# cslab-ntua/sparsex

Measured on AMD Instinct MI355X. Metric: SpMV GFLOP/s (2*nnz/t, alpha=0.5, x/y resident in HBM), higher is better.
Workload: dtype f64

## Files before the change

include/sparsex_hip.h:

```cpp
#ifndef SPARSEX_HIP_H
#define SPARSEX_HIP_H

#include <sparsex/sparsex.h>
#include <stdint.h>

#ifdef __cplusplus
extern "C" {
#endif

spx_error_t spx_hip_matvec_mult(spx_value_t alpha, const spx_matrix_t *A,
                                const spx_value_t *x_dev, spx_value_t *y_dev,
                                void *stream);
spx_error_t spx_hip_matvec_kernel(spx_value_t alpha, const spx_matrix_t *A,
                                  const spx_value_t *x_dev, spx_value_t beta,
                                  spx_value_t *y_dev, void *stream);

spx_error_t spx_hip_matvec_trans_mult(spx_value_t alpha, const spx_matrix_t *A,
                                      const spx_value_t *x_dev, spx_value_t *y_dev,
                                      void *stream);
spx_error_t spx_hip_matvec_trans_kernel(spx_value_t alpha, const spx_matrix_t *A,
                                        const spx_value_t *x_dev, spx_value_t beta,
                                        spx_value_t *y_dev, void *stream);
int spx_hip_matvec_trans_mode(const spx_matrix_t *A);

spx_error_t spx_hip_matvec_mult_f32(spx_value_t alpha, const spx_matrix_t *A, const spx_value_t *x_dev,
                                    spx_value_t *y_dev, void *stream);
spx_error_t spx_hip_matvec_kernel_f32(spx_value_t alpha, const spx_matrix_t *A, const spx_value_t *x_dev,
                                      spx_value_t beta, spx_value_t *y_dev, void *stream);
int64_t spx_hip_mat_values_f32_bytes(const spx_matrix_t *A);
double spx_hip_mat_values_f32_narrow_seconds(const spx_matrix_t *A);

spx_error_t spx_hip_matmat_kernel(spx_value_t alpha, const spx_matrix_t *A, size_t nvec,
                                  const spx_value_t *X_dev, size_t ldx, spx_value_t beta,
                                  spx_value_t *Y_dev, size_t ldy, void *stream);
int spx_hip_matmat_group(const spx_matrix_t *A);

spx_error_t spx_hip_matmat_rm_kernel(spx_value_t alpha, const spx_matrix_t *A, size_t nvec,
                                     const spx_value_t *X_dev, size_t ldx, spx_value_t beta,
                                     spx_value_t *Y_dev, size_t ldy, void *stream);
int spx_hip_matmat_rm_group(const spx_matrix_t *A);

spx_error_t spx_hip_matmat_kernel_f32(spx_value_t alpha, const spx_matrix_t *A, size_t nvec,
                                      const spx_value_t *X_dev, size_t ldx, spx_value_t beta,
                                      spx_value_t *Y_dev, size_t ldy, void *stream);
spx_error_t spx_hip_matmat_rm_kernel_f32(spx_value_t alpha, const spx_matrix_t *A, size_t nvec,
                                         const spx_value_t *X_dev, size_t ldx, spx_value_t beta,
                                         spx_value_t *Y_dev, size_t ldy, void *stream);
int spx_hip_matmat_group_f32(const spx_matrix_t *A);

typedef struct spx_hip_vec spx_hip_vec_t;

void spx_hip_vec_touch(const spx_vector_t *v);
int spx_hip_vec_page_locked(const spx_vector_t *v);

spx_hip_vec_t *spx_hip_vec_create(size_t size);
spx_hip_vec_t *spx_hip_vec_create_from_host(const spx_vector_t *v);
spx_error_t spx_hip_vec_destroy(spx_hip_vec_t *v);
spx_value_t *spx_hip_vec_data(spx_hip_vec_t *v);
size_t spx_hip_vec_size(const spx_hip_vec_t *v);
spx_error_t spx_hip_vec_upload(spx_hip_vec_t *dst, const spx_vector_t *src, void *stream);
spx_error_t spx_hip_vec_download(const spx_hip_vec_t *src, spx_vector_t *dst, void *stream);
spx_error_t spx_hip_vec_init(spx_hip_vec_t *v, spx_value_t val, void *stream);
spx_error_t spx_hip_vec_scale(const spx_hip_vec_t *v1, spx_hip_vec_t *v2, spx_value_t num,
                              void *stream);
spx_error_t spx_hip_vec_scale_add(const spx_hip_vec_t *v1, const spx_hip_vec_t *v2,
                                  spx_hip_vec_t *v3, spx_value_t num, void *stream);
spx_error_t spx_hip_vec_add(const spx_hip_vec_t *v1, const spx_hip_vec_t *v2,
                            spx_hip_vec_t *v3, void *stream);
spx_error_t spx_hip_vec_sub(const spx_hip_vec_t *v1, const spx_hip_vec_t *v2,
                            spx_hip_vec_t *v3, void *stream);
spx_error_t spx_hip_vec_mul(const spx_hip_vec_t *v1, const spx_hip_vec_t *v2,
                            spx_value_t *result, void *stream);
spx_error_t spx_hip_vec_copy(const spx_hip_vec_t *v1, spx_hip_vec_t *v2, void *stream);
spx_error_t spx_hip_vec_mul_dev(const spx_hip_vec_t *v1, const spx_hip_vec_t *v2,
                                spx_value_t *result_dev, void *stream);
spx_error_t spx_hip_vec_scale_add_ratio(const spx_hip_vec_t *v1, const spx_hip_vec_t *v2, spx_hip_vec_t *v3,
                                        spx_value_t scale, const spx_value_t *num_dev,
                                        const spx_value_t *den_dev, void *stream);
spx_error_t spx_hip_vec_cg_update(spx_hip_vec_t *x, const spx_hip_vec_t *p, spx_hip_vec_t *r,
                                  const spx_hip_vec_t *ap, spx_value_t *rr_dev,
                                  const spx_value_t *pap_dev, spx_value_t *beta_dev, void *stream);
spx_error_t spx_hip_vec_mul_elem(const spx_hip_vec_t *v1, const spx_hip_vec_t *v2, spx_hip_vec_t *v3, void *stream);
spx_error_t spx_hip_vec_reciprocal(const spx_hip_vec_t *v1, spx_hip_vec_t *v2, spx_value_t if_zero, void *stream);
spx_error_t spx_hip_vec_pcg_update(spx_hip_vec_t *x, const spx_hip_vec_t *p, spx_hip_vec_t *r, const spx_hip_vec_t *ap,
                                   const spx_hip_vec_t *minv, spx_value_t *rz_dev, const spx_value_t *pap_dev,
                                   spx_value_t *beta_dev, spx_value_t *rr_dev, void *stream);
spx_error_t spx_hip_vec_pcg_direction(spx_hip_vec_t *p, const spx_hip_vec_t *r, const spx_hip_vec_t *minv,
                                      const spx_value_t *beta_dev, void *stream);
spx_error_t spx_hip_probe_read_write(const spx_hip_vec_t *src, spx_hip_vec_t *dst, size_t chunk_doubles,
                                     size_t write_doubles, void *stream);
spx_error_t spx_hip_matvec_kernel_vec(spx_value_t alpha, const spx_matrix_t *A,
                                      const spx_hip_vec_t *x, spx_value_t beta,
                                      spx_hip_vec_t *y, void *stream);
spx_error_t spx_hip_matvec_kernel_f32_vec(spx_value_t alpha, const spx_matrix_t *A, const spx_hip_vec_t *x,
                                          spx_value_t beta, spx_hip_vec_t *y, void *stream);
spx_error_t spx_hip_matvec_trans_kernel_vec(spx_value_t alpha, const spx_matrix_t *A,
                                            const spx_hip_vec_t *x, spx_value_t beta,
                                            spx_hip_vec_t *y, void *stream);

typedef struct spx_hip_transport {
    void *ctx;
    int rank, world;
    int (*exchange_host)(void *ctx, const uint64_t *send, const size_t *send_off,
                         const size_t *send_cnt, uint64_t *recv, const size_t *recv_off,
                         const size_t *recv_cnt);
    int (*exchange_device)(void *ctx, const spx_value_t *send, const size_t *send_off,
                           const size_t *send_cnt, spx_value_t *recv, const size_t *recv_off,
                           const size_t *recv_cnt, void *stream);
} spx_hip_transport_t;

#define SPX_RCCL_ID_BYTES 128
spx_error_t spx_hip_rccl_unique_id(void *id);
// ... 182 lines not shown
```

sparsex_amd/api.py:

```python
import ctypes as C
import os

import numpy as np

SPX_SUCCESS = 0
SPX_FAILURE = -1
SPX_MAT_REORDER = 42
SPX_VEC_AS_IS = 43
SPX_VEC_TUNE = 44
SPX_INDEX_ZERO_BASED = 45
SPX_INDEX_ONE_BASED = 46

_HERE = os.path.dirname(os.path.abspath(__file__))


def lib_path():
    return os.environ.get("SPX_LIB_PATH") or os.path.join(_HERE, "lib", "libsparsex.so")


class SpxError(RuntimeError):
    pass


class VectorStruct(C.Structure):
# ... 56 lines not shown

class UnitRecord(C.Structure):
    _fields_ = [("type", C.c_int32), ("delta", C.c_int32), ("size", C.c_int32),
                ("row", C.c_int32), ("col", C.c_int32)]


_lib = None


def lib():
    global _lib
    if _lib is not None:
        return _lib
    path = lib_path()
    if not os.path.exists(path):
        raise SpxError(
            "libsparsex.so is not built (%s); run `make lib` or "
            "__graft_entry__.build() -- there is no fallback path" % path)
    L = C.CDLL(path, mode=C.RTLD_GLOBAL)
    vp, i, d = C.c_void_p, C.c_int, C.c_double
    L.spx_input_load_csr.restype = vp
    L.spx_input_load_mmf.restype = vp
    L.spx_input_load_mmf.argtypes = [C.c_char_p]
    L.spx_input_destroy.argtypes = [vp]
    L.spx_mat_tune.restype = vp
    L.spx_mat_destroy.argtypes = [vp]
    L.spx_mat_get_nrows.argtypes = [vp]
    L.spx_mat_get_ncols.argtypes = [vp]
    L.spx_mat_get_nnz.argtypes = [vp]
    L.spx_mat_get_partition.restype = vp
    L.spx_mat_get_partition.argtypes = [vp]
    L.spx_partition_get_rs.restype = C.POINTER(C.c_int)
    L.spx_partition_get_rs.argtypes = [vp]
    L.spx_partition_get_re.restype = C.POINTER(C.c_int)
    L.spx_partition_get_re.argtypes = [vp]
    L.spx_partition_destroy.argtypes = [vp]
    L.spx_option_set.argtypes = [C.c_char_p, C.c_char_p]
    L.spx_option_set.restype = None
    L.spx_hip_options_reset.restype = None
    L.spx_vec_create_from_buff.restype = C.POINTER(VectorStruct)
    L.spx_vec_create_from_buff.argtypes = [C.POINTER(C.c_double), vp, C.c_size_t, vp,
                                           C.c_uint]
    L.spx_vec_destroy.argtypes = [C.POINTER(VectorStruct)]
    L.spx_vec_destroy.restype = None
    L.spx_matvec_mult.argtypes = [d, vp, C.POINTER(VectorStruct), C.POINTER(VectorStruct)]
    L.spx_matvec_kernel.argtypes = [d, vp, C.POINTER(VectorStruct), d,
                                    C.POINTER(VectorStruct)]
    L.spx_hip_matvec_mult.argtypes = [d, vp, vp, vp, vp]
    L.spx_hip_matvec_kernel.argtypes = [d, vp, vp, d, vp, vp]
    L.spx_hip_mat_info.argtypes = [vp, C.POINTER(HipInfo)]
    L.spx_hip_mat_export_csx.argtypes = [vp, i, C.POINTER(CsxExport)]
    L.spx_hip_mat_export_units.restype = C.c_int64
    L.spx_hip_mat_export_units.argtypes = [vp, i, C.POINTER(UnitRecord), C.c_int64]
    L.spx_hip_mat_tune_log.restype = C.c_char_p
    L.spx_hip_mat_tune_log.argtypes = [vp]
    L.spx_hip_vec_create.restype = vp
    L.spx_hip_vec_create.argtypes = [C.c_size_t]
    L.spx_hip_vec_destroy.argtypes = [vp]
    L.spx_hip_vec_data.restype = vp
    L.spx_hip_vec_data.argtypes = [vp]
    L.spx_hip_vec_size.restype = C.c_size_t
    L.spx_hip_vec_size.argtypes = [vp]
    L.spx_hip_vec_upload.argtypes = [vp, C.POINTER(VectorStruct), vp]
    L.spx_hip_vec_download.argtypes = [vp, C.POINTER(VectorStruct), vp]
    L.spx_hip_vec_init.argtypes = [vp, d, vp]
    L.spx_hip_vec_scale.argtypes = [vp, vp, d, vp]
    L.spx_hip_vec_scale_add.argtypes = [vp, vp, vp, d, vp]
    L.spx_hip_vec_add.argtypes = [vp, vp, vp, vp]
    L.spx_hip_vec_sub.argtypes = [vp, vp, vp, vp]
    L.spx_hip_vec_mul.argtypes = [vp, vp, C.POINTER(C.c_double), vp]
    L.spx_hip_vec_copy.argtypes = [vp, vp, vp]
    L.spx_hip_vec_mul_dev.argtypes = [vp, vp, vp, vp]
    L.spx_hip_vec_scale_add_ratio.argtypes = [vp, vp, vp, d, vp, vp, vp]
    L.spx_hip_vec_cg_update.argtypes = [vp, vp, vp, vp, vp, vp, vp, vp]
    L.spx_hip_matvec_kernel_vec.argtypes = [d, vp, vp, d, vp, vp]
    L.spx_hip_matvec_trans_mult.argtypes = [d, vp, vp, vp, vp]
    L.spx_hip_matvec_trans_kernel.argtypes = [d, vp, vp, d, vp, vp]
    L.spx_hip_matvec_trans_kernel_vec.argtypes = [d, vp, vp, d, vp, vp]
    L.spx_hip_matvec_mult_f32.argtypes = [d, vp, vp, vp, vp]
    L.spx_hip_matvec_kernel_f32.argtypes = [d, vp, vp, d, vp, vp]
    L.spx_hip_matvec_kernel_f32_vec.argtypes = [d, vp, vp, d, vp, vp]
    L.spx_hip_mat_values_f32_bytes.restype = C.c_int64
    L.spx_hip_mat_values_f32_bytes.argtypes = [vp]
    L.spx_hip_mat_values_f32_narrow_seconds.restype = C.c_double
    L.spx_hip_mat_values_f32_narrow_seconds.argtypes = [vp]
    L.spx_hip_matvec_trans_mode.restype = C.c_int
    L.spx_hip_matvec_trans_mode.argtypes = [vp]
    L.spx_hip_mat_values_plan.argtypes = [vp, vp, vp, i]
    L.spx_hip_mat_values_plan_drop.argtypes = [vp]
    L.spx_hip_mat_set_values.argtypes = [vp, vp, vp]
    L.spx_hip_mat_set_values_host.argtypes = [vp, vp]
    L.spx_hip_mat_values_plan_get.argtypes = [vp, C.POINTER(ValuesPlan)]
    L.spx_hip_mat_diag_plan.argtypes = [vp]
    L.spx_hip_mat_diag_plan_drop.argtypes = [vp]
    L.spx_hip_mat_get_diag.argtypes = [vp, vp, vp]
    L.spx_hip_mat_get_diag_vec.argtypes = [vp, vp, vp]
    L.spx_hip_mat_get_diag_host.argtypes = [vp, vp]
    L.spx_hip_mat_diag_plan_get.argtypes = [vp, C.POINTER(DiagPlan)]
    L.spx_hip_vec_mul_elem.argtypes = [vp, vp, vp, vp]
    L.spx_hip_vec_reciprocal.argtypes = [vp, vp, d, vp]
    L.spx_hip_vec_pcg_update.argtypes = [vp, vp, vp, vp, vp, vp, vp, vp, vp, vp]
    L.spx_hip_vec_pcg_direction.argtypes = [vp, vp, vp, vp, vp]
    L.spx_log_disable_all.restype = None
    L.spx_log_error_console.restype = None
    _lib = L
    return L


def option_set(option, value):
    lib().spx_option_set(str(option).encode(), str(value).encode())


def options_reset():
    lib().spx_hip_options_reset()


class Input:

    def __init__(self, handle, keep=()):
        self.handle = handle
        self._keep = keep

    def destroy(self):
        if self.handle:
            lib().spx_input_destroy(self.handle)
            self.handle = None

    def __del__(self):
        try:
            self.destroy()
        except Exception:
            pass


def input_load_csr(rowptr, colind, values, nrows, ncols, indexing=SPX_INDEX_ZERO_BASED):
    rp = np.ascontiguousarray(rowptr, dtype=np.int32)
    ci = np.ascontiguousarray(colind, dtype=np.int32)
    va = np.ascontiguousarray(values, dtype=np.float64)
    h = lib().spx_input_load_csr(
        rp.ctypes.data_as(C.c_void_p), ci.ctypes.data_as(C.c_void_p),
        va.ctypes.data_as(C.c_void_p), C.c_int(nrows), C.c_int(ncols), C.c_int(indexing))
    if not h:
        raise SpxError("spx_input_load_csr failed")
    return Input(h, keep=(rp, ci, va))


def input_load_mmf(filename):
    h = lib().spx_input_load_mmf(str(filename).encode())
    if not h:
        raise SpxError("spx_input_load_mmf failed for %s" % filename)
    return Input(h)


class Matrix:

    def __init__(self, handle):
        self.handle = handle
        L = lib()
        self.nrows = L.spx_mat_get_nrows(handle)
        self.ncols = L.spx_mat_get_ncols(handle)
        self.nnz = L.spx_mat_get_nnz(handle)

    def matvec_mult(self, alpha, x, y):
        return self._host(alpha, x, None, y)

    def matvec_kernel(self, alpha, x, beta, y):
        return self._host(alpha, x, beta, y)

    def _host(self, alpha, x, beta, y):
        L = lib()
        assert x.dtype == np.float64 and y.dtype == np.float64
        assert x.flags.c_contiguous and y.flags.c_contiguous
        xv = L.spx_vec_create_from_buff(x.ctypes.data_as(C.POINTER(C.c_double)), None,
                                        x.size, None, SPX_VEC_AS_IS)
        yv = L.spx_vec_create_from_buff(y.ctypes.data_as(C.POINTER(C.c_double)), None,
                                        y.size, None, SPX_VEC_AS_IS)
        try:
            if beta is None:
                rc = L.spx_matvec_mult(alpha, self.handle, xv, yv)
            else:
                rc = L.spx_matvec_kernel(alpha, self.handle, xv, beta, yv)
        finally:
            L.spx_vec_destroy(xv)
            L.spx_vec_destroy(yv)
        if rc != SPX_SUCCESS:
            raise SpxError("spx_matvec failed (see stderr)")
        return y

    def partition(self):
        L = lib()
        p = L.spx_mat_get_partition(self.handle)
        n = self.info().nr_partitions
        rs = [L.spx_partition_get_rs(p)[i] for i in range(n)]
        re = [L.spx_partition_get_re(p)[i] for i in range(n)]
        L.spx_partition_destroy(p)
        return rs, re

    def hip_matvec_mult(self, alpha, x_ptr, y_ptr, stream=0):
        rc = lib().spx_hip_matvec_mult(alpha, self.handle, x_ptr, y_ptr, stream)
        if rc != SPX_SUCCESS:
            raise SpxError("spx_hip_matvec_mult failed (see stderr)")

    def hip_matvec_kernel(self, alpha, x_ptr, beta, y_ptr, stream=0):
        rc = lib().spx_hip_matvec_kernel(alpha, self.handle, x_ptr, beta, y_ptr, stream)
        if rc != SPX_SUCCESS:
            raise SpxError("spx_hip_matvec_kernel failed (see stderr)")

    def hip_matvec_trans_kernel(self, alpha, x_ptr, beta, y_ptr, stream=0):
        rc = lib().spx_hip_matvec_trans_kernel(alpha, self.handle, x_ptr, beta, y_ptr, stream)
        if rc != SPX_SUCCESS:
            raise SpxError("spx_hip_matvec_trans_kernel failed (see stderr)")

    def trans_mode(self):
        return int(lib().spx_hip_matvec_trans_mode(self.handle))

    def matvec_trans(self, alpha, x, beta, y, stream=None):
        import torch
        pairs = (("x", x, self.nrows), ("y", y, self.ncols))
        for name, t, n in pairs:
            if not isinstance(t, torch.Tensor):
                raise ValueError("%s must be a torch tensor" % name)
            if t.dtype != torch.float64:
                raise ValueError("%s must be float64, not %s" % (name, t.dtype))
            if t.dim() != 1 or t.shape[0] != n:
                raise ValueError("%s must have the shape (%d,), not %s" % (name, n, tuple(t.shape)))
            if t.shape[0] > 1 and t.stride(0) != 1:
                raise ValueError("%s needs stride(0) == 1, not %d" % (name, t.stride(0)))
        for name, t, n in pairs:
            if t.device.type != "cuda":
                raise ValueError("%s must live on the matrix' HIP device, not on %s" % (name, t.device))
        if x.device != y.device:
            raise ValueError("x and y live on different devices (%s, %s)" % (x.device, y.device))
        inf = self.info()
        if inf.on_device and x.device.index != inf.device:
            raise ValueError("the matrix lives on cuda:%d, the tensors on %s" % (inf.device, x.device))
        st = stream if stream is not None else torch.cuda.current_stream(y.device)
        self.hip_matvec_trans_kernel(alpha, x.data_ptr(), beta, y.data_ptr(), st.cuda_stream)
        return y

    def hip_matvec_kernel_f32(self, alpha, x_ptr, beta, y_ptr, stream=0):
        rc = lib().spx_hip_matvec_kernel_f32(alpha, self.handle, x_ptr, beta, y_ptr, stream)
        if rc != SPX_SUCCESS:
            raise SpxError("spx_hip_matvec_kernel_f32 failed (see stderr)")

    def values_f32_bytes(self):
        return int(lib().spx_hip_mat_values_f32_bytes(self.handle))

    def matvec_f32(self, alpha, x, beta, y, stream=None):
        import torch
        pairs = (("x", x, self.ncols), ("y", y, self.nrows))
        for name, t, n in pairs:
            if not isinstance(t, torch.Tensor):
                raise ValueError("%s must be a torch tensor" % name)
            if t.dtype != torch.float64:
                raise ValueError("%s must be float64, not %s" % (name, t.dtype))
            if t.dim() != 1 or t.shape[0] != n:
                raise ValueError("%s must have the shape (%d,), not %s" % (name, n, tuple(t.shape)))
            if t.shape[0] > 1 and t.stride(0) != 1:
                raise ValueError("%s needs stride(0) == 1, not %d" % (name, t.stride(0)))
        for name, t, n in pairs:
            if t.device.type != "cuda":
                raise ValueError("%s must live on the matrix' HIP device, not on %s" % (name, t.device))
        if x.device != y.device:
            raise ValueError("x and y live on different devices (%s, %s)" % (x.device, y.device))
        inf = self.info()
        if inf.on_device and x.device.index != inf.device:
            raise ValueError("the matrix lives on cuda:%d, the tensors on %s" % (inf.device, x.device))
        st = stream if stream is not None else torch.cuda.current_stream(y.device)
        self.hip_matvec_kernel_f32(alpha, x.data_ptr(), beta, y.data_ptr(), st.cuda_stream)
        return y

    def hip_matmat_kernel(self, alpha, x_ptr, ldx, nvec, beta, y_ptr, ldy, stream=0):
        L = lib()
        L.spx_hip_matmat_kernel.restype = C.c_int
        L.spx_hip_matmat_kernel.argtypes = [C.c_double, C.c_void_p, C.c_size_t, C.c_void_p, C.c_size_t,
                                            C.c_double, C.c_void_p, C.c_size_t, C.c_void_p]
        rc = L.spx_hip_matmat_kernel(alpha, self.handle, nvec, x_ptr, ldx, beta, y_ptr, ldy, stream)
        if rc != SPX_SUCCESS:
            raise SpxError("spx_hip_matmat_kernel failed (see stderr)")

    def matmat_group(self):
        L = lib()
        L.spx_hip_matmat_group.restype = C.c_int
        L.spx_hip_matmat_group.argtypes = [C.c_void_p]
        return int(L.spx_hip_matmat_group(C.c_void_p(self.handle)))

    def matmat(self, alpha, X, beta, Y, stream=None):
        return self._matmat(self.hip_matmat_kernel, alpha, X, beta, Y, stream)

    def _matmat(self, kernel, alpha, X, beta, Y, stream):
        import torch
        pairs = (("X", X, self.ncols), ("Y", Y, self.nrows))
        for name, t, n in pairs:
            if not isinstance(t, torch.Tensor):
                raise ValueError("%s must be a torch tensor" % name)
            if t.dtype != torch.float64:
                raise ValueError("%s must be float64, not %s" % (name, t.dtype))
            if t.dim() != 2 or t.shape[1] != n:
                raise ValueError("%s must have the shape (nvec, %d), not %s" % (name, n, tuple(t.shape)))
            if t.shape[0] > 0 and t.shape[1] > 1 and t.stride(1) != 1:
                raise ValueError("%s needs stride(1) == 1, not %d" % (name, t.stride(1)))
            if t.shape[0] > 1 and t.stride(0) < n:
                raise ValueError("%s: stride(0) %d is below the vector length %d" % (name, t.stride(0), n))
        if X.shape[0] != Y.shape[0]:
            raise ValueError("X holds %d vectors, Y %d" % (X.shape[0], Y.shape[0]))
        for name, t, n in pairs:
            if t.device.type != "cuda":
                raise ValueError("%s must live on the matrix' HIP device, not on %s" % (name, t.device))
        if X.device != Y.device:
            raise ValueError("X and Y live on different devices (%s, %s)" % (X.device, Y.device))
        inf = self.info()
        if inf.on_device and X.device.index != inf.device:
            raise ValueError("the matrix lives on cuda:%d, the tensors on %s" % (inf.device, X.device))
        nvec = int(X.shape[0])
        ldx = max(int(X.stride(0)), self.ncols) if nvec > 1 else max(self.ncols, 1)
        ldy = max(int(Y.stride(0)), self.nrows) if nvec > 1 else max(self.nrows, 1)
        st = stream if stream is not None else torch.cuda.current_stream(Y.device)
        kernel(alpha, X.data_ptr(), ldx, nvec, beta, Y.data_ptr(), ldy, st.cuda_stream)
        return Y

    def hip_matmat_kernel_f32(self, alpha, x_ptr, ldx, nvec, beta, y_ptr, ldy, stream=0):
        L = lib()
        L.spx_hip_matmat_kernel_f32.restype = C.c_int
        L.spx_hip_matmat_kernel_f32.argtypes = [C.c_double, C.c_void_p, C.c_size_t, C.c_void_p, C.c_size_t,
                                                C.c_double, C.c_void_p, C.c_size_t, C.c_void_p]
        rc = L.spx_hip_matmat_kernel_f32(alpha, self.handle, nvec, x_ptr, ldx, beta, y_ptr, ldy, stream)
        if rc != SPX_SUCCESS:
            raise SpxError("spx_hip_matmat_kernel_f32 failed (see stderr)")

# ... 750 lines not shown
```

sparsex_amd/csrc/api.cpp:

```cpp
#include <sparsex/sparsex.h>
#include <sparsex_hip.h>

#include "config.hpp"
#include "csx_emit.hpp"
#include "device.hpp"
#include "dist.hpp"
#include "encoder.hpp"
#include "gpu_emit.hpp"
#include "input.hpp"
#include "reorder.hpp"
#include "stream_index.hpp"
#include "threads.hpp"

#include <chrono>
#include <cmath>
#include <cstdarg>
#include <cstdint>
#include <cstring>
#include <functional>
#include <memory>
#include <mutex>
#include <atomic>
#include <sstream>
#include <thread>
// ... 497 lines not shown
            emit_pieces(fulls, &tiles, use_segs ? &segs : nullptr);
            {
                struct Gone {
                    std::vector<Partition> fulls;
                    std::vector<SymSegVec> segs;
                    std::vector<std::vector<SymTile>> tiles;
                };
                Gone *g = new Gone();
                g->fulls.swap(fulls);
                g->segs.swap(segs);
                g->tiles.swap(tiles);
                release_after_upload = [g] {
                    parallel_for(g->fulls.size(), host_threads(), [&](size_t i) {
                        g->fulls[i] = Partition();
                        if (i < g->segs.size()) SymSegVec().swap(g->segs[i]);
                        if (i < g->tiles.size()) std::vector<SymTile>().swap(g->tiles[i]);
                    });
                    delete g;
                };
            }
            for (size_t k = 0; k < thin.size(); ++k) {
                if (k == 0 || thin[k].row != thin[k - 1].row) {
                    gs.mirror_rows.push_back((uint32_t) thin[k].row);
                    gs.mirror_ptr.push_back((uint32_t) k);
                }
                gs.mirror_col.push_back((uint32_t) thin[k].col);
                gs.mirror_val.push_back(thin[k].val);
            }
            gs.mirror_ptr.push_back((uint32_t) thin.size());
            gs.nnz_stored += thin.size();
            gs.n_delta_elems += thin.size();
        } else {
            Partition full;
            for (size_t i = 0; i < nown; ++i) append_sym_expanded(A->parts[i], full, gp.sym_remine);
            if (gs.sym_fused) full.nr_rows = (size_t) A->nrows;
            emit_gpu(full, gp, gs, hw);
        }
    } else if (A->col_phases <= 1) {
        emit_pieces(A->parts, nullptr);
    } else {
        const size_t K = A->col_phases;
        GpuEmitParams keep = gp;
        gp.max_rows = std::max<size_t>(gp.max_rows, SPX_MAX_WIDE_ROWS);
        for (size_t k = 0; k < K; ++k) {
            const idx_t c_lo = (idx_t)((int64_t) A->ncols * (int64_t) k / (int64_t) K) + 1;
            const idx_t c_hi = (idx_t)((int64_t) A->ncols * (int64_t)(k + 1) / (int64_t) K) + 1;
            std::vector<Partition> sub(nown);
            parallel_for(nown, hw, [&](size_t i) {
                const Partition &p = A->parts[i];
                Partition &q = sub[i];
                q.nr_rows = p.nr_rows; q.nr_cols = p.nr_cols; q.type = p.type; q.row_start = p.row_start;
                q.pool = p.pool;
                for (size_t e = 0; e < p.elems_size; ++e)
                    if (p.elems[e].col >= c_lo && p.elems[e].col < c_hi) {
                        q.elems.push_back(p.elems[e]);
                        q.nnz += p.elems[e].size;
                    }
                q.elems_size = q.elems.size();
            });
            gp.skip_empty = k > 0 || A->col_concurrent;
            const size_t rb0 = gs.rbs.size();
            emit_pieces(sub, nullptr);
            if (k > 0 && gs.rbs.size() > rb0) gs.rbs[rb0].flags |= SPX_RB_PHASE_START;
            if (A->col_concurrent && gs.rbs.size() == rb0) throw FatalError("column phases: an empty slice");
        }
        if (A->col_concurrent)
            for (SpxRowBlock &rb : gs.rbs) rb.flags |= SPX_RB_ACCUM;
        gp = keep;
        if (!gs.shared.empty()) throw FatalError("column phases: the matrix holds rows that are split over row-blocks");
    }
    const double t_emit1 = now_sec();
    A->conflict_rows.clear();
    if (sym && !gs.sym_fused) stream_touched_rows(gs, A->own_lo, A->conflict_rows);
    A->halo_cols.clear();
    if (A->own_lo > 0 || A->own_hi < A->nrows) stream_read_cols(gs, A->own_lo, A->own_hi, (size_t) A->ncols, A->halo_cols);
    A->first_block_row = A->own_lo;
    for (const SpxRowBlock &rb : gs.rbs) A->first_block_row = std::min<idx_t>(A->first_block_row, (idx_t) rb.row0);
    finalize_stream(gs, (size_t) A->nrows);
    if (sym) mark_private_rowblocks(gs, (size_t) A->nrows, A->own_lo, A->own_hi);
    std::vector<std::pair<uint32_t, uint32_t>>().swap(gs.direct_cols);
    gs.waves = (uint32_t) A->waves;
    gs.band_order = Config::instance().get_bool("spx.gpu.band_order");
    gs.arena = Config::instance().get_bool("spx.gpu.arena");
    gs.xw_budget = (A->unit_windows != 0 && !A->deterministic && !sym) ? (A->rb_joined ? std::max(A->xw_budget, JOINED_XW_BUDGET) : A->xw_budget) : 0u;
    gs.xw_gap = A->xw_gap;
    gs.xw_on = A->xw_on;
    gs.sx_plan = sym && A->sym_pipeline != 0 && !A->deterministic && A->wave_tiles != 1;
    gs.sx_on = A->sx_on;
    gs.sym_matmat = A->sym_matmat;
    gs.sym_atomic = A->sym_atomic && !A->deterministic;
    gs.deterministic = A->deterministic;
    gs.wave_tiles = A->deterministic || A->wave_tiles == 1;
    A->nnz_stored = gs.nnz_stored;
    A->n_unit_elems = gs.n_unit_elems;
    A->n_delta_elems = gs.n_delta_elems;
    A->n_units = gs.n_units;
    A->value_bytes = gs.values.size() * sizeof(val_t);
    A->index_bytes = gs.index_bytes();
    A->n_rowblocks = gs.rbs.size();
    A->n_shared = gs.shared.size();
    A->has_tiles = stream_has_tiles(gs);
    A->has_symtiles = stream_has_pass(gs, SPX_PASS_SYMTILE);
    if (A->dev) {
        device_free(A->dev);
        A->dev = nullptr;
    }
    const double t_emit2 = now_sec();
    if (!A->host_only) {
        A->dev = device_upload(gs, (size_t) A->nrows, (size_t) A->ncols, sym, A->own_lo, A->own_hi,
                               A->device_ordinal);
        device_set_trans_windows(A->dev, A->trans_windows);
        log_msg(LOG_INFO, "descriptor stream: emitted in %.2f s, finalized in %.2f s, uploaded in %.2f s (%zu row-blocks)\n",
                t_emit1 - t_emit0, t_emit2 - t_emit1, now_sec() - t_emit2, gs.rbs.size());
        if (A->dist && sym) {
            device_set_init_rows(A->dev, (size_t) dist_first_init_row(*A));
        }
        keep_index(A, std::move(gs));
    } else {
        A->host_stream.reset(new GpuStream(std::move(gs)));
    }
    if (release_after_upload) {
        std::function<void()> f;
        f.swap(release_after_upload);
        A->release_wait();
        A->release_later(std::move(f));
    }
}

static void autotune_launch(spx_matrix_t *A, bool tune_waves, bool tune_spill, bool tune_wave_tiles, bool tune_xw)
{
    A->release_wait();
    const double t_est = device_time_spmv(A->dev, 2, 3);
    const int N = (int) std::min(100.0, std::max(8.0, 0.02 / std::max(t_est, 1e-7)));
    const int W = std::max(2, N / 10);
    auto best_time = [&]() {
        A->release_wait();
        double best = device_time_spmv(A->dev, W, N);
        for (int rep = 0; rep < 3; ++rep) best = std::min(best, device_time_spmv(A->dev, 0, N));
        return best;
    };
    auto time_xw = [&](bool &xw) {
        if (!tune_xw || !device_has_xw(A->dev) || A->wave_tiles == 1) {
            xw = device_get_xw(A->dev);
            return best_time();
        }
        device_set_xw(A->dev, false);
        const double t0 = best_time();
        device_set_xw(A->dev, true);
        const double t1 = best_time();
        xw = t1 < 0.985 * t0;
        device_set_xw(A->dev, xw);
        return std::min(t0, xw ? t1 : t0);
    };
    if (!tune_waves) {
        if (tune_wave_tiles && !device_has_tiles(A->dev) && !(A->unit_windows == 1 && device_has_xw(A->dev))) {
            auto t_of = [&](bool on) {
                device_set_wave_tiles(A->dev, on);
                return best_time();
            };
            const double t0 = t_of(false), t1 = t_of(true);
            bool on = t1 < 0.985 * t0;
            if (on) {
                const double t0b = t_of(false), t1b = t_of(true);
                on = t1b < 0.985 * t0b;
            }
            A->wave_tiles = on ? 1 : 0;
// ... 58 lines not shown
            emit_and_upload(A);
            bool xw2 = false;
            const double t2 = time_with(2, xw2);
            if (t2 < 0.985 * best_t) {
                best_t = t2;
                best_waves = 2;
                best_scale = scale;
                best_xw = xw2;
            }
        }
        A->xw_on = best_xw;
        if (A->rb_scale != best_scale) {
            A->rb_scale = best_scale;
            A->waves = best_waves;
            emit_and_upload(A);
        }
    }
    if (A->auto_rb && A->n_rowblocks > 4096 &&
        auto_target_elems(A, 2.0) != auto_target_elems(A, best_scale)) {
        A->rb_scale = 2.0;
        A->waves = best_waves;
        emit_and_upload(A);
        bool xwb = false;
        const double tb = time_with(best_waves, xwb);
        if (tb < 0.985 * best_t) {
            best_t = tb;
            best_scale = 2.0;
            best_xw = xwb;
            A->xw_on = best_xw;
        } else {
            A->rb_scale = best_scale;
            A->xw_on = best_xw;
            emit_and_upload(A);
        }
    }
    A->rb_scale = best_scale;
    A->waves = best_waves;
    A->xw_on = best_xw;
    if (A->auto_rb && best_xw && A->wave_tiles != 1 && A->emit_params.max_rows <= SPX_MAX_RB_ROWS &&
        A->value_bytes > ((size_t) 1 << 30)) {
        A->rb_joined = true;
        A->waves = 8;
        emit_and_upload(A);
        bool xwj = false;
        const double tj = time_with(8, xwj);
        if (xwj && tj < 0.995 * best_t) {
            best_t = tj;
            best_waves = 8;
            log_msg(LOG_INFO, "launch autotune: row-blocks joined side by side (%zu of them)\n", A->n_rowblocks);
        } else {
            A->rb_joined = false;
            A->waves = best_waves;
            A->xw_on = best_xw;
            emit_and_upload(A);
        }
    }
    A->waves = best_waves;
    A->xw_on = best_xw;
    device_set_waves(A->dev, best_waves);
    device_set_xw(A->dev, best_xw);
    log_msg(LOG_INFO, "launch autotune: %d wavefronts per workgroup, row-block scale %.2f%s, unit windows %s (%.2f us per SpMV)\n",
            best_waves, best_scale, A->rb_joined ? ", joined" : "", best_xw ? "on" : "off", 1e6 * best_t);
}

static int read_trans_windows()
{
    const std::string tw = Config::instance().get_str("spx.gpu.trans_windows");
    if (tw != "auto" && tw != "true" && tw != "false") {
        log_msg(LOG_ERR, "spx.gpu.trans_windows: true, false or auto\n");
        throw FatalError("bad spx.gpu.trans_windows");
    }
    return tw == "auto" ? -1 : (tw == "true" ? 1 : 0);
}

static int read_values_f32()
{
    const std::string v = Config::instance().get_str("spx.gpu.values_f32");
    if (v != "true" && v != "false" && v != "all") {
        log_msg(LOG_ERR, "spx.gpu.values_f32: false, true or all\n");
        throw FatalError("bad spx.gpu.values_f32");
    }
    return v == "all" ? 2 : (v == "true" ? 1 : 0);
}
static bool wants_values_f32(int mode, bool symmetric) { return mode == 2 || (mode == 1 && !symmetric); }

static spx_matrix_t *do_tune(spx_input_t *in)
{
    Config &cfg = Config::instance();
    const double t0 = now_sec();
    const size_t P = cfg.nr_partitions();
    long world = std::max<long>(1, cfg.get_long("spx.rt.gpu_world"));
    long rank = cfg.get_long("spx.rt.gpu_rank");
    if (rank < 0 || rank >= world || P % (size_t) world != 0) {
        log_msg(LOG_ERR, "spx.rt.gpu_rank/gpu_world (%ld/%ld) do not divide "
                "spx.rt.nr_threads=%zu partitions\n", rank, world, P);
        throw FatalError("bad gpu_rank/gpu_world");
    }
    const size_t first = (size_t) rank * (P / (size_t) world);
    const size_t last = first + P / (size_t) world;
    const long slice_rows = cfg.get_long("spx.rt.global_rows");
    const long slice_off = slice_rows > 0 ? cfg.get_long("spx.rt.row_offset") : 0;
    if (slice_rows > 0 && (world != 1 || slice_off < 0 || slice_off + (long) in->nrows > slice_rows)) {
        log_msg(LOG_ERR, "spx.rt.row_offset/global_rows (%ld/%ld) do not hold the %ld input rows "
                "(and exclude spx.rt.gpu_world > 1)\n", slice_off, slice_rows, (long) in->nrows);
        throw FatalError("bad row slice");
    }
    in->mat->row_base = (size_t) slice_off;
    in->mat->global_rows = slice_rows > 0 ? (size_t) slice_rows : 0;
    const idx_t rows_end = slice_rows > 0 ? (idx_t)(slice_off + in->nrows) : in->nrows;
    const bool sym = cfg.get_bool("spx.matrix.symmetric");
    const bool host_only = cfg.get_bool("spx.rt.host_only");
    EncoderParams prm = EncoderParams::from_config(cfg);
    XformSeq seq = cfg.xform();
    cfg.cpu_affinity();
    log_msg(LOG_INFO, "Format: %s\n", sym ? "CSX-sym" : "CSX");
    if (!host_only && device_count() <= 0) {
        log_msg(LOG_ERR, "no usable HIP device: this library multiplies on an MI355X "
                "only (spx.rt.host_only=true preprocesses without one)\n");
        throw FatalError("no HIP device");
    }

    std::unique_ptr<matrix> A(new matrix);
    A->nrows = slice_rows > 0 ? (spx_index_t) slice_rows : in->nrows;
    A->ncols = in->ncols;
    A->nnz = in->nnz;
    A->symmetric = sym ? 1 : 0;
    A->permutation = SPX_INVALID_PERM;
    A->nr_partitions = P;
    A->first_part = first;
    A->last_part = last;
    A->full_colind = cfg.get_bool("spx.matrix.full_colind");
    A->dev = nullptr;
    A->host_only = host_only;
    A->device_ordinal = (int) cfg.get_long("spx.rt.device");
    A->input_row_base = slice_rows > 0 ? (int64_t) slice_off : -1;

    const size_t nown = last - first;
    std::vector<std::ostringstream> logs(nown);
    std::vector<std::string> errors(nown);
    std::vector<PartitionSym> sparts;
    if (sym) {
        build_partitions_sym(*in->mat, P, first, last, sparts, A->bounds);
        A->diag.resize(nown);
    } else {
        build_partitions(*in->mat, P, first, last, A->parts, A->bounds);
    }

    const double t_parts = now_sec();
    log_msg(LOG_INFO, "partitions built in %.2f s\n", t_parts - t0);
    auto work = [&](size_t i) {
        try {
            std::ostream *lg = &logs[i];
            *lg << "==> Thread: #" << (first + i) << "\n==== ENCODING STATISTICS ====\n";
            if (sym) {
                PartitionSym &ps = sparts[i];
                ps.divide();
                Encoder e1(&ps.m1, prm), e2(&ps.m2, prm);
                if (seq.explicit_deltas) {
                    e1.encode_serial(seq);
                    e2.encode_serial(seq);
                } else {
                    e1.remove_ignore(seq);
                    e2.remove_ignore(seq);
                    if (ps.lower.row_start > 0) e1.encode_all(lg);
                    e2.encode_all(lg);
                }
// ... 45 lines not shown
    A->emit_params.sym_pure_passes = cfg.get_bool("spx.gpu.sym_pure_passes");
    A->emit_params.x_window = cfg.get_bool("spx.gpu.x_window");
    {
        const std::string m = cfg.get_str("spx.gpu.sym_segments");
        if (m != "auto" && m != "true" && m != "false") {
            log_msg(LOG_ERR, "spx.gpu.sym_segments: true, false or auto\n");
            throw FatalError("bad spx.gpu.sym_segments");
        }
        A->emit_params.sym_segments = m == "auto" ? -1 : (m == "true" ? 1 : 0);
        const long wide = cfg.get_long("spx.gpu.sym_wide_rows");
        if (wide < 1 || wide > SPX_MAX_WIDE_ROWS) {
            log_msg(LOG_ERR, "spx.gpu.sym_wide_rows: 1 .. %d\n", SPX_MAX_WIDE_ROWS);
            throw FatalError("bad spx.gpu.sym_wide_rows");
        }
        A->emit_params.wide_rows = (size_t) wide;
        const long mr = cfg.get_long("spx.gpu.sym_segment_min");
        if (mr < 2 || mr > 8) {
            log_msg(LOG_ERR, "spx.gpu.sym_segment_min: 2 .. 8\n");
            throw FatalError("bad spx.gpu.sym_segment_min");
        }
        A->emit_params.sym_min_run = (size_t) mr;
        const long xr = cfg.get_long("spx.gpu.sym_segment_max");
        if (xr < mr || xr > SPX_MAX_SEG_WIDTH) {
            log_msg(LOG_ERR, "spx.gpu.sym_segment_max: spx.gpu.sym_segment_min .. %d\n", SPX_MAX_SEG_WIDTH);
            throw FatalError("bad spx.gpu.sym_segment_max");
        }
        A->emit_params.sym_max_run = (size_t) xr;
    }
    A->emit_params.stack_segments = cfg.get_bool("spx.gpu.stack_segments");
    {
        idx_t lo = nown ? A->bounds[first].row_start : 0;
        idx_t hi = nown ? A->bounds[last - 1].row_start + A->bounds[last - 1].nr_rows : 0;
        if (last == P) hi = rows_end;
        A->own_lo = lo;
        A->own_hi = hi;
    }
    A->waves = (int) cfg.get_long("spx.gpu.waves");
    const bool autotune = A->waves == 0;
    if (autotune) A->waves = 4;
    const std::string spill_mode = cfg.get_str("spx.gpu.sym_spill");
    if (spill_mode != "auto" && spill_mode != "lists" && spill_mode != "atomic") {
        log_msg(LOG_ERR, "spx.gpu.sym_spill: lists, atomic or auto\n");
        throw FatalError("bad spx.gpu.sym_spill");
    }
    A->deterministic = cfg.get_bool("spx.gpu.deterministic");
    A->sym_atomic = spill_mode == "atomic" && !A->deterministic;
    A->spill_mode = spill_mode == "lists" ? 0 : (spill_mode == "atomic" ? 1 : -1);
    {
        const std::string sm = cfg.get_str("spx.gpu.sym_matmat");
        if (sm != "true" && sm != "false") {
            log_msg(LOG_ERR, "spx.gpu.sym_matmat: true or false\n");
            throw FatalError("bad spx.gpu.sym_matmat");
        }
        A->sym_matmat = sm == "true" && sym && A->emit_params.sym_once;
        if (A->sym_matmat) {
            if (spill_mode == "auto" && !A->deterministic) A->sym_atomic = true;
            A->emit_params.wide_rows = std::min<size_t>(A->emit_params.wide_rows, SPX_MAX_RB_ROWS);
        }
    }
    const std::string wt_mode = cfg.get_str("spx.gpu.wave_tiles");
    if (wt_mode != "auto" && wt_mode != "true" && wt_mode != "false") {
        log_msg(LOG_ERR, "spx.gpu.wave_tiles: true, false or auto\n");
        throw FatalError("bad spx.gpu.wave_tiles");
    }
    A->wave_tiles = wt_mode == "true" ? 1 : 0;
    const std::string xw_mode = cfg.get_str("spx.gpu.unit_windows");
    if (xw_mode != "auto" && xw_mode != "true" && xw_mode != "false") {
        log_msg(LOG_ERR, "spx.gpu.unit_windows: true, false or auto\n");
        throw FatalError("bad spx.gpu.unit_windows");
    }
    {
        const long xb = cfg.get_long("spx.gpu.unit_window_doubles"), xg = cfg.get_long("spx.gpu.unit_window_gap");
        if (xb < 0 || xb > 16384 || xg < 0 || xg > 255) {
            log_msg(LOG_ERR, "spx.gpu.unit_window_doubles: 0 .. 16384, spx.gpu.unit_window_gap: 0 .. 255\n");
            throw FatalError("bad spx.gpu.unit_window_doubles / spx.gpu.unit_window_gap");
        }
        A->xw_budget = (uint32_t) xb;
        A->xw_gap = (uint32_t) xg;
    }
    A->unit_windows = xw_mode == "auto" ? -1 : (xw_mode == "true" ? 1 : 0);
    A->xw_on = xw_mode == "true";
    A->trans_windows = read_trans_windows();
    A->values_f32 = read_values_f32();
    const std::string sx_mode = cfg.get_str("spx.gpu.sym_pipeline");
    if (sx_mode != "auto" && sx_mode != "true" && sx_mode != "false") {
        log_msg(LOG_ERR, "spx.gpu.sym_pipeline: true, false or auto\n");
        throw FatalError("bad spx.gpu.sym_pipeline");
    }
    A->sym_pipeline = sx_mode == "auto" ? -1 : (sx_mode == "true" ? 1 : 0);
    A->sx_on = sx_mode == "true";
    const std::string ph_mode = cfg.get_str("spx.gpu.col_phases");
    const bool ph_conc = ph_mode.size() == 2 && ph_mode[0] == 'c';
    long ph_fixed = ph_mode == "auto" ? 0 : strtol(ph_mode.c_str() + (ph_conc ? 1 : 0), nullptr, 10);
    if (ph_mode != "auto" && (ph_fixed < 1 || ph_fixed > 8 || (ph_conc && ph_fixed != 2 && ph_fixed != 4 && ph_fixed != 8))) {
        log_msg(LOG_ERR, "spx.gpu.col_phases: 1 .. 8 (launched in turn), c2 | c4 | c8 (one launch, a group of XCDs each) or auto\n");
        throw FatalError("bad spx.gpu.col_phases");
    }
    A->col_phases = (!sym && ph_fixed > 1) ? (size_t) ph_fixed : 1;
    A->col_concurrent = A->col_phases > 1 && ph_conc && !A->deterministic;
    if (A->col_phases > 1 && ph_conc && !A->col_concurrent) A->col_phases = 1;
    try {
        emit_and_upload(A.get());
    } catch (const FatalError &) {
        if (A->col_phases <= 1) throw;
        A->col_phases = 1;
        emit_and_upload(A.get());
    }
    const bool tune_spill = spill_mode == "auto" && !A->deterministic && !A->has_symsegs && !A->sym_matmat;
    const bool tune_wt = wt_mode == "auto" && !A->deterministic && !A->has_symsegs;
    const bool tune_xw = xw_mode == "auto" && !A->deterministic && !sym;
    const double t_auto = now_sec();
    if (A->dev && A->nnz_stored >= 100000 && (autotune || tune_spill || tune_wt || tune_xw))
        autotune_launch(A.get(), autotune, tune_spill, tune_wt, tune_xw);
    if (A->dev && sym && A->sym_pipeline == -1 && device_has_sx(A->dev)) {
        A->release_wait();
        const double t_est = device_time_spmv(A->dev, 2, 3);
        const int N = (int) std::min(100.0, std::max(8.0, 0.02 / std::max(t_est, 1e-7)));
        auto best_of = [&](bool on) {
            device_set_sx(A->dev, on);
            double best = device_time_spmv(A->dev, std::max(2, N / 10), N);
            for (int rep = 0; rep < 3; ++rep) best = std::min(best, device_time_spmv(A->dev, 0, N));
            return best;
        };
        const double t0 = best_of(false), t1 = best_of(true);
        A->sx_on = t1 < 0.985 * t0;
        device_set_sx(A->dev, A->sx_on);
        log_msg(LOG_INFO, "read-once pipeline: %s (%.2f us per SpMV with, %.2f without)\n", A->sx_on ? "on" : "off", 1e6 * t1, 1e6 * t0);
    }
    const double t_auto_end = now_sec();
    if (A->dev && !sym && ph_mode == "auto" && A->n_shared == 0 && A->nnz_stored >= 100000 &&
        2 * A->n_delta_elems >= A->nnz_stored && (size_t) A->ncols * sizeof(val_t) >= ((size_t) 6 << 20)) {
        auto best_of = [&]() {
            double best = device_time_spmv(A->dev, 10, 100);
            for (int rep = 0; rep < 3; ++rep) best = std::min(best, device_time_spmv(A->dev, 0, 100));
            return best;
        };
        const double t_plain = best_of();
        size_t K = 1;
        double t_ph = t_plain;
        if (!A->deterministic) {
            for (size_t k : {(size_t) 2, (size_t) 4}) {
                if ((size_t) A->ncols * sizeof(val_t) < k * ((size_t) 3 << 19)) break;
                try {
                    A->col_phases = k;
                    A->col_concurrent = true;
                    emit_and_upload(A.get());
                    const double t = best_of();
                    if (t < 0.97 * t_ph) {
                        t_ph = t;
                        K = k;
                    }
                } catch (const FatalError &) {
                    break;
                }
            }
        }
        if (A->col_phases != K || !A->col_concurrent) {
            A->col_phases = K;
            A->col_concurrent = K > 1;
            emit_and_upload(A.get());
        }
        log_msg(LOG_INFO, "column slices: %zu on XCD groups %.2f us, plain %.2f us per SpMV\n", K, 1e6 * t_ph, 1e6 * t_plain);
    }

    if (A->dev && wants_values_f32(A->values_f32, sym)) device_build_values_f32(A->dev);

    if (!cfg.get_bool("spx.rt.keep_encoded")) {
        std::vector<Partition> *old = new std::vector<Partition>();
        old->swap(A->parts);
        A->release_later([old] {
            parallel_for(old->size(), host_threads(), [&](size_t i) { (*old)[i] = Partition(); });
            delete old;
        });
    }
    log_msg(LOG_INFO, "launch parameters measured in %.2f s\n", t_auto_end - t_auto);
    A->emit_seconds = now_sec() - t1;
    return A.release();
}

spx_matrix_t *spx_mat_tune(spx_input_t *in, ...)
try {
    if (!in) {
        SETERROR_1(SPX_ERR_ARG_INVALID, "invalid input matrix");
        return SPX_INVALID_MAT;
    }
    va_list ap;
    va_start(ap, in);
    spx_option_t option = va_arg(ap, spx_option_t);
    va_end(ap);
    std::vector<idx_t> perm;
    if (option == SPX_MAT_REORDER && Config::instance().get_long("spx.rt.global_rows") > 0) {
        SETWARNING(SPX_WARN_REORDER);
        option = 0;
    }
    int re_mode = SPX_DIST_REORDER_RCM;
    size_t re_world = 1;
// ... 479 lines not shown
    if (good) {
        good = h.nrows >= 0 && h.ncols >= 0 && bnd.size() == 3 * h.nr_partitions &&
               h.first_part <= h.last_part && h.last_part <= h.nr_partitions &&
               (perm.empty() || perm.size() == (size_t) h.nrows) && h.own_lo >= 0 &&
               h.own_lo <= h.own_hi && h.own_hi <= h.nrows &&
               (!h.symmetric || gs->dvalues.size() == (size_t) h.nrows);
        for (int32_t v : perm) good = good && v >= 0 && v < h.nrows;
    }
    if (good) {
        gs->n_carry = h.n_carry;
        gs->sym_fused = (h.pad & 1u) != 0;
        gs->pass_stride = h.pad >> 1;
        gs->n_spill = h.n_spill;
        gs->lds_doubles = h.lds_doubles;
        gs->waves = h.waves;
        gs->sym_atomic = h.sym_atomic != 0;
        gs->deterministic = (h.pad3 & 1u) != 0;
        gs->wave_tiles = (h.pad3 & 2u) != 0;
        gs->xw_on = (h.pad3 & 4u) != 0;
        gs->sx_on = (h.pad3 & 8u) != 0;
        gs->sx_plan = gs->sx_on;
        gs->xw_gap = gs->xw_on ? ((h.pad3 >> 8) & 255u) : 16u;
        gs->xw_budget = gs->xw_on ? (h.pad3 >> 16) : 0u;
        gs->nnz_stored = h.nnz_stored; gs->n_unit_elems = h.n_unit_elems;
        gs->n_delta_elems = h.n_delta_elems; gs->n_units = h.n_units;
        good = stream_checksum(*gs) == h.checksum;
        if (!good) why = "tuned-matrix file is damaged (checksum of the index arrays)";
        else good = stream_validate(*gs, (size_t) h.nrows, (size_t) h.ncols, gs->values.size(), why);
    }
    if (!good) {
        SETERROR_1(SPX_ERR_FILE, why.c_str());
        return SPX_INVALID_MAT;
    }
    A->nrows = h.nrows; A->ncols = h.ncols; A->nnz = h.nnz; A->symmetric = h.symmetric;
    A->permutation = SPX_INVALID_PERM;
    if (!perm.empty()) {
        A->permutation = (spx_perm_t *) malloc(perm.size() * sizeof(spx_perm_t));
        std::copy(perm.begin(), perm.end(), A->permutation);
    }
    A->nr_partitions = h.nr_partitions; A->first_part = h.first_part; A->last_part = h.last_part;
    for (size_t i = 0; i < h.nr_partitions; ++i)
        A->bounds.push_back(PartBounds{bnd[3 * i], bnd[3 * i + 1], (size_t) bnd[3 * i + 2]});
    A->full_colind = false;
    A->dev = nullptr;
    A->waves = (h.waves == 2 || h.waves == 8) ? (int) h.waves : 4;
    A->own_lo = h.own_lo; A->own_hi = h.own_hi;
    if (h.first_part == 0 && h.last_part == h.nr_partitions && (h.own_lo > 0 || h.own_hi < h.nrows))
        A->input_row_base = h.own_lo;
    A->nnz_stored = h.nnz_stored; A->n_unit_elems = h.n_unit_elems;
    A->n_delta_elems = h.n_delta_elems; A->n_units = h.n_units;
    A->value_bytes = gs->values.size() * sizeof(val_t);
    A->index_bytes = gs->index_bytes();
    A->n_rowblocks = gs->rbs.size();
    A->n_shared = gs->shared.size();
    A->has_tiles = stream_has_tiles(*gs);
    A->has_symtiles = stream_has_pass(*gs, SPX_PASS_SYMTILE);
    A->has_symsegs = stream_has_symsegs(*gs);
    A->sym_atomic = gs->sym_atomic;
    A->deterministic = gs->deterministic;
    A->wave_tiles = gs->wave_tiles ? 1 : 0;
    A->xw_on = gs->xw_on;
    A->unit_windows = gs->xw_on ? 1 : 0;
    A->sx_on = gs->sx_on;
    A->sym_pipeline = gs->sx_on ? 1 : 0;
    A->xw_budget = gs->xw_budget;
    A->xw_gap = gs->xw_gap;
    {
        size_t slices = 1;
        for (size_t i = 1; i < gs->rbs.size(); ++i) slices += (gs->rbs[i].flags & SPX_RB_PHASE_START) ? 1 : 0;
        A->col_phases = slices;
        A->col_concurrent = slices > 1 && !gs->rbs.empty() && (gs->rbs[0].flags & SPX_RB_ACCUM);
    }
    A->tune_seconds = 0.0;
    A->auto_rb = false;
    const double t0 = now_sec();
    Config &cfg = Config::instance();
    A->host_only = cfg.get_bool("spx.rt.host_only");
    A->device_ordinal = (int) cfg.get_long("spx.rt.device");
    A->full_colind = cfg.get_bool("spx.matrix.full_colind");
    A->sym_matmat = gs->sym_matmat = A->symmetric && cfg.get_str("spx.gpu.sym_matmat") == "true";
    try {
        A->trans_windows = read_trans_windows();
        A->values_f32 = read_values_f32();
    } catch (const FatalError &) {
        SETERROR_0(SPX_ERR_TUNED_MAT);
        return SPX_INVALID_MAT;
    }
    if (A->symmetric && !gs->sym_fused) stream_touched_rows(*gs, A->own_lo, A->conflict_rows);
    if (A->own_lo > 0 || A->own_hi < A->nrows) stream_read_cols(*gs, A->own_lo, A->own_hi, (size_t) A->ncols, A->halo_cols);
    A->first_block_row = A->own_lo;
    for (const SpxRowBlock &rb : gs->rbs) A->first_block_row = std::min<idx_t>(A->first_block_row, (idx_t) rb.row0);
    try {
        if (!A->host_only) {
            A->dev = device_upload(*gs, (size_t) A->nrows, (size_t) A->ncols, A->symmetric != 0,
                                   A->own_lo, A->own_hi, A->device_ordinal);
            device_set_trans_windows(A->dev, A->trans_windows);
            if (wants_values_f32(A->values_f32, A->symmetric != 0)) device_build_values_f32(A->dev);
            keep_index(A.get(), std::move(*gs));
        } else {
            A->host_stream = std::move(gs);
        }
    } catch (const FatalError &) {
        SETERROR_0(SPX_ERR_TUNED_MAT);
        return SPX_INVALID_MAT;
    }
    A->emit_seconds = now_sec() - t0;
    return A.release();
} SPX_C_BOUNDARY(return SPX_INVALID_MAT;)

spx_index_t spx_mat_get_nrows(const spx_matrix_t *A)
try {
    if (!A) { SETERROR_1(SPX_ERR_ARG_INVALID, "invalid matrix handle"); return SPX_FAILURE; }
    return A->nrows;
} SPX_C_BOUNDARY(return 0;)

spx_index_t spx_mat_get_ncols(const spx_matrix_t *A)
try {
    if (!A) { SETERROR_1(SPX_ERR_ARG_INVALID, "invalid matrix handle"); return SPX_FAILURE; }
    return A->ncols;
} SPX_C_BOUNDARY(return 0;)

spx_index_t spx_mat_get_nnz(const spx_matrix_t *A)
try {
    if (!A) { SETERROR_1(SPX_ERR_ARG_INVALID, "invalid matrix handle"); return SPX_FAILURE; }
    return A->nnz;
} SPX_C_BOUNDARY(return 0;)

static spx_partition_t *part_alloc(size_t n)
{
    spx_partition_t *p = (spx_partition_t *) malloc(sizeof(spx_partition_t));
    p->nr_partitions = n;
    p->parts = NULL;
    p->nodes = NULL;
    p->affinity = NULL;
    p->row_start = (spx_index_t *) malloc(sizeof(spx_index_t) * (n ? n : 1));
    p->row_end = (spx_index_t *) malloc(sizeof(spx_index_t) * (n ? n : 1));
    return p;
}

spx_partition_t *spx_mat_get_partition(const spx_matrix_t *A)
try {
    if (!A) {
        SETERROR_1(SPX_ERR_ARG_INVALID, "invalid matrix handle");
        return SPX_INVALID_PART;
    }
    spx_partition_t *p = part_alloc(A->nr_partitions);
    for (size_t i = 0; i < A->nr_partitions; ++i) {
        p->row_start[i] = A->bounds[i].row_start;
        p->row_end[i] = A->bounds[i].row_start + A->bounds[i].nr_rows;
    }
    return p;
} SPX_C_BOUNDARY(return SPX_INVALID_PART;)

spx_index_t *spx_partition_get_rs(const spx_partition_t *p)
try {
    if (!p) { SETERROR_1(SPX_ERR_ARG_INVALID, "invalid partition handle"); return NULL; }
    return p->row_start;
} SPX_C_BOUNDARY(return nullptr;)

spx_index_t *spx_partition_get_re(const spx_partition_t *p)
try {
    if (!p) { SETERROR_1(SPX_ERR_ARG_INVALID, "invalid partition handle"); return NULL; }
    return p->row_end;
} SPX_C_BOUNDARY(return nullptr;)

spx_perm_t *spx_mat_get_perm(const spx_matrix_t *A)
try {
    if (!A) {
        SETERROR_1(SPX_ERR_ARG_INVALID, "invalid matrix handle");
        return SPX_INVALID_PERM;
    }
    if (!A->permutation) {
        SETERROR_1(SPX_ERR_ARG_INVALID, "a permutation is not available");
        return SPX_INVALID_PERM;
    }
    return A->permutation;
} SPX_C_BOUNDARY(return SPX_INVALID_PERM;)

spx_partition_t *spx_partition_csr(const spx_index_t *rowptr, spx_index_t nr_rows,
// ... 165 lines not shown
    }
    return SPX_SUCCESS;
}

spx_error_t spx_hip_matvec_mult(spx_value_t alpha, const spx_matrix_t *A,
                                const spx_value_t *x_dev, spx_value_t *y_dev, void *stream)
try {
    return spx_hip_matvec_kernel(alpha, A, x_dev, 0.0, y_dev, stream);
} SPX_C_BOUNDARY(return SPX_FAILURE;)

spx_error_t spx_hip_matvec_kernel(spx_value_t alpha, const spx_matrix_t *A,
                                  const spx_value_t *x_dev, spx_value_t beta,
                                  spx_value_t *y_dev, void *stream)
try {
    if (check_dev(A, x_dev, y_dev) != SPX_SUCCESS) return SPX_FAILURE;
    try {
        device_spmv(A->dev, alpha, x_dev, beta, y_dev, stream);
    } catch (const FatalError &e) {
        SETERROR_1(SPX_ERR_TUNED_MAT, e.what.c_str());
        return SPX_FAILURE;
    }
    return SPX_SUCCESS;
} SPX_C_BOUNDARY(return SPX_FAILURE;)

spx_error_t spx_hip_matvec_trans_mult(spx_value_t alpha, const spx_matrix_t *A,
                                      const spx_value_t *x_dev, spx_value_t *y_dev, void *stream)
try {
    return spx_hip_matvec_trans_kernel(alpha, A, x_dev, 0.0, y_dev, stream);
} SPX_C_BOUNDARY(return SPX_FAILURE;)

spx_error_t spx_hip_matvec_trans_kernel(spx_value_t alpha, const spx_matrix_t *A,
                                        const spx_value_t *x_dev, spx_value_t beta,
                                        spx_value_t *y_dev, void *stream)
try {
    if (check_dev(A, x_dev, y_dev) != SPX_SUCCESS) return SPX_FAILURE;
    const uintptr_t x0 = (uintptr_t) x_dev, x1 = x0 + (size_t) A->nrows * sizeof(double);
    const uintptr_t y0 = (uintptr_t) y_dev, y1 = y0 + (size_t) A->ncols * sizeof(double);
    if (x0 < y1 && y0 < x1) {
        SETERROR_1(SPX_ERR_ARG_INVALID, "vectors x and y overlap");
        return SPX_FAILURE;
    }
    if (A->dist && !A->symmetric) {
        SETERROR_1(SPX_ERR_TUNED_MAT, "no transposed product on a general matrix with an exchange plan attached");
        return SPX_FAILURE;
    }
    try {
        device_spmv_trans(A->dev, alpha, x_dev, beta, y_dev, stream);
    } catch (const FatalError &e) {
        SETERROR_1(SPX_ERR_TUNED_MAT, e.what.c_str());
        return SPX_FAILURE;
    }
    return SPX_SUCCESS;
} SPX_C_BOUNDARY(return SPX_FAILURE;)

spx_error_t spx_hip_matvec_mult_f32(spx_value_t alpha, const spx_matrix_t *A,
                                    const spx_value_t *x_dev, spx_value_t *y_dev, void *stream)
try {
    return spx_hip_matvec_kernel_f32(alpha, A, x_dev, 0.0, y_dev, stream);
} SPX_C_BOUNDARY(return SPX_FAILURE;)

spx_error_t spx_hip_matvec_kernel_f32(spx_value_t alpha, const spx_matrix_t *A,
                                      const spx_value_t *x_dev, spx_value_t beta,
                                      spx_value_t *y_dev, void *stream)
try {
    if (check_dev(A, x_dev, y_dev) != SPX_SUCCESS) return SPX_FAILURE;
    const uintptr_t x0 = (uintptr_t) x_dev, x1 = x0 + (size_t) A->ncols * sizeof(double);
    const uintptr_t y0 = (uintptr_t) y_dev, y1 = y0 + (size_t) A->nrows * sizeof(double);
    if (x0 < y1 && y0 < x1) {
        SETERROR_1(SPX_ERR_ARG_INVALID, "vectors x and y overlap");
        return SPX_FAILURE;
    }
    try {
        device_spmv_f32(A->dev, alpha, x_dev, beta, y_dev, stream);
    } catch (const FatalError &e) {
        SETERROR_1(SPX_ERR_TUNED_MAT, e.what.c_str());
        return SPX_FAILURE;
    }
    return SPX_SUCCESS;
} SPX_C_BOUNDARY(return SPX_FAILURE;)

int64_t spx_hip_mat_values_f32_bytes(const spx_matrix_t *A)
try {
    return A && A->dev ? device_values_f32_bytes(A->dev) : -1;
} SPX_C_BOUNDARY(return -1;)

double spx_hip_mat_values_f32_narrow_seconds(const spx_matrix_t *A)
try {
    if (!A || !A->dev || device_values_f32_bytes(A->dev) <= 0) return -1.0;
    return device_time_narrow_values(A->dev);
} SPX_C_BOUNDARY(return -1.0;)

int spx_hip_matvec_trans_mode(const spx_matrix_t *A)
try {
    return A && A->dev ? device_trans_mode(A->dev) : -1;
} SPX_C_BOUNDARY(return -1;)

spx_error_t spx_hip_matvec_parts(spx_value_t alpha, const spx_matrix_t *A, const spx_value_t *x_dev,
                                 spx_value_t beta, spx_value_t *y_dev, int parts, void *stream, int *launched)
try {
    if (check_dev(A, x_dev, y_dev) != SPX_SUCCESS) return SPX_FAILURE;
    try {
        std::vector<size_t> bounds;
        const size_t K = (A->symmetric || parts < 2) ? 0 : device_plan_chunks(A->dev, (size_t) parts, bounds, 1);
        if (K == 0) {
            device_spmv(A->dev, alpha, x_dev, beta, y_dev, stream);
        } else {
            for (size_t k = 0; k < K; ++k) device_spmv_chunk(A->dev, k, alpha, x_dev, beta, y_dev, stream, 1);
        }
        if (launched) *launched = K ? (int) K : 1;
    } catch (const FatalError &e) {
        SETERROR_1(SPX_ERR_TUNED_MAT, e.what.c_str());
        return SPX_FAILURE;
    }
    return SPX_SUCCESS;
} SPX_C_BOUNDARY(return SPX_FAILURE;)

spx_error_t spx_hip_matvec_dist(spx_value_t alpha, const spx_matrix_t *A,
                                const spx_value_t *x_dev, spx_value_t beta,
                                spx_value_t *y_dev, int flags, void *stream)
try {
    if (check_dev(A, x_dev, y_dev) != SPX_SUCCESS) return SPX_FAILURE;
    if (!A->dist) {
        SETERROR_1(SPX_ERR_TUNED_MAT, "matrix has no exchange plan (spx_hip_mat_dist_attach)");
        return SPX_FAILURE;
    }
    try {
        if ((flags & SPX_DIST_OVERLAP) && (flags & SPX_DIST_HALO_X) && !(flags & SPX_DIST_GATHER_Y) &&
            !A->symmetric && A->dist->rounds && A->dist->world > 1) {
            dist_step_overlapped(A->dist, A->dev, alpha, x_dev, beta, y_dev, stream);
            return SPX_SUCCESS;
        }
        device_spmv(A->dev, alpha, x_dev, beta, y_dev, stream);
        dist_complete(A->dist, y_dev, (flags & SPX_DIST_GATHER_Y) != 0, (flags & SPX_DIST_HALO_X) != 0, stream);
    } catch (const FatalError &e) {
        SETERROR_1(SPX_ERR_TUNED_MAT, e.what.c_str());
        return SPX_FAILURE;
    }
    return SPX_SUCCESS;
} SPX_C_BOUNDARY(return SPX_FAILURE;)

static spx_error_t matmat_checked(bool f32, spx_value_t alpha, const spx_matrix_t *A, size_t nvec,
                                  const spx_value_t *X_dev, size_t ldx, spx_value_t beta,
                                  spx_value_t *Y_dev, size_t ldy, void *stream)
{
    if (!A) { SETERROR_1(SPX_ERR_ARG_INVALID, "invalid matrix handle"); return SPX_FAILURE; }
    if (!A->dev) {
        SETERROR_1(SPX_ERR_TUNED_MAT,
                   "matrix was tuned with spx.rt.host_only=true: no HIP executor");
        return SPX_FAILURE;
    }
    if (nvec == 0) return SPX_SUCCESS;
    if (!X_dev) { SETERROR_1(SPX_ERR_ARG_INVALID, "invalid block X"); return SPX_FAILURE; }
    if (!Y_dev) { SETERROR_1(SPX_ERR_ARG_INVALID, "invalid block Y"); return SPX_FAILURE; }
    const size_t nr = (size_t) A->nrows, nc = (size_t) A->ncols;
    if (ldx < nc || ldy < nr) {
        SETERROR_1(SPX_ERR_DIM, "leading dimension below the vector length (ldx >= ncols, ldy >= nrows)");
        return SPX_FAILURE;
    }
    const size_t limit = SIZE_MAX / sizeof(double);
    if ((ldx && nvec - 1 > (limit - nc) / ldx) || (ldy && nvec - 1 > (limit - nr) / ldy)) {
        SETERROR_1(SPX_ERR_ARG_INVALID, "block larger than the address space");
        return SPX_FAILURE;
    }
    const uintptr_t x0 = (uintptr_t) X_dev, x1 = x0 + ((nvec - 1) * ldx + nc) * sizeof(double);
    const uintptr_t y0 = (uintptr_t) Y_dev, y1 = y0 + ((nvec - 1) * ldy + nr) * sizeof(double);
    if (x0 < y1 && y0 < x1) {
// ... 844 lines not shown
```

sparsex_amd/csrc/config.cpp:

```cpp
#include "config.hpp"

#include <cstdlib>
#include <regex>
#include <sstream>

namespace spx {

Config &Config::instance()
{
    static Config c;
    return c;
}

Config::Config() { reset_defaults(); }

void Config::reset_defaults()
{
    props_.clear();
    props_["spx.rt.nr_threads"] = "1";
    props_["spx.rt.cpu_affinity"] = "0";
    props_["spx.preproc.heuristic"] = "ratio";
    props_["spx.preproc.xform"] = "all";
    props_["spx.preproc.sampling"] = "portion";
    props_["spx.preproc.sampling.nr_samples"] = "48";
    props_["spx.preproc.sampling.portion"] = "0.01";
    props_["spx.preproc.sampling.window_size"] = "0";
    props_["spx.matrix.symmetric"] = "false";
    props_["spx.matrix.split_blocks"] = "true";
    props_["spx.matrix.full_colind"] = "false";
    props_["spx.matrix.min_unit_size"] = "4";
    props_["spx.matrix.max_unit_size"] = "255";
    props_["spx.matrix.min_coverage"] = "0.1";
    props_["spx.matrix.onedim_blocks"] = "false";
    props_["spx.rt.host_only"] = "false";
    props_["spx.rt.gpu_rank"] = "0";
    props_["spx.rt.gpu_world"] = "1";
    props_["spx.rt.device"] = "-1";
    props_["spx.vec.register"] = "auto";
    props_["spx.vec.device"] = "false";
    props_["spx.rt.host_parts"] = "0";
    props_["spx.rt.dist_chunks"] = "4";
    props_["spx.rt.dist_reorder"] = "none";
    props_["spx.rt.row_offset"] = "0";
    props_["spx.rt.global_rows"] = "0";
    props_["spx.rt.keep_encoded"] = "true";
    props_["spx.gpu.rowblock_elems"] = "0";
    props_["spx.gpu.rowblock_rows"] = "512";
    props_["spx.gpu.stack_segments"] = "true";
    props_["spx.gpu.waves"] = "0";
    props_["spx.gpu.inline_desc"] = "true";
    props_["spx.gpu.arena"] = "false";
    props_["spx.gpu.band_order"] = "false";
    props_["spx.gpu.col_phases"] = "auto";
    props_["spx.gpu.keep_units"] = "true";
    props_["spx.gpu.recut_linear"] = "true";
    props_["spx.gpu.sym_once"] = "true";
    props_["spx.gpu.deterministic"] = "false";
    props_["spx.gpu.wave_tiles"] = "auto";
    props_["spx.gpu.x_window"] = "true";
    props_["spx.gpu.sym_segments"] = "auto";
    props_["spx.gpu.sym_segment_min"] = "2";
    props_["spx.gpu.sym_segment_max"] = "8";
    props_["spx.gpu.sym_wide_rows"] = "1024";
    props_["spx.gpu.sym_spill"] = "auto";
    props_["spx.gpu.sym_matmat"] = "false";
    props_["spx.gpu.sym_remine"] = "true";
    props_["spx.gpu.sym_pure_passes"] = "true";
    props_["spx.gpu.sym_pipeline"] = "auto";
    props_["spx.gpu.unit_windows"] = "auto";
    props_["spx.gpu.unit_window_doubles"] = "3072";
    props_["spx.gpu.unit_window_gap"] = "16";
    props_["spx.gpu.values_f32"] = "false";
    props_["spx.gpu.trans_windows"] = "auto";
}

bool Config::set(const std::string &key, const std::string &value)
{
    auto it = props_.find(key);
    if (it == props_.end()) {
        log_msg(LOG_WARN, "mnemonic \"%s\" not found\n", key.c_str());
        return false;
    }
    if (key == "spx.preproc.heuristic" && value != "ratio" && value != "cost") {
        log_msg(LOG_ERR, "invalid value \"%s\" while setting property "
                "\"spx.preproc.heuristic\"\n", value.c_str());
        throw FatalError("invalid heuristic");
    }
    if (key == "spx.preproc.sampling" && value != "none" && value != "window" &&
        value != "portion") {
        log_msg(LOG_ERR, "invalid value \"%s\" while setting property "
                "\"spx.preproc.sampling\"\n", value.c_str());
        throw FatalError("invalid sampling method");
    }
    it->second = value;
    return true;
}

void Config::load_from_env()
{
    const char *s;
    if ((s = getenv("SYMMETRIC"))) set("spx.matrix.symmetric", s);
    if ((s = getenv("CPU_AFFINITY"))) set("spx.rt.cpu_affinity", s);
    if ((s = getenv("NUM_THREADS"))) set("spx.rt.nr_threads", s);
    if ((s = getenv("XFORM_CONF"))) set("spx.preproc.xform", s);
    if ((s = getenv("WINDOW_SIZE"))) {
        set("spx.preproc.sampling", "window");
        set("spx.preproc.sampling.window_size", s);
    }
    if ((s = getenv("SAMPLES"))) set("spx.preproc.sampling.nr_samples", s);
    if ((s = getenv("SAMPLING_PORTION"))) {
        set("spx.preproc.sampling", "portion");
        set("spx.preproc.sampling.portion", s);
    }
    if ((s = getenv("SAMPLING"))) set("spx.preproc.sampling", s);
    if ((s = getenv("SPX_VEC_DEVICE"))) set("spx.vec.device", s);
}

std::string Config::get_str(const std::string &key) const
{
    auto it = props_.find(key);
    if (it == props_.end()) {
        log_msg(LOG_ERR, "property \"%s\" not found\n", key.c_str());
        throw FatalError("unknown property");
    }
    return it->second;
}

long Config::get_long(const std::string &key) const
{
    std::string v = get_str(key);
    char *end = nullptr;
    long r = strtol(v.c_str(), &end, 10);
    if (end == v.c_str() || *end != '\0') {
        log_msg(LOG_ERR, "invalid value \"%s\" while setting property \"%s\"\n",
                v.c_str(), key.c_str());
        throw FatalError("bad integer property");
    }
    return r;
}

double Config::get_double(const std::string &key) const
{
    std::string v = get_str(key);
    char *end = nullptr;
    double r = strtod(v.c_str(), &end);
    if (end == v.c_str() || *end != '\0') {
        log_msg(LOG_ERR, "invalid value \"%s\" while setting property \"%s\"\n",
                v.c_str(), key.c_str());
        throw FatalError("bad floating-point property");
    }
    return r;
}

bool Config::get_bool(const std::string &key) const
{
// ... 63 lines not shown
```

sparsex_amd/csrc/device.hpp:

```cpp
#pragma once

#include "gpu_emit.hpp"

#include <functional>
#include <string>
#include <vector>

namespace spx {

struct DeviceMatrix;

int device_count();
DeviceMatrix *device_upload(const GpuStream &s, size_t nrows, size_t ncols,
                            bool symmetric, idx_t own_row_lo, idx_t own_row_hi,
                            int device);
void device_free(DeviceMatrix *m);

void device_spmv(DeviceMatrix *m, double alpha, const double *d_x, double beta,
                 double *d_y, void *stream);

void device_build_values_f32(DeviceMatrix *m);
int64_t device_values_f32_bytes(const DeviceMatrix *m);
double device_time_narrow_values(DeviceMatrix *m);
void device_spmv_f32(DeviceMatrix *m, double alpha, const double *d_x, double beta,
                     double *d_y, void *stream);

void device_spmv_trans(DeviceMatrix *m, double alpha, const double *d_x, double beta,
                       double *d_y, void *stream);
void device_set_trans_windows(DeviceMatrix *m, int mode);
int device_trans_mode(const DeviceMatrix *m);

void device_spmm(DeviceMatrix *m, double alpha, const double *d_X, size_t ldx, size_t nvec, double beta,
                 double *d_Y, size_t ldy, void *stream);
int device_mv_group(const DeviceMatrix *m);
void device_spmm_rm(DeviceMatrix *m, double alpha, const double *d_X, size_t ldx, size_t nvec, double beta,
                    double *d_Y, size_t ldy, void *stream);
int device_mv_group_rm(const DeviceMatrix *m);
void device_spmm_f32(DeviceMatrix *m, double alpha, const double *d_X, size_t ldx, size_t nvec, double beta,
                     double *d_Y, size_t ldy, void *stream);
int device_mv_group_f32(const DeviceMatrix *m);
void device_spmm_rm_f32(DeviceMatrix *m, double alpha, const double *d_X, size_t ldx, size_t nvec, double beta,
                        double *d_Y, size_t ldy, void *stream);

size_t device_plan_chunks(DeviceMatrix *m, size_t K, std::vector<size_t> &row_bounds, int slot = 0);
void device_spmv_chunk(DeviceMatrix *m, size_t k, double alpha, const double *d_x, double beta,
                       double *d_y, void *stream, int slot = 0, int position = -1);

void device_spmv_host(DeviceMatrix *m, double alpha, const double *h_x, bool x_pinned,
                      double beta, double *h_y, bool y_pinned,
                      const std::function<void(double *, void *)> &after = nullptr,
                      uint64_t x_version = 0);

bool device_stream_is_capturing(void *stream);

void *device_host_alloc(size_t bytes);
void device_host_free(void *p);
size_t device_host_parts_min_bytes();
int device_host_register(void *p, size_t bytes);
void device_host_unregister(void *p);

void device_set_init_rows(DeviceMatrix *m, size_t first_row);

void device_set_sym_atomic(DeviceMatrix *m, bool on);
bool device_get_sym_atomic(const DeviceMatrix *m);
bool device_has_spill(const DeviceMatrix *m);

void device_set_deterministic(DeviceMatrix *m, bool on);
bool device_get_deterministic(const DeviceMatrix *m);
void device_set_wave_tiles(DeviceMatrix *m, bool on);
bool device_get_wave_tiles(const DeviceMatrix *m);
bool device_has_tiles(const DeviceMatrix *m);

void device_set_waves(DeviceMatrix *m, int waves);
int device_get_waves(const DeviceMatrix *m);

bool device_has_xw(const DeviceMatrix *m);
int device_host_order(const DeviceMatrix *m, int32_t *order, int cap);
void device_set_host_parts(DeviceMatrix *m, size_t parts);
int device_host_parts(const DeviceMatrix *m);
void device_set_xw(DeviceMatrix *m, bool on);
bool device_get_xw(const DeviceMatrix *m);
void device_xw_info(const DeviceMatrix *m, uint64_t &elems_lds, uint64_t &unit_elems, uint64_t &staged_doubles,
                    uint32_t &lds_bytes);

bool device_has_sx(const DeviceMatrix *m);
void device_set_sx(DeviceMatrix *m, bool on);
bool device_get_sx(const DeviceMatrix *m);
void device_sx_info(const DeviceMatrix *m, uint64_t &elems_sx, uint64_t &elems_sym, size_t &rowblocks);

double device_time_spmv(DeviceMatrix *m, int warmup, int launches);

void device_download(const DeviceMatrix *m, GpuStream &s);

double device_peek(const DeviceMatrix *m, bool diagonal, size_t index);
void device_poke(DeviceMatrix *m, bool diagonal, size_t index, double value);
void device_poke_mirror(DeviceMatrix *m, size_t index, double value);

struct ValuesPlan;
size_t device_values_plan_set(DeviceMatrix *m, const ValuesPlan &plan);
void device_values_plan_drop(DeviceMatrix *m);
void device_set_values(DeviceMatrix *m, const double *d_csr_values, void *stream);
void device_set_values_host(DeviceMatrix *m, const double *h_csr_values, size_t csr_nnz);
struct DiagPlan;
size_t device_diag_plan_set(DeviceMatrix *m, const DiagPlan &plan);
void device_diag_plan_drop(DeviceMatrix *m);
void device_get_diag(DeviceMatrix *m, double *d_diag, void *stream);
void device_get_diag_host(DeviceMatrix *m, double *h_diag);
size_t device_n_values(const DeviceMatrix *m);

struct DeviceMatrixInfo {
    size_t n_rowblocks, n_shared_rows;
    size_t value_bytes, index_bytes;
    int device;
};
void device_info(const DeviceMatrix *m, DeviceMatrixInfo &info);

}
```

sparsex_amd/csrc/device_runtime.cpp:

```cpp
#include "device.hpp"
#include "hip_check.hpp"
#include "spmv_launch.hpp"
#include "spx_abl.hpp"
#include "stream_index.hpp"
#include "sxplan.hpp"
#include "threads.hpp"
#include "values_plan.hpp"
#include "diag_plan.hpp"
#include "xwindows.hpp"

#include <hip/hip_runtime_api.h>

#include <algorithm>
#include <cstdio>
#include <cstdlib>
#include <cstring>
#include <string>
#include <type_traits>
#include <vector>

namespace spx {

struct DeviceMatrix {
    int device = 0;
    size_t nrows = 0, ncols = 0;
    bool symmetric = false;
    bool sym_fused = false;
    uint32_t pass_stride = 1;
    size_t own_lo = 0, own_hi = 0;
    size_t init_lo = 0;
    bool init_limited = false;
    uint32_t n_rb = 0, n_shared = 0, n_carry = 0;
    double *carry_mv = nullptr;
    uint32_t mv_rows = 0, mv_xwin = 0;
    bool sym_matmat = false;
    uint32_t mvsym_core = 0, mvsym_full = 0;
    SpxRowBlock *rbs = nullptr;
    double *values = nullptr;
    SpxUnitDesc *descs = nullptr;
    SpxPass *passes = nullptr;
    uint8_t *cidx = nullptr;
    uint16_t *segrows = nullptr;
    SpxSharedRow *shared = nullptr;
    double *carry = nullptr;
    double *dvalues = nullptr;
    bool has_tiles = false;
    int waves = 4;
    int waves_req = 4;
    uint32_t n_spill = 0, lds_doubles = SPX_MAX_RB_ROWS;
    double *spill = nullptr;
    uint32_t *fix_ptr = nullptr, *fix_idx = nullptr;
    size_t n_fix_ptr = 0, n_fix_idx = 0;
    bool sym_atomic = false;
    size_t n_private_rb = 0;
    bool use_private = false;
    size_t max_slot_groups = 0;
    std::vector<XcdSplit> xcd_split;
    std::vector<uint32_t> xcd_longest;
    bool accum = false;
    std::vector<uint32_t> launch_order;
    size_t band_stride = 0;
    bool launched_since_edit = true;
    bool has_symsegs = false;
    bool has_symtiles = false;
    bool wave_tiles = false;
    bool deterministic = false;
    uint32_t *slot_col = nullptr;
    size_t n_slot_col = 0;
    std::vector<std::pair<size_t, size_t>> private_rows;
    uint32_t n_mirror_rows = 0;
    size_t n_mirror_nnz = 0;
    uint32_t *mirror_rows = nullptr, *mirror_ptr = nullptr, *mirror_col = nullptr;
    double *mirror_val = nullptr;
    double *d_x = nullptr, *d_y = nullptr;
    double *p_x = nullptr, *p_y = nullptr;
    uint64_t x_version = 0;
    hipStream_t host_stream = nullptr;
    hipStream_t copy_stream = nullptr;
    std::vector<hipEvent_t> stage_events;
    std::vector<hipEvent_t> part_events;
    int host_parts = 0;
    bool host_x_by_need = false;
    size_t host_parts_want = 0;
    size_t value_bytes = 0, index_bytes = 0;
    size_t n_values = 0, n_descs = 0, n_passes = 0, n_cidx = 0, n_segrows = 0;
    void *arena = nullptr;
    size_t arena_bytes = 0;
    std::vector<uint64_t> rb_upto;
    std::vector<uint32_t> rb_row0;
    struct ChunkPlan {
        std::vector<XcdSplit> split;
        std::vector<uint32_t> longest;
        std::vector<size_t> bounds;
        size_t asked = 0;
        std::vector<uint32_t> order;
        std::vector<std::vector<uint32_t>> step_pieces;
        XcdSplit front;
        uint32_t front_longest = 0;
    };
    ChunkPlan chunks[3];
    SpxPass *passes_xw = nullptr;
    SpxUnitDesc *xdescs = nullptr;
    XwEntry *xw_tab = nullptr;
    uint32_t lds_doubles_xw = 0;
    uint32_t xw_budget = 0, xw_gap = 0;
    bool xw_on = false;
    uint64_t xw_elems = 0, xw_unit_elems = 0, xw_staged = 0;
    size_t xw_rowblocks = 0;
    bool trans_xw = false;
    uint32_t trans_lds_doubles = 0;
    SpxPass *passes_sx = nullptr;
    uint32_t *sx_tab = nullptr;
    bool sx_on = false;
    uint64_t sx_elems = 0, sx_sym_elems = 0;
    size_t sx_rowblocks = 0;
    std::vector<uint64_t> rb_xneed;
    size_t xneed_piece = 0;
    hipStream_t up_stream = nullptr;
    uint32_t *plan_values = nullptr, *plan_mirror = nullptr, *plan_diag = nullptr;
    size_t plan_n_diag = 0, plan_diag_lo = 0, plan_csr_nnz = 0, plan_bytes = 0;
    bool has_plan = false;
    float *values_f32 = nullptr;
    uint32_t *diag_pos = nullptr;
    size_t diag_n = 0;
    bool has_diag_plan = false;
};

constexpr size_t VALUES_SLACK = 160;

constexpr int MV_MAX_GROUP = 8;
constexpr size_t MV_LDS_BUDGET = (size_t) 80 << 10;
constexpr size_t MVSYM_LDS_BUDGET = (size_t) 80 << 10;
constexpr size_t MVSYM_LDS_FEW = (size_t) 40 << 10;

constexpr size_t STAGE_PIECE = (size_t) 16 << 20;
constexpr size_t HOST_PARTS = 8;
constexpr size_t HOST_PARTS_X = 24, HOST_PARTS_X_SYM = 16;
constexpr size_t HOST_X_PIECE = (size_t) 4 << 20;
constexpr size_t HOST_PARTS_MIN_BYTES = (size_t) 32 << 20;

static size_t host_parts_min_bytes()
{
    static const size_t v = getenv("SPX_HOST_PARTS_MIN_BYTES") ? (size_t) atoll(getenv("SPX_HOST_PARTS_MIN_BYTES"))
                                                               : HOST_PARTS_MIN_BYTES;
    return v;
}

static size_t host_xpiece_doubles(size_t ncols)
{
    static const size_t env = getenv("SPX_HOST_XPIECE_BYTES") ? (size_t) atoll(getenv("SPX_HOST_XPIECE_BYTES")) / sizeof(double) : 0;
    size_t piece = env ? env : HOST_X_PIECE / sizeof(double);
    piece = std::max(piece, (ncols + 63) / 64);
    return (piece + 511) & ~(size_t) 511;
}

int device_count()
{
    int n = 0;
    if (hipGetDeviceCount(&n) != hipSuccess) return 0;
    return n;
}

struct Placement {
    struct Item { void **dst; const void *src; size_t copy_bytes, alloc_bytes; };
    std::vector<Item> items;
    template <typename T, typename A>
    void put(T **dst, const std::vector<T, A> &v, size_t slack_elems = 0)
    {
        size_t bytes = (v.size() + slack_elems) * sizeof(T);
        if (bytes == 0) bytes = sizeof(T);
        items.push_back(Item{reinterpret_cast<void **>(dst), v.data(), v.size() * sizeof(T), bytes});
    }
    static size_t piece(size_t bytes)
    {
        const size_t a = bytes >= ((size_t) 1 << 20) ? ((size_t) 2 << 20) : 256u;
        return (bytes + a - 1) / a * a;
    }
    void flush(DeviceMatrix *m, bool arena)
    {
        if (!arena) {
            for (const Item &it : items) {
                void *d = nullptr;
                HIP_CHECK(hipMalloc(&d, it.alloc_bytes));
                *it.dst = d;
                HIP_CHECK(hipMemset(d, 0, it.alloc_bytes));
                if (it.copy_bytes) HIP_CHECK(hipMemcpy(d, it.src, it.copy_bytes, hipMemcpyHostToDevice));
            }
            return;
        }
        size_t total = 0;
        for (const Item &it : items) total += piece(it.alloc_bytes);
        total = (total + ((size_t) 2 << 20) - 1) & ~(((size_t) 2 << 20) - 1);
        void *base = nullptr;
        HIP_CHECK(hipMalloc(&base, total));
        m->arena = base;
        m->arena_bytes = total;
        HIP_CHECK(hipMemset(base, 0, total));
        std::vector<size_t> order(items.size());
        for (size_t i = 0; i < order.size(); ++i) order[i] = i;
        std::stable_sort(order.begin(), order.end(), [&](size_t a, size_t b) { return items[a].alloc_bytes > items[b].alloc_bytes; });
        size_t at = 0;
        for (size_t i : order) {
            const Item &it = items[i];
            char *d = static_cast<char *>(base) + at;
            *it.dst = d;
            if (it.copy_bytes) HIP_CHECK(hipMemcpy(d, it.src, it.copy_bytes, hipMemcpyHostToDevice));
            at += piece(it.alloc_bytes);
        }
    }
};

DeviceMatrix *device_upload(const GpuStream &s, size_t nrows, size_t ncols,
                            bool symmetric, idx_t own_lo, idx_t own_hi, int device)
{
    if (device_count() <= 0) {
        log_msg(LOG_ERR, "no usable HIP device: the SpMV path of this library runs "
                "on an MI355X only (set spx.rt.host_only=true to tune without one)\n");
        throw FatalError("no HIP device");
    }
    if (device >= 0) HIP_CHECK(hipSetDevice(device));
    if (!s.pass_stride && !s.rbs.empty()) throw FatalError("descriptor stream was not finalized");
    DeviceMatrix *m = new DeviceMatrix;
    HIP_CHECK(hipGetDevice(&m->device));
    m->nrows = nrows;
    m->ncols = ncols;
    m->symmetric = symmetric;
    m->sym_fused = symmetric && s.sym_fused;
    m->pass_stride = s.pass_stride;
    m->waves = m->waves_req = (s.waves == 2 || s.waves == 8) ? (int) s.waves : 4;
    m->own_lo = (size_t) own_lo;
    m->own_hi = (size_t) own_hi;
    m->n_rb = (uint32_t) s.rbs.size();
    m->n_shared = (uint32_t) s.shared.size();
    m->n_carry = s.n_carry;
    Placement place;
    const std::vector<double> no_doubles;
    std::vector<double> dv;
    std::vector<SpxRowBlock> rbs_ordered;
    std::vector<SpxPass> passes_ordered;
    place.put(&m->cidx, s.cidx, 64);
    place.put(&m->segrows, s.segrows, 80);
    place.put(&m->shared, s.shared);
    place.put(&m->carry, no_doubles, s.n_carry ? s.n_carry : 1);
    if (symmetric) {
        dv = s.dvalues;
        dv.resize(nrows, 0.0);
        place.put(&m->dvalues, dv);
    }
    m->n_spill = s.n_spill;
    m->lds_doubles = s.lds_doubles;
    for (const SpxRowBlock &rb : s.rbs)
        for (uint32_t k = 0; k < rb.n_pass && !m->has_tiles; ++k)
            m->has_tiles = s.passes[rb.pass_off + k].kind == SPX_PASS_SYMTILE ||
                           s.passes[rb.pass_off + k].kind == SPX_PASS_SYMSEG;
    if (!m->has_tiles) {
        for (const SpxRowBlock &rb : s.rbs) {
            m->mv_rows = std::max<uint32_t>(m->mv_rows, rb.n_rows);
            m->mv_xwin = std::max<uint32_t>(m->mv_xwin, rb.xwin_len);
        }
        place.put(&m->carry_mv, no_doubles, (size_t) MV_MAX_GROUP * (s.n_carry ? s.n_carry : 1));
        spmv_mv_allow_lds(160u * 1024u);
        if (!symmetric) spmv_mvr_allow_lds(160u * 1024u);
    } else if (symmetric && s.sym_matmat) {
        m->sym_matmat = true;
        for (const SpxRowBlock &rb : s.rbs) {
            m->mv_xwin = std::max<uint32_t>(m->mv_xwin, rb.xwin_len);
            m->mvsym_core = std::max<uint32_t>(m->mvsym_core, (uint32_t) rb.n_slots + rb.n_rows);
            m->mvsym_full = std::max<uint32_t>(m->mvsym_full, (uint32_t) rb.n_slots + rb.n_rows + rb.xwin_len);
        }
        place.put(&m->carry_mv, no_doubles, (size_t) MV_MAX_GROUP * (s.n_carry ? s.n_carry : 1));
        spmv_mv_allow_lds(160u * 1024u);
        spmv_mvsym_allow_lds(160u * 1024u);
    }
    for (const SpxRowBlock &rb : s.rbs)
        for (uint32_t k = 0; k < rb.n_pass && !m->has_symsegs; ++k)
            m->has_symsegs = s.passes[rb.pass_off + k].kind == SPX_PASS_SYMSEG;
    for (const SpxRowBlock &rb : s.rbs)
        for (uint32_t k = 0; k < rb.n_pass && !m->has_symtiles; ++k)
            m->has_symtiles = s.passes[rb.pass_off + k].kind == SPX_PASS_SYMTILE;
    if (s.n_spill) {
        place.put(&m->spill, no_doubles, s.n_spill);
        place.put(&m->fix_ptr, s.fix_ptr);
        place.put(&m->fix_idx, s.fix_idx);
        m->n_fix_ptr = s.fix_ptr.size();
        m->n_fix_idx = s.fix_idx.size();
        place.put(&m->slot_col, s.slot_group_col);
// ... 16 lines not shown
        for (const auto &r : pr) {
            if (!m->private_rows.empty() && m->private_rows.back().second == r.first) m->private_rows.back().second = r.second;
            else m->private_rows.push_back(r);
        }
        m->n_private_rb = pr.size();
        size_t covered = 0;
        for (const auto &r : m->private_rows) covered += r.second - r.first;
        if (m->private_rows.size() > 4 || covered * 4 < nrows) m->private_rows.clear();
        m->use_private = !m->private_rows.empty();
        for (const SpxRowBlock &rb : s.rbs) m->max_slot_groups = std::max<size_t>(m->max_slot_groups, (rb.n_slots + 7u) / 8u);
    }
    {
        const size_t n = s.rbs.size();
        std::vector<uint64_t> upto(n + 1, 0);
        for (size_t i = 0; i < n; ++i) {
            const uint64_t end = i + 1 < n ? s.rbs[i + 1].val_off : (uint64_t) s.values.size();
            upto[i + 1] = upto[i] + (end > s.rbs[i].val_off ? end - s.rbs[i].val_off : 0) + 64u + 2u * s.rbs[i].n_rows;
        }
        m->rb_upto = upto;
        m->rb_row0.resize(n);
        for (size_t i = 0; i < n; ++i) m->rb_row0[i] = s.rbs[i].row0;
        std::vector<size_t> starts(1, 0);
        for (size_t i = 1; i < n; ++i)
            if (s.rbs[i].flags & SPX_RB_PHASE_START) starts.push_back(i);
        starts.push_back(n);
        m->accum = n > 0 && (s.rbs[0].flags & SPX_RB_ACCUM) != 0;
        const size_t K = starts.size() - 1;
        if (m->accum && (K == 2 || K == 4 || K == 8)) {
            XcdSplit xs;
            const uint32_t per = (uint32_t)(8 / K);
            for (size_t k = 0; k < K; ++k) {
                const size_t lo = starts[k], hi = starts[k + 1];
                for (uint32_t j = 0; j < per; ++j) {
                    const uint64_t want = upto[lo] + (upto[hi] - upto[lo]) * j / per;
                    size_t i = (size_t)(std::lower_bound(upto.begin() + lo, upto.begin() + hi + 1, want) - upto.begin());
                    xs.first[k * per + j] = (uint32_t) std::min(std::max(i, lo), hi);
                }
            }
            xs.first[8] = (uint32_t) n;
            uint32_t longest = 0;
            for (uint32_t x = 0; x < 8; ++x) longest = std::max(longest, xs.first[x + 1] - xs.first[x]);
            m->xcd_split.push_back(xs);
            m->xcd_longest.push_back(longest);
            starts.assign(1, n);
        } else if (m->accum) {
            throw FatalError("column slices for one launch: 2, 4 or 8 of them");
        }
        for (size_t ph = 0; ph + 1 < starts.size(); ++ph) {
            const size_t lo = starts[ph], hi = starts[ph + 1];
            XcdSplit xs;
            xs.first[0] = (uint32_t) lo;
            for (uint32_t x = 1; x < 8; ++x) {
                const uint64_t want = upto[lo] + (upto[hi] - upto[lo]) * x / 8;
                size_t i = (size_t)(std::lower_bound(upto.begin() + lo, upto.begin() + hi + 1, want) - upto.begin());
                i = std::min(std::max<size_t>(i, xs.first[x - 1]), hi);
                xs.first[x] = (uint32_t) i;
            }
            xs.first[8] = (uint32_t) hi;
            uint32_t longest = 0;
            for (uint32_t x = 0; x < 8; ++x) longest = std::max(longest, xs.first[x + 1] - xs.first[x]);
            m->xcd_split.push_back(xs);
            m->xcd_longest.push_back(longest);
        }
    }
    {
        std::vector<uint32_t> order;
        if (s.band_order) {
            order.resize(s.rbs.size());
            for (size_t i = 0; i < order.size(); ++i) order[i] = (uint32_t) i;
            bool any = false;
            for (const XcdSplit &xs : m->xcd_split) {
                for (uint32_t x = 0; x < 8; ++x) {
                    size_t S = 0;
                    const std::vector<uint32_t> part = stream_band_order(s, xs.first[x], xs.first[x + 1], S);
                    if (part.empty()) continue;
                    std::copy(part.begin(), part.end(), order.begin() + xs.first[x]);
                    m->band_stride = S;
                    any = true;
                }
            }
            if (!any) order.clear();
        }
        if (order.empty()) {
            place.put(&m->values, s.values, VALUES_SLACK);
            place.put(&m->descs, s.descs, 8);
            place.put(&m->rbs, s.rbs);
            place.put(&m->passes, s.passes, (size_t) s.pass_stride + 6 * MAX_WAVES_PER_BLOCK);
        } else {
            const size_t stride = s.pass_stride;
            std::vector<SpxRowBlock> &rbs = rbs_ordered;
            std::vector<SpxPass> &passes = passes_ordered;
            rbs.resize(s.rbs.size());
            passes.resize(s.passes.size());
            for (size_t i = 0; i < order.size(); ++i) {
                rbs[i] = s.rbs[order[i]];
                rbs[i].pass_off = (uint32_t)(i * stride);
                std::copy(s.passes.begin() + (size_t) order[i] * stride, s.passes.begin() + ((size_t) order[i] + 1) * stride,
                          passes.begin() + i * stride);
            }
            place.put(&m->values, s.values, VALUES_SLACK);
            place.put(&m->descs, s.descs, 8);
            place.put(&m->rbs, rbs);
            place.put(&m->passes, passes, stride + 6 * MAX_WAVES_PER_BLOCK);
            m->launch_order.swap(order);
        }
    }
    if (m->has_symsegs && (size_t) m->lds_doubles * sizeof(double) + 8192u > 64u * 1024u) {
        spmv_allow_lds(SpmvFamily::symseg, 160u * 1024u);
        spmv_allow_lds(SpmvFamily::symseg_notile, 160u * 1024u);
    }
    if (s.deterministic) device_set_deterministic(m, true);
    else if (s.wave_tiles) device_set_wave_tiles(m, true);
    m->n_values = s.values.size(); m->n_descs = s.descs.size(); m->n_passes = s.passes.size();
    m->n_cidx = s.cidx.size(); m->n_segrows = s.segrows.size();
    m->value_bytes = s.values.size() * sizeof(double);
    m->index_bytes = s.index_bytes();
    try {
        place.flush(m, s.arena);
    } catch (...) {
        device_free(m);
        throw;
    }
    m->xw_budget = s.xw_budget;
    m->xw_gap = s.xw_gap;
    if (s.xw_budget && !symmetric && !m->accum && m->xcd_split.size() == 1 && !s.rbs.empty()) {
        try {
            XwPlan plan;
            plan_unit_xwindows(s, ncols, s.xw_budget, s.xw_gap, plan, host_threads());
            for (size_t i = 0; i < s.rbs.size(); ++i)
                m->trans_lds_doubles = std::max(m->trans_lds_doubles, (((uint32_t) s.rbs[i].n_rows + 1u) & ~1u) +
                                                                          plan.tab[i * XW_TAB].off_len);
            if (!m->launch_order.empty()) {
                const size_t stride = s.pass_stride;
                std::vector<SpxPass> po(plan.passes.size());
                std::vector<XwEntry> to(plan.tab.size());
                for (size_t i = 0; i < m->launch_order.size(); ++i) {
                    const size_t from = m->launch_order[i];
                    std::copy(plan.passes.begin() + from * stride, plan.passes.begin() + (from + 1) * stride, po.begin() + i * stride);
                    std::copy(plan.tab.begin() + from * XW_TAB, plan.tab.begin() + (from + 1) * XW_TAB, to.begin() + i * XW_TAB);
                }
                plan.passes.swap(po);
                plan.tab.swap(to);
            }
            if (plan.n_rb_windows && (size_t) plan.lds_doubles * sizeof(double) > 160u * 1024u) {
                log_msg(LOG_INFO, "unit windows: %u KB of LDS per workgroup do not fit, not used\n",
                        (unsigned) ((size_t) plan.lds_doubles * sizeof(double) / 1024u));
            } else if (plan.n_rb_windows) {
                auto up = [&](auto **dst, const auto &v, size_t slack) {
                    typedef typename std::remove_reference<decltype(v[0])>::type T;
                    const size_t bytes = (v.size() + slack) * sizeof(T);
                    HIP_CHECK(hipMalloc(reinterpret_cast<void **>(dst), bytes));
                    HIP_CHECK(hipMemset(*dst, 0, bytes));
                    HIP_CHECK(hipMemcpy(*dst, v.data(), v.size() * sizeof(T), hipMemcpyHostToDevice));
                };
                up(&m->passes_xw, plan.passes, (size_t) s.pass_stride + 6 * MAX_WAVES_PER_BLOCK);
                up(&m->xdescs, plan.xdescs, 8);
                up(&m->xw_tab, plan.tab, 0);
                m->lds_doubles_xw = plan.lds_doubles;
                m->xw_elems = plan.unit_elems_lds;
                m->xw_unit_elems = plan.unit_elems;
                m->xw_staged = plan.staged_doubles;
                m->xw_rowblocks = plan.n_rb_windows;
                m->xw_on = s.xw_on;
                if ((size_t) m->lds_doubles_xw * sizeof(double) > 64u * 1024u) spmv_xw_allow_lds(160u * 1024u);
                if ((size_t) m->trans_lds_doubles * sizeof(double) > 64u * 1024u) spmv_t_allow_lds(160u * 1024u);
                log_msg(LOG_INFO, "unit windows: %zu of %zu row-blocks, %.1f %% of the unit nonzeros read x from LDS, "
                        "%.2f doubles staged per such nonzero, %u KB of LDS per workgroup\n", plan.n_rb_windows, plan.n_rb_units,
                        100.0 * (double) plan.unit_elems_lds / (double) std::max<uint64_t>(plan.unit_elems, 1),
                        (double) plan.staged_doubles / (double) std::max<uint64_t>(plan.unit_elems_lds, 1),
                        (unsigned) (m->lds_doubles_xw * sizeof(double) / 1024u));
            }
        } catch (...) {
            device_free(m);
            throw;
        }
    }
    if (symmetric && s.sx_plan && m->has_symsegs && !m->has_symtiles &&
        m->xcd_split.size() == 1 && !s.rbs.empty() && !s.deterministic && !s.wave_tiles) {
        try {
            SxPlan plan;
            plan_sym_pipeline(s, plan, host_threads());
            const size_t lds_need = (size_t) m->lds_doubles * sizeof(double) + m->max_slot_groups * sizeof(uint32_t) +
                                    spmv_sx_header_bytes(s.pass_stride);
            if (!m->launch_order.empty()) {
                const size_t stride = s.pass_stride;
                std::vector<SpxPass> po(plan.passes.size());
                std::vector<uint32_t> no(plan.n_sx.size());
                for (size_t i = 0; i < m->launch_order.size(); ++i) {
                    std::copy(plan.passes.begin() + (size_t) m->launch_order[i] * stride,
                              plan.passes.begin() + ((size_t) m->launch_order[i] + 1) * stride, po.begin() + i * stride);
                    no[i] = plan.n_sx[m->launch_order[i]];
                }
                plan.passes.swap(po);
                plan.n_sx.swap(no);
            }
            if (plan.n_rb_sx && lds_need <= 160u * 1024u) {
                const size_t pbytes = (plan.passes.size() + (size_t) s.pass_stride + 6 * MAX_WAVES_PER_BLOCK) * sizeof(SpxPass);
                HIP_CHECK(hipMalloc(reinterpret_cast<void **>(&m->passes_sx), pbytes));
                HIP_CHECK(hipMemset(m->passes_sx, 0, pbytes));
                HIP_CHECK(hipMemcpy(m->passes_sx, plan.passes.data(), plan.passes.size() * sizeof(SpxPass), hipMemcpyHostToDevice));
                HIP_CHECK(hipMalloc(reinterpret_cast<void **>(&m->sx_tab), plan.n_sx.size() * sizeof(uint32_t)));
                HIP_CHECK(hipMemcpy(m->sx_tab, plan.n_sx.data(), plan.n_sx.size() * sizeof(uint32_t), hipMemcpyHostToDevice));
                m->sx_elems = plan.sx_elems;
                m->sx_sym_elems = plan.sym_elems;
                m->sx_rowblocks = plan.n_rb_sx;
                m->sx_on = s.sx_on;
                if (lds_need > 64u * 1024u) spmv_sx_allow_lds(160u * 1024u);
                log_msg(LOG_INFO, "read-once pipeline: %zu row-blocks, %llu of %llu read-once passes (%.1f %% of their nonzeros) "
                        "carry their geometry in the header\n", plan.n_rb_sx, (unsigned long long) plan.sx_passes,
                        (unsigned long long) plan.sym_passes,
                        100.0 * (double) plan.sx_elems / (double) std::max<uint64_t>(plan.sym_elems, 1));
            }
        } catch (...) {
            device_free(m);
            throw;
        }
    }
    if (!m->accum && !m->n_shared && m->xcd_split.size() == 1 && m->launch_order.empty() &&
        (!symmetric || !m->n_mirror_rows) && m->n_rb >= 64 &&
        m->nrows * sizeof(double) >= host_parts_min_bytes()) {
        try {
            m->xneed_piece = host_xpiece_doubles(m->ncols);
            stream_rowblock_xpieces(s, m->ncols, m->xneed_piece, m->rb_xneed, host_threads());
        } catch (...) {
            device_free(m);
            throw;
        }
    }
    return m;
}

void device_free(DeviceMatrix *m)
{
    if (!m) return;
    if (m->arena) {
        (void) hipFree(m->arena);
    } else {
        (void) hipFree(m->rbs); (void) hipFree(m->values); (void) hipFree(m->descs);
        (void) hipFree(m->passes);
        (void) hipFree(m->cidx); (void) hipFree(m->segrows); (void) hipFree(m->shared);
        (void) hipFree(m->carry);
        if (m->carry_mv) (void) hipFree(m->carry_mv);
        if (m->dvalues) (void) hipFree(m->dvalues);
        if (m->spill) (void) hipFree(m->spill);
        if (m->fix_ptr) (void) hipFree(m->fix_ptr);
        if (m->fix_idx) (void) hipFree(m->fix_idx);
        if (m->slot_col) (void) hipFree(m->slot_col);
        if (m->mirror_rows) (void) hipFree(m->mirror_rows);
        if (m->mirror_ptr) (void) hipFree(m->mirror_ptr);
        if (m->mirror_col) (void) hipFree(m->mirror_col);
        if (m->mirror_val) (void) hipFree(m->mirror_val);
    }
    device_values_plan_drop(m);
    device_diag_plan_drop(m);
    if (m->values_f32) (void) hipFree(m->values_f32);
    if (m->passes_sx) (void) hipFree(m->passes_sx);
    if (m->sx_tab) (void) hipFree(m->sx_tab);
    if (m->passes_xw) (void) hipFree(m->passes_xw);
    if (m->xdescs) (void) hipFree(m->xdescs);
    if (m->xw_tab) (void) hipFree(m->xw_tab);
    if (m->d_x) (void) hipFree(m->d_x);
    if (m->d_y) (void) hipFree(m->d_y);
    if (m->p_x) (void) hipHostFree(m->p_x);
    if (m->p_y) (void) hipHostFree(m->p_y);
    if (m->host_stream) (void) hipStreamDestroy(m->host_stream);
    if (m->copy_stream) (void) hipStreamDestroy(m->copy_stream);
    if (m->up_stream) (void) hipStreamDestroy(m->up_stream);
    for (hipEvent_t e : m->stage_events) (void) hipEventDestroy(e);
    for (hipEvent_t e : m->part_events) (void) hipEventDestroy(e);
    delete m;
}

struct SpmvPart {
    XcdSplit split;
    uint32_t longest;
    bool first, last;
};
static void device_product(DeviceMatrix *m, int K, double alpha, const double *X, size_t ldx, double beta, double *Y,
                           size_t ldy, void *stream_, const SpmvPart *part, bool f32 = false, bool rm = false);

void device_spmv(DeviceMatrix *m, double alpha, const double *d_x, double beta,
                 double *d_y, void *stream_)
{
    device_product(m, 1, alpha, d_x, 0, beta, d_y, 0, stream_, nullptr);
}

void device_build_values_f32(DeviceMatrix *m)
{
    HIP_CHECK(hipSetDevice(m->device));
    if (m->values_f32) {
        (void) hipFree(m->values_f32);
        m->values_f32 = nullptr;
    }
    const size_t n_alloc = (m->n_values + VALUES_SLACK + 3) & ~(size_t) 3;
    const size_t n_narrow = (m->n_values + 3) & ~(size_t) 3;
    void *d = nullptr;
    if (hipMalloc(&d, n_alloc * sizeof(float)) != hipSuccess) {
        (void) hipGetLastError();
        log_msg(LOG_ERR, "spx.gpu.values_f32: no room in HBM for a float copy of the values (%zu bytes)\n", n_alloc * sizeof(float));
        throw FatalError("spx.gpu.values_f32: cannot allocate " + std::to_string(n_alloc * sizeof(float)) +
                         " bytes of HBM for the float copy of the values");
    }
    m->values_f32 = static_cast<float *>(d);
    try {
        HIP_CHECK(hipMemset(d, 0, n_alloc * sizeof(float)));
        launch_narrow_values(nullptr, m->values_f32, m->values, n_narrow);
        HIP_CHECK(hipDeviceSynchronize());
    } catch (...) {
        (void) hipFree(d);
        m->values_f32 = nullptr;
        throw;
    }
    if (!m->has_tiles && m->carry_mv) {
        spmv_mv_f32_allow_lds(160u * 1024u);
        if (!m->symmetric) spmv_mvr_f32_allow_lds(160u * 1024u);
    }
}

int64_t device_values_f32_bytes(const DeviceMatrix *m)
// ... 49 lines not shown
    if (m->ncols) launch_scale(stream_, 1, d_y, 0, 0, m->ncols, beta);
    const bool windows = m->trans_xw && m->passes_xw;
    TransArgs a{};
    a.rbs = m->rbs; a.values = m->values; a.cidx = m->cidx; a.segrows = m->segrows;
    a.passes = windows ? m->passes_xw : m->passes;
    a.descs = windows ? m->xdescs : m->descs;
    a.xw_tab = windows ? m->xw_tab : nullptr;
    a.x = d_x; a.y = d_y; a.alpha = alpha; a.pass_stride = m->pass_stride;
    const size_t lds = (windows ? (size_t) m->trans_lds_doubles : (((size_t) m->mv_rows + 1u) & ~(size_t) 1)) * sizeof(double);
    for (size_t ph = 0; ph < m->xcd_split.size(); ++ph) {
        const uint32_t blocks = 8u * m->xcd_longest[ph];
        if (blocks) launch_spmv_t(windows, m->waves, blocks, lds, stream_, a, m->xcd_split[ph]);
    }
    HIP_CHECK(hipGetLastError());
}

void device_set_trans_windows(DeviceMatrix *m, int mode)
{
    m->trans_xw = m->passes_xw && !m->symmetric && (mode == 1 || (mode < 0 && m->xw_staged < m->xw_elems));
}

int device_trans_mode(const DeviceMatrix *m)
{
    if (m->symmetric) return 0;
    return m->trans_xw && m->passes_xw ? 2 : 1;
}

static bool diagonal_at_writeout(const DeviceMatrix *m) { return m->sym_fused && !m->sym_atomic; }

static KernelArgs kernel_args(const DeviceMatrix *m, double alpha, const double *d_x, double beta, double *d_y)
{
    KernelArgs a{};
    a.rbs = m->rbs; a.values = m->values; a.descs = m->descs; a.passes = m->passes;
    a.cidx = m->cidx; a.segrows = m->segrows;
    a.x = d_x; a.y = d_y; a.pass_stride = m->pass_stride;
    a.carry = m->carry; a.alpha = alpha; a.beta = beta; a.n_rb = m->n_rb;
    a.dvalues = diagonal_at_writeout(m) ? m->dvalues : nullptr;
    a.slot_col = m->slot_col;
    a.spill = m->spill;
    return a;
}

static bool launch_rowblocks(const DeviceMatrix *m, const KernelArgs &a_, const XcdSplit &xcd_now, uint32_t blocks,
                             void *stream, bool f32 = false)
{
    if (!blocks) return false;
    if (f32 && !m->values_f32) throw FatalError("no float copy of the values");
    KernelArgs af;
    if (f32) {
        af = a_;
        af.values = reinterpret_cast<const double *>(m->values_f32);
    }
    const KernelArgs &a = f32 ? af : a_;
    const size_t lds = m->lds_doubles * sizeof(double);
    if (m->wave_tiles && !m->accum) {
        launch_spmv(m->has_tiles ? SpmvFamily::symtile_det : SpmvFamily::det, m->waves, blocks, (size_t) m->waves * lds,
                    stream, a, xcd_now, f32);
        return m->has_tiles && m->n_spill != 0;
    }
    if (m->has_tiles) {
        const size_t lds_a = lds + m->max_slot_groups * sizeof(uint32_t);
        if (m->sym_atomic && m->has_symsegs && !m->has_symtiles && m->sx_on && m->passes_sx) {
            KernelArgs as = a;
            as.passes = m->passes_sx;
            launch_spmv_sx(m->waves, blocks, lds_a + spmv_sx_header_bytes(m->pass_stride), stream, as, xcd_now, m->sx_tab, f32);
        } else if (m->sym_atomic && m->has_symsegs && !m->has_symtiles) {
            launch_spmv(SpmvFamily::symseg_notile, m->waves, blocks, lds_a, stream, a, xcd_now, f32);
        } else if (m->sym_atomic && m->has_symsegs) {
            launch_spmv(SpmvFamily::symseg, m->waves, blocks, lds_a, stream, a, xcd_now, f32);
        } else if (m->sym_atomic) {
            launch_spmv(SpmvFamily::symtile_atomic, m->waves, blocks, lds_a, stream, a, xcd_now, f32);
        } else {
            launch_spmv(SpmvFamily::symtile, m->waves, blocks, lds, stream, a, xcd_now, f32);
        }
        return m->n_spill && !m->sym_atomic;
    }
    if (m->accum) {
        launch_spmv(SpmvFamily::accum, m->waves, blocks, lds, stream, a, xcd_now, f32);
    } else if (m->xw_on && m->passes_xw) {
        KernelArgs ax = a;
        ax.passes = m->passes_xw;
        ax.descs = m->xdescs;
        ax.xw_tab = m->xw_tab;
        launch_spmv_xw(m->waves, blocks, (size_t) m->lds_doubles_xw * sizeof(double), stream, ax, xcd_now, f32);
    } else {
        launch_spmv(SpmvFamily::plain, m->waves, blocks, lds, stream, a, xcd_now, f32);
    }
    return false;
}


static size_t mv_copies(const DeviceMatrix *m) { return m->wave_tiles && !m->accum ? (size_t) m->waves : 1u; }

static size_t mv_lds_bytes(const DeviceMatrix *m, int K, bool stage)
{
    return ((size_t) K * (mv_copies(m) * m->mv_rows + (stage ? m->mv_xwin : 0u))) * sizeof(double);
}

static size_t mvsym_lds_bytes(const DeviceMatrix *m, int K, bool stage)
{
    return (size_t) K * (stage ? m->mvsym_full : m->mvsym_core) * sizeof(double) + m->max_slot_groups * sizeof(uint32_t);
}

static bool mvsym_on(const DeviceMatrix *m)
{
    return m->has_tiles && m->sym_matmat && m->sym_atomic && !m->wave_tiles && m->carry_mv;
}

int device_mv_group(const DeviceMatrix *m)
{
    if (mvsym_on(m)) {
        for (int K = MV_MAX_GROUP; K >= 2; K /= 2)
            if (mvsym_lds_bytes(m, K, false) <= MVSYM_LDS_BUDGET) return K;
        return 1;
    }
    if (m->has_tiles || !m->carry_mv) return 1;
    for (int K = MV_MAX_GROUP; K >= 2; K /= 2)
        if (mv_lds_bytes(m, K, false) <= MV_LDS_BUDGET) return K;
    return 1;
}

static uint32_t mv_n_carry(const DeviceMatrix *m) { return m->n_carry ? m->n_carry : 1u; }

static void launch_rowblocks_mv(const DeviceMatrix *m, int K, const KernelArgs &a, size_t ldx, size_t ldy,
                                const XcdSplit &xcd_now, uint32_t blocks, void *stream, bool rm, bool f32 = false)
{
    if (!blocks) return;
    if (f32 && !m->values_f32) throw FatalError("no float copy of the values");
    if (f32 && m->has_tiles) throw FatalError("the float multi-vector product has no kernel for read-once passes");
    MvArgs mv{};
    static_cast<StreamArgs &>(mv) = a;
    if (f32) mv.values = reinterpret_cast<const double *>(m->values_f32);
    mv.x = a.x; mv.y = a.y; mv.ldx = ldx; mv.ldy = ldy;
    mv.carry = m->carry_mv; mv.n_carry = mv_n_carry(m);
    mv.dvalues = a.dvalues; mv.alpha = a.alpha; mv.beta = a.beta; mv.pass_stride = a.pass_stride;
    if (rm) {
        MvrArgs mr{};
        static_cast<MvArgs &>(mr) = mv;
        mr.stage = m->mv_xwin && mv_lds_bytes(m, K, true) <= MV_LDS_BUDGET ? 1u : 0u;
        mr.x16 = ((uintptr_t) a.x % 16u == 0 && (ldx * sizeof(double)) % 16u == 0) ? 1u : 0u;
        const MvFamily family = m->wave_tiles && !m->accum ? MvFamily::det : m->accum ? MvFamily::accum : MvFamily::plain;
        (f32 ? launch_spmv_mvr_f32 : launch_spmv_mvr)(family, K, m->waves, blocks, mv_lds_bytes(m, K, mr.stage != 0), stream,
                                                      mr, xcd_now);
        return;
    }
    if (m->has_tiles) {
        MvSymArgs ms{};
        static_cast<MvArgs &>(ms) = mv;
        ms.slot_col = a.slot_col;
        ms.stage = m->mv_xwin && mvsym_lds_bytes(m, K, true) <= MVSYM_LDS_BUDGET ? 1u : 0u;
        const size_t lds = mvsym_lds_bytes(m, K, ms.stage != 0);
        launch_spmv_mvsym(K, lds > MVSYM_LDS_FEW ? MAX_WAVES_PER_BLOCK : m->waves, blocks, lds, stream, ms, xcd_now);
        return;
    }
    mv.stage = m->mv_xwin && mv_lds_bytes(m, K, true) <= MV_LDS_BUDGET ? 1u : 0u;
    const MvFamily family = m->wave_tiles && !m->accum ? MvFamily::det : m->accum ? MvFamily::accum : MvFamily::plain;
    (f32 ? launch_spmv_mv_f32 : launch_spmv_mv)(family, K, m->waves, blocks, mv_lds_bytes(m, K, mv.stage != 0), stream, mv,
                                                xcd_now);
}

static void device_product(DeviceMatrix *m, int K, double alpha, const double *X, size_t ldx, double beta, double *Y,
                           size_t ldy, void *stream_, const SpmvPart *part, bool f32, bool rm)
{
    int cur = -1;
    if (hipGetDevice(&cur) != hipSuccess || cur != m->device)
        throw FatalError("the matrix lives on HIP device " + std::to_string(m->device) +
                         ", the calling thread's current device is " + std::to_string(cur));
// ... 260 lines not shown
        return;
    }
    if (!blocks) return;
    launch_rowblocks(m, kernel_args(m, alpha, d_x, beta, d_y), xs, blocks, stream_);
    HIP_CHECK(hipGetLastError());
}

void device_set_init_rows(DeviceMatrix *m, size_t first_row)
{
    m->init_lo = first_row;
    m->init_limited = true;
}

void device_set_sym_atomic(DeviceMatrix *m, bool on)
{
    m->sym_atomic = (on || m->has_symsegs) && m->has_tiles && !m->wave_tiles;
}

void device_set_wave_tiles(DeviceMatrix *m, bool on)
{
    m->wave_tiles = on;
    if (!on) {
        m->waves = m->waves_req;
        return;
    }
    m->sym_atomic = false;
    const size_t per_copy = (size_t) m->lds_doubles * sizeof(double);
    int w = m->waves_req;
    while (w > 2 && (size_t) w * per_copy > 160u * 1024u) w /= 2;
    if ((size_t) w * per_copy > 160u * 1024u) throw FatalError("row-blocks too large for per-wavefront tiles");
    m->waves = w;
    spmv_allow_lds(SpmvFamily::det, 160u * 1024u);
    spmv_allow_lds(SpmvFamily::symtile_det, 160u * 1024u);
}
bool device_get_wave_tiles(const DeviceMatrix *m) { return m->wave_tiles; }
bool device_has_tiles(const DeviceMatrix *m) { return m->has_tiles; }

void device_set_deterministic(DeviceMatrix *m, bool on)
{
    m->deterministic = on;
    if (on) device_set_wave_tiles(m, true);
}
bool device_get_deterministic(const DeviceMatrix *m) { return m->deterministic; }
bool device_get_sym_atomic(const DeviceMatrix *m) { return m->sym_atomic; }
bool device_has_spill(const DeviceMatrix *m) { return m->has_tiles && m->n_spill; }

void device_set_waves(DeviceMatrix *m, int waves)
{
    m->waves = m->waves_req = (waves == 2 || waves == 8) ? waves : 4;
    if (m->wave_tiles) device_set_wave_tiles(m, true);
}

int device_get_waves(const DeviceMatrix *m) { return m->waves; }

int device_host_parts(const DeviceMatrix *m) { return m ? m->host_parts : 0; }
void device_set_host_parts(DeviceMatrix *m, size_t parts) { m->host_parts_want = std::min<size_t>(parts, 64); }

int device_host_order(const DeviceMatrix *m, int32_t *order, int cap)
{
    if (!m || m->host_parts < 2 || !m->host_x_by_need) return 0;
    const DeviceMatrix::ChunkPlan &cp = m->chunks[2];
    for (int j = 0; j < cap && j < (int) cp.order.size(); ++j) order[j] = (int32_t) cp.order[(size_t) j];
    return (int) cp.order.size();
}

bool device_has_sx(const DeviceMatrix *m) { return m->passes_sx != nullptr; }
void device_set_sx(DeviceMatrix *m, bool on) { m->sx_on = on && m->passes_sx && m->sym_atomic && !m->wave_tiles; }
bool device_get_sx(const DeviceMatrix *m) { return m->sx_on && m->passes_sx && m->sym_atomic && !m->wave_tiles; }
void device_sx_info(const DeviceMatrix *m, uint64_t &elems_sx, uint64_t &elems_sym, size_t &rowblocks)
{
    elems_sx = m->sx_elems;
    elems_sym = m->sx_sym_elems;
    rowblocks = m->sx_rowblocks;
}
bool device_has_xw(const DeviceMatrix *m) { return m->passes_xw != nullptr; }
void device_set_xw(DeviceMatrix *m, bool on) { m->xw_on = on && m->passes_xw && !m->wave_tiles; }
bool device_get_xw(const DeviceMatrix *m) { return m->xw_on && m->passes_xw && !m->wave_tiles; }
void device_xw_info(const DeviceMatrix *m, uint64_t &elems_lds, uint64_t &unit_elems, uint64_t &staged, uint32_t &lds_bytes)
{
    elems_lds = m->xw_elems;
    unit_elems = m->xw_unit_elems;
    staged = m->xw_staged;
    lds_bytes = (uint32_t) (m->lds_doubles_xw * sizeof(double));
}

static void ensure_staging(DeviceMatrix *m)
{
    const size_t xb = m->ncols * sizeof(double), yb = m->nrows * sizeof(double);
    if (!m->d_x) {
        HIP_CHECK(hipMalloc(reinterpret_cast<void **>(&m->d_x), xb ? xb : 8));
        HIP_CHECK(hipMalloc(reinterpret_cast<void **>(&m->d_y), yb ? yb : 8));
    }
    if (!m->p_x) {
        HIP_CHECK(hipHostMalloc(reinterpret_cast<void **>(&m->p_x), xb ? xb : 8, hipHostMallocDefault));
        HIP_CHECK(hipHostMalloc(reinterpret_cast<void **>(&m->p_y), yb ? yb : 8, hipHostMallocDefault));
    }
    if (!m->host_stream) HIP_CHECK(hipStreamCreateWithFlags(&m->host_stream, hipStreamNonBlocking));
}

double device_time_spmv(DeviceMatrix *m, int warmup, int launches)
{
    HIP_CHECK(hipSetDevice(m->device));
    if (!m->d_x) {
        const size_t xb = m->ncols * sizeof(double), yb = m->nrows * sizeof(double);
        HIP_CHECK(hipMalloc(reinterpret_cast<void **>(&m->d_x), xb ? xb : 8));
        HIP_CHECK(hipMalloc(reinterpret_cast<void **>(&m->d_y), yb ? yb : 8));
    }
    if (!m->host_stream) HIP_CHECK(hipStreamCreateWithFlags(&m->host_stream, hipStreamNonBlocking));
    hipStream_t st = m->host_stream;
    HIP_CHECK(hipMemsetAsync(m->d_x, 0, m->ncols * sizeof(double), st));
    HIP_CHECK(hipMemsetAsync(m->d_y, 0, m->nrows * sizeof(double), st));
    m->x_version = 0;
    hipEvent_t e0, e1;
    HIP_CHECK(hipEventCreate(&e0));
    HIP_CHECK(hipEventCreate(&e1));
    for (int i = 0; i < warmup; ++i) device_spmv(m, 1.0, m->d_x, 0.0, m->d_y, st);
    HIP_CHECK(hipEventRecord(e0, st));
    for (int i = 0; i < launches; ++i) device_spmv(m, 1.0, m->d_x, 0.0, m->d_y, st);
    HIP_CHECK(hipEventRecord(e1, st));
    HIP_CHECK(hipEventSynchronize(e1));
    float ms = 0.f;
    HIP_CHECK(hipEventElapsedTime(&ms, e0, e1));
    (void) hipEventDestroy(e0);
    (void) hipEventDestroy(e1);
    return 1e-3 * ms / (launches > 0 ? launches : 1);
}

namespace {


void copy_threads(void *dst, const void *src, size_t bytes)
{
    const unsigned t = bytes >= ((size_t) 4 << 20) ? std::min(4u, host_threads()) : 1u;
    if (t <= 1) {
        std::memcpy(dst, src, bytes);
        return;
    }
    const size_t part = ((bytes / t) + 63) & ~(size_t) 63;
    parallel_for(t, t, [&](size_t k) {
        const size_t a = std::min(bytes, k * part), b = k + 1 == t ? bytes : std::min(bytes, (k + 1) * part);
        if (b > a) std::memcpy(static_cast<char *>(dst) + a, static_cast<const char *>(src) + a, b - a);
    });
}

void upload_staged(double *d, double *stage, const double *h, size_t bytes, hipStream_t st)
{
    for (size_t off = 0; off < bytes; off += STAGE_PIECE) {
        const size_t n = std::min(STAGE_PIECE, bytes - off);
        copy_threads(reinterpret_cast<char *>(stage) + off, reinterpret_cast<const char *>(h) + off, n);
        HIP_CHECK(hipMemcpyAsync(reinterpret_cast<char *>(d) + off, reinterpret_cast<char *>(stage) + off, n,
                                 hipMemcpyHostToDevice, st));
    }
}

}

void device_spmv_host(DeviceMatrix *m, double alpha, const double *h_x, bool x_pinned,
                      double beta, double *h_y, bool y_pinned,
                      const std::function<void(double *, void *)> &after, uint64_t x_version)
{
    HIP_CHECK(hipSetDevice(m->device));
    const size_t xb = m->ncols * sizeof(double), yb = m->nrows * sizeof(double);
    ensure_staging(m);
    hipStream_t st = m->host_stream;
    const bool whole = m->own_lo == 0 && m->own_hi == m->nrows && (!m->symmetric || m->sym_fused);
    std::vector<size_t> bounds;
// ... 488 lines not shown
```

sparsex_amd/csrc/gpu_emit.hpp:

```cpp
#pragma once

#include "gpu_format.h"
#include "partition.hpp"

#include <utility>
#include <vector>

namespace spx {

struct SymTile {
    idx_t row0, col0;
    val_t v[64];
};

struct SymSeg {
    idx_t row, col;
    uint8_t width;
    val_t v[8];
};
typedef std::vector<SymSeg, BigAlloc<SymSeg>> SymSegVec;

struct GpuStream {
    ValVec values;
    std::vector<SpxUnitDesc> descs;
    std::vector<SpxPass> passes;
    std::vector<uint8_t> cidx;
    std::vector<uint16_t> segrows;
    std::vector<SpxRowBlock> rbs;
    std::vector<SpxSharedRow> shared;
    uint32_t n_carry = 0;
    std::vector<val_t> dvalues;
    bool sym_fused = false;
    std::vector<uint32_t> spill_col;
    std::vector<uint32_t> fix_ptr, fix_idx;
    std::vector<uint32_t> slot_group_col;
    std::vector<std::pair<uint32_t, uint32_t>> direct_cols;
    std::vector<uint32_t> mirror_rows;
    std::vector<uint32_t> mirror_ptr;
    std::vector<uint32_t> mirror_col;
    std::vector<val_t> mirror_val;
    bool sym_atomic = false;
    bool deterministic = false;
    bool wave_tiles = false;
    uint32_t n_spill = 0;
    uint32_t lds_doubles = SPX_MAX_RB_ROWS;
    uint32_t pass_stride = 0;
    uint32_t waves = 4;
    bool band_order = false;
    bool arena = false;
    uint32_t xw_budget = 0, xw_gap = 16;
    bool xw_on = false;
    bool sx_plan = false, sx_on = false;
    bool sym_matmat = false;
    size_t nnz_stored = 0;
    size_t n_unit_elems = 0;
    size_t n_delta_elems = 0;
    size_t n_units = 0;

    size_t n_pass_used() const
    {
        size_t n = 0;
        for (const SpxRowBlock &rb : rbs) n += rb.n_pass;
        return n;
    }
    size_t index_bytes() const
    {
        return descs.size() * sizeof(SpxUnitDesc) + n_pass_used() * sizeof(SpxPass) + cidx.size() +
               (sym_atomic ? slot_group_col.size() : fix_ptr.size() + fix_idx.size()) * 4 +
               (mirror_rows.size() + mirror_ptr.size() + mirror_col.size()) * 4 +
               segrows.size() * 2 + rbs.size() * sizeof(SpxRowBlock);
    }
};

struct GpuEmitParams {
    size_t target_elems = 2048;
    size_t max_rows = SPX_MAX_RB_ROWS;
    size_t sym_min_run = 2;
    size_t sym_max_run = SPX_MAX_SEG_WIDTH;
    size_t wide_rows = SPX_MAX_RB_ROWS;
    bool skip_empty = false;
    bool stack_segments = true;
    bool recut_linear = true;
    bool inline_desc = true;
    bool keep_units = true;
    bool sym_remine = true;
    bool x_window = true;
    int sym_segments = -1;
    bool sym_pure_passes = true;
    bool sym_once = true;
    const std::vector<SymTile> *tiles = nullptr;
    const SymSegVec *symsegs = nullptr;
};

void emit_gpu(const Partition &p, const GpuEmitParams &prm, GpuStream &out, unsigned nthreads = 1);

void append_stream(GpuStream &dst, GpuStream &&src, uint64_t values_placed_at = UINT64_MAX);

void finalize_stream(GpuStream &s, size_t nrows);

void mark_private_rowblocks(GpuStream &s, size_t nrows, idx_t own_lo, idx_t own_hi);

void append_sym_expanded(const Partition &lower, Partition &out, bool remine_upper = true);

struct SymRange { idx_t lo, hi; };
struct MirrorPoint { idx_t row, col; val_t val; };
void build_sym_ranges(const std::vector<Partition> &lowers, const std::vector<SymRange> &ranges,
                      bool want_tiles, std::vector<Partition> &outs,
                      std::vector<std::vector<SymTile>> &tiles, unsigned nthreads,
                      std::vector<MirrorPoint> *sparse_mirror = nullptr,
                      std::vector<SymSegVec> *symsegs = nullptr, size_t min_run = 2, size_t max_run = SPX_MAX_SEG_WIDTH);

inline void unit_elem_coords(const Elem &u, size_t k, idx_t &r, idx_t &c)
{
    const idx_t d = (idx_t) u.delta;
    switch (u.type) {
    case ENC_H:  r = u.row;               c = u.col + (idx_t) k * d; return;
    case ENC_V:  r = u.row + (idx_t) k * d; c = u.col;               return;
    case ENC_D:  r = u.row + (idx_t) k * d; c = u.col + (idx_t) k * d; return;
    case ENC_AD: r = u.row + (idx_t) k * d; c = u.col - (idx_t) k * d; return;
    default: break;
    }
    const idx_t a = (idx_t) enc_block_align(u.type);
    if (enc_is_block_row(u.type)) {
        r = u.row + (idx_t) k % a;
        c = u.col + (idx_t) k / a;
    } else {
        r = u.row + (idx_t) k / a;
        c = u.col + (idx_t) k % a;
    }
}

}
// ... 1 lines not shown
```

sparsex_amd/csrc/handles.hpp:

```cpp
#pragma once

#include <sparsex/sparsex.h>
#include <sparsex_hip.h>

#include "csx_emit.hpp"
#include "device.hpp"
#include "gpu_emit.hpp"
#include "input.hpp"
#include "xwindows.hpp"
#include "sxplan.hpp"
#include "values_plan.hpp"
#include "diag_plan.hpp"

#include <algorithm>
#include <functional>
#include <memory>
#include <mutex>
#include <string>
#include <vector>
#include <thread>

namespace spx { struct DistPlan; }

using namespace spx;

struct input {
    spx_index_t nrows, ncols, nnz;
    char type;
    MatrixInput *mat;
};

struct partition {
    size_t nr_partitions;
    size_t *parts;
    int *nodes;
    int *affinity;
    spx_index_t *row_start;
    spx_index_t *row_end;
};

struct matrix {
    spx_index_t nrows = 0, ncols = 0, nnz = 0;
    int symmetric = 0;
    spx_perm_t *permutation = SPX_INVALID_PERM;
    size_t nr_partitions = 0;
    size_t first_part = 0, last_part = 0;
    std::vector<PartBounds> bounds;
    std::vector<Partition> parts;
    std::vector<std::thread> release_threads;
    template <class F> void release_later(F &&f)
    {
        std::function<void()> work(std::forward<F>(f));
        try {
            release_threads.emplace_back([work] { work(); });
        } catch (const std::exception &) {
            work();
        }
    }
    void release_wait()
    {
        for (std::thread &t : release_threads)
            if (t.joinable()) t.join();
        release_threads.clear();
    }
    ~matrix() { release_wait(); }
    std::vector<std::vector<val_t>> diag;
    std::vector<std::unique_ptr<CsxStream>> exported;
    std::vector<std::vector<spx_index_t>> exported_rows_info;
    bool full_colind = false;
    DeviceMatrix *dev = nullptr;
    std::unique_ptr<GpuStream> host_stream;
    std::unique_ptr<GpuStream> index;
    idx_t own_lo = 0, own_hi = 0;
    std::vector<idx_t> conflict_rows;
    std::vector<idx_t> halo_cols;
    idx_t first_block_row = 0;
    spx::DistPlan *dist = nullptr;
    GpuEmitParams emit_params;
    bool auto_rb = false;
    double rb_scale = 1.0;
    int waves = 4;
    size_t col_phases = 1;
    bool col_concurrent = false;
    bool host_only = false;
    bool has_tiles = false;
    bool sym_atomic = false;
    bool deterministic = false;
    bool has_symtiles = false;
    bool has_symsegs = false;
    int spill_mode = -1;
    bool sym_matmat = false;
    int wave_tiles = -1;
    int unit_windows = -1;
    bool xw_on = false;
    int values_f32 = 0;
    int trans_windows = -1;
    bool rb_joined = false;
    int sym_pipeline = -1;
    bool sx_on = false;
    uint32_t xw_budget = 3072, xw_gap = 16;
    std::unique_ptr<spx::XwPlan> xw_inspect;
    std::unique_ptr<spx::SxPlan> sx_inspect;
    std::unique_ptr<spx::ValuesPlan> values_plan;
    size_t values_plan_bytes = 0;
    bool values_refreshed = false;
    std::unique_ptr<spx::DiagPlan> diag_plan;
    size_t diag_plan_bytes = 0;
    spx::ValuesDigest pre_refresh_digest;
    bool has_pre_refresh_digest = false, edited_while_stale = false;
    int64_t input_row_base = -1;
    int device_ordinal = -1;
    std::vector<std::vector<idx_t>> spans;
    std::vector<idx_t> max_span;
    size_t nnz_stored = 0, n_unit_elems = 0, n_delta_elems = 0, n_units = 0;
    size_t value_bytes = 0, index_bytes = 0, n_rowblocks = 0, n_shared = 0;
    double tune_seconds = 0.0, emit_seconds = 0.0;
    std::string log;
    std::mutex mtx;
};

inline idx_t dist_first_init_row(const matrix &A)
{
    idx_t first = A.first_block_row;
    if (A.conflict_rows.empty()) return first;
    if (A.has_tiles) first = std::min(first, A.conflict_rows.front());
    return std::max(first, std::min(A.conflict_rows.front(), A.own_lo));
}
```

sparsex_amd/csrc/spmv_launch.hpp:

```cpp
#pragma once

#include "gpu_format.h"
#include "xwindows.hpp"

#include <cstddef>
#include <cstdint>

namespace spx {

struct StreamArgs {
    const SpxRowBlock *rbs;
    const SpxPass *passes;
    const double *values;
    const SpxUnitDesc *descs;
    const uint8_t *cidx;
    const uint16_t *segrows;
};

struct KernelArgs : StreamArgs {
    const double *x;
    double *y;
    double *carry;
    const double *dvalues;
    double *spill;
    const uint32_t *slot_col;
    double alpha, beta;
    const double *dvalues_priv;
    double beta_priv;
    uint32_t n_rb;
    uint32_t pass_stride;
    const XwEntry *xw_tab;
};

struct XcdSplit {
    uint32_t first[9];
};

constexpr int MAX_WAVES_PER_BLOCK = 8;

enum class SpmvFamily {
    plain,
    accum,
    symtile,
    symtile_atomic,
    symseg,
    symseg_notile,
    det,
    symtile_det,
};

void launch_spmv(SpmvFamily family, int waves, unsigned blocks, size_t lds_bytes, void *stream, const KernelArgs &a,
                 const XcdSplit &xs, bool f32 = false);
void spmv_allow_lds(SpmvFamily family, size_t bytes);
void launch_sym_init(void *stream, int nvec, double *y, size_t ldy, const double *x, size_t ldx, const double *dvalues,
                     size_t lo, size_t hi, size_t own_lo, size_t own_hi, double alpha, double beta, bool f32 = false);
void launch_sym_mirror_rows(void *stream, int nvec, const uint32_t *rows, const uint32_t *ptr, const uint32_t *col,
                            const double *val, const double *x, size_t ldx, double *y, size_t ldy, double alpha,
                            uint32_t n, bool f32 = false);
void launch_scale(void *stream, int nvec, double *y, size_t ldy, size_t lo, size_t hi, double beta);
void launch_fixup(void *stream, int nvec, const SpxSharedRow *shared, uint32_t n_shared, const double *carry,
                  uint32_t n_carry, double *y, size_t ldy, double alpha, double beta, const double *dvalues,
                  const double *x, size_t ldx, bool f32 = false);
void launch_symfix(void *stream, const uint32_t *fix_ptr, const uint32_t *fix_idx, const double *spill, double *y,
                   double alpha, size_t nrows);

void launch_spmv_sx(int waves, unsigned blocks, size_t lds_bytes, void *stream, const KernelArgs &a, const XcdSplit &xs,
                    const uint32_t *sx_tab, bool f32 = false);
size_t spmv_sx_header_bytes(uint32_t pass_stride);
void spmv_sx_allow_lds(size_t bytes);

void launch_spmv_xw(int waves, unsigned blocks, size_t lds_bytes, void *stream, const KernelArgs &a, const XcdSplit &xs,
                    bool f32 = false);
void spmv_xw_allow_lds(size_t bytes);

struct TransArgs : StreamArgs {
    const double *x;
    double *y;
    double alpha;
    uint32_t pass_stride;
    const XwEntry *xw_tab;
};
void launch_spmv_t(bool windows, int waves, unsigned blocks, size_t lds_bytes, void *stream, const TransArgs &a,
                   const XcdSplit &xs);
void spmv_t_allow_lds(size_t bytes);

struct MvArgs : StreamArgs {
    const double *x;
    double *y;
    size_t ldx, ldy;
    double *carry;
    const double *dvalues;
    double alpha, beta;
    uint32_t n_carry;
    uint32_t pass_stride;
    uint32_t stage;
};
enum class MvFamily {
    plain,
    accum,
    det,
};
void launch_spmv_mv(MvFamily family, int K, int waves, unsigned blocks, size_t lds_bytes, void *stream, const MvArgs &a,
                    const XcdSplit &xs);
void spmv_mv_allow_lds(size_t bytes);
void launch_spmv_mv_f32(MvFamily family, int K, int waves, unsigned blocks, size_t lds_bytes, void *stream, const MvArgs &a,
                        const XcdSplit &xs);
void spmv_mv_f32_allow_lds(size_t bytes);

struct MvrArgs : MvArgs {
    uint32_t x16;
};
void launch_spmv_mvr(MvFamily family, int K, int waves, unsigned blocks, size_t lds_bytes, void *stream, const MvrArgs &a,
                     const XcdSplit &xs);
void spmv_mvr_allow_lds(size_t bytes);
void launch_spmv_mvr_f32(MvFamily family, int K, int waves, unsigned blocks, size_t lds_bytes, void *stream,
                         const MvrArgs &a, const XcdSplit &xs);
void spmv_mvr_f32_allow_lds(size_t bytes);
void launch_scale_rm(void *stream, int nvec, double *y, size_t ldy, size_t lo, size_t hi, double beta);
void launch_fixup_rm(void *stream, int nvec, const SpxSharedRow *shared, uint32_t n_shared, const double *carry,
                     uint32_t n_carry, double *y, size_t ldy, double alpha, double beta);

struct MvSymArgs : MvArgs {
    const uint32_t *slot_col;
};
void launch_spmv_mvsym(int K, int waves, unsigned blocks, size_t lds_bytes, void *stream, const MvSymArgs &a,
                       const XcdSplit &xs);
void spmv_mvsym_allow_lds(size_t bytes);

void launch_refresh_values(void *stream, double *dst, const uint32_t *map, const double *src, size_t n,
                           float *dst_f32 = nullptr);
void launch_gather_diag(void *stream, double *dst, const uint32_t *pos, const double *values, size_t n);
void launch_narrow_values(void *stream, float *dst, const double *src, size_t n);

}
```

sparsex_amd/csrc/spmv_xw_kernels.hip:

```cpp
#include "spmv_device.hpp"

#include <cstddef>
#include <cstdio>
#include <cstdlib>
#include <vector>

namespace spx {


template <int B, class V = double>
struct XwStage {
    uint2 q[B];
    uint32_t segl[B];
    uint32_t width[B];
    uint32_t row0[B];
    typename ValueVec<V>::pair_u va[B], vb[B];
};

template <int B, class V = double>
__device__ __forceinline__ void xw_issue(const KernelArgs &a, const SpxRowBlock &rb, const PassWords (&ps)[B],
                                         XwStage<B, V> &S, int lane)
{
#pragma unroll
    for (int b = 0; b < B; ++b) {
        const uint32_t nseg = ps[b].nseg(), W = ps[b].width();
        const bool active = (uint32_t) lane < nseg;
        const uint32_t l = active ? (uint32_t) lane : 0u;
        S.segl[b] = ps[b].seg0() + l + (active ? 0x10000u : 0u);
        S.width[b] = W;
        S.row0[b] = ps[b].w[5];
        const uint64_t mk = (ps[b].flags() & SPX_PASSF_INLINE) ? 0ull : ps[b].mask();
        const uint32_t rank = ps[b].rank0() + (active ? starts_upto(mk, lane) : 0u);
        S.q[b] = ld_stream(reinterpret_cast<const uint2 *>(a.descs + rb.desc_off + rank));
        const V *vals = reinterpret_cast<const V *>(a.values) + rb.val_off + ps[b].val_off();
        const uint32_t off_a = W == 1u ? l : 2u * l;
        const uint32_t off_b = W == 3u ? 2u * nseg + l : (W == 4u ? 2u * nseg + 2u * l : off_a);
        S.va[b] = *reinterpret_cast<const typename ValueVec<V>::pair_u *>(vals + off_a);
        S.vb[b] = *reinterpret_cast<const typename ValueVec<V>::pair_u *>(vals + off_b);
    }
}

template <int W, class V2 = spx_d2u_t>
__device__ __forceinline__ void xw_finish_pass(uint2 q, uint32_t segl, uint32_t row0, V2 va, V2 vb,
                                               double *tile, const double *xw)
{
    const UnitOrigin o = unit_origin(q.y, segl, row0);
    const int row = o.row;
    const double *xp = xw + (int) (q.x + (uint32_t) o.dcol);
    double t = (double) va.x * xp[0];
    if (W >= 2) t = fma((double) va.y, xp[1], t);
    if (W >= 3) t = fma((double) vb.x, xp[2], t);
    if (W >= 4) t = fma((double) vb.y, xp[3], t);
    if (segl >> 16) atomicAdd(&tile[row], t);
}

template <int B, class V = double>
__device__ __forceinline__ void xw_finish(const XwStage<B, V> &S, double *tile, const double *xw)
{
#pragma unroll
    for (int b = 0; b < B; ++b) {
        switch (S.width[b]) {
        case 1: xw_finish_pass<1>(S.q[b], S.segl[b], S.row0[b], S.va[b], S.vb[b], tile, xw); break;
        case 2: xw_finish_pass<2>(S.q[b], S.segl[b], S.row0[b], S.va[b], S.vb[b], tile, xw); break;
        case 3: xw_finish_pass<3>(S.q[b], S.segl[b], S.row0[b], S.va[b], S.vb[b], tile, xw); break;
        default: xw_finish_pass<4>(S.q[b], S.segl[b], S.row0[b], S.va[b], S.vb[b], tile, xw); break;
        }
    }
}

template <int W, class V = double>
__device__ __forceinline__ void xw_wide(const KernelArgs &a, const SpxRowBlock &rb, const PassWords &ps,
                                        double *tile, const double *xw, int lane)
{
    const uint32_t nseg = ps.nseg();
    const bool active = (uint32_t) lane < nseg;
    const uint32_t l = active ? (uint32_t) lane : 0u;
    const uint64_t mk = (ps.flags() & SPX_PASSF_INLINE) ? 0ull : ps.mask();
    const uint32_t rank = ps.rank0() + (active ? starts_upto(mk, lane) : 0u);
    const uint2 q = ld_stream(reinterpret_cast<const uint2 *>(a.descs + rb.desc_off + rank));
    const V *vals = reinterpret_cast<const V *>(a.values) + rb.val_off + ps.val_off();
    typename ValueVec<V>::pair v2[W / 2];
    V v1 = 0;
#pragma unroll
    for (int p = 0; p < W / 2; ++p)
        v2[p] = ld_stream(reinterpret_cast<const typename ValueVec<V>::pair *>(vals + (uint32_t) p * 2u * nseg + l * 2u));
    if (W & 1) v1 = ld_stream(vals + (uint32_t) (W / 2) * 2u * nseg + l);
    const UnitOrigin o = unit_origin(q.y, ps.seg0() + l, ps.w[5]);
    const int row = o.row;
    const double *xp = xw + (int) (q.x + (uint32_t) o.dcol);
    double t = 0.0;
#pragma unroll
    for (int p = 0; p < W / 2; ++p) {
        t = fma((double) v2[p].x, xp[2 * p], t);
        t = fma((double) v2[p].y, xp[2 * p + 1], t);
    }
    if (W & 1) t = fma((double) v1, xp[W - 1], t);
    if (active) atomicAdd(&tile[row], t);
}

template <class V = double>
__device__ __forceinline__ void xw_one(const KernelArgs &a, const SpxRowBlock &rb, const PassWords &ps,
                                       double *tile, const double *win, const double *xw, int lane)
{
    if (ps.kind() == SPX_PASS_UNIT && (ps.flags() & SPX_PASSF_XLDS)) {
        if (ps.width() <= 4u) {
            XwStage<1, V> S;
            xw_issue<1, V>(a, rb, {ps}, S, lane);
            xw_finish<1, V>(S, tile, xw);
            return;
        }
        switch (ps.width()) {
        case 5: xw_wide<5, V>(a, rb, ps, tile, xw, lane); break;
        case 6: xw_wide<6, V>(a, rb, ps, tile, xw, lane); break;
        case 7: xw_wide<7, V>(a, rb, ps, tile, xw, lane); break;
        default: xw_wide<8, V>(a, rb, ps, tile, xw, lane); break;
        }
    } else {
        run_pass<1, V>(a, rb, ps.pass(), tile, win, lane);
    }
}

template <int WAVES>
__device__ __forceinline__ int xw_in_range(int t, int lo, int hi)
{
    return (t >= lo && t < hi) ? (hi - 1 - t) / WAVES + 1 : 0;
}

template <int WAVES, class V = double>
__device__ __forceinline__ void xw_run(const KernelArgs &a, const SpxRowBlock &rb, const uint32_t *hdr, int hi,
                                       int n_in, int &t, XwStage<2, V> &A, double *tile, const double *xw, int lane)
{
    XwStage<2, V> B;
    PassWords c0, c1;
    const int n_rounds = (n_in + 1) / 2, t_end = t + n_in * WAVES;
#define SPX_XW_HEADERS()                                                                          \
    do {                                                                                          \
        t += 2 * WAVES;                                                                           \
        c0 = lds_pass(hdr, t);                                                                    \
        c1 = lds_pass(hdr, t + WAVES);                                                            \
        if (t + WAVES >= hi) c1 = no_pass(c0);                                                    \
    } while (0)
    int r = 1;
    for (; r + 1 < n_rounds; r += 2) {
        SPX_XW_HEADERS();
        xw_issue<2, V>(a, rb, {c0, c1}, B, lane);
        xw_finish<2, V>(A, tile, xw);
        SPX_XW_HEADERS();
        xw_issue<2, V>(a, rb, {c0, c1}, A, lane);
        xw_finish<2, V>(B, tile, xw);
    }
    if (r < n_rounds) {
        SPX_XW_HEADERS();
        xw_issue<2, V>(a, rb, {c0, c1}, B, lane);
        xw_finish<2, V>(A, tile, xw);
        xw_finish<2, V>(B, tile, xw);
    } else {
        xw_finish<2, V>(A, tile, xw);
    }
    t = t_end;
#undef SPX_XW_HEADERS
}

template <int WAVES, class V = double>
__device__ __forceinline__ void spmv_body_xw(const KernelArgs &a, const XcdSplit &xs, double *lds)
{
    constexpr int BLOCK_THREADS = 64 * WAVES;
    const int lane = threadIdx.x & 63;
    const int wave = __builtin_amdgcn_readfirstlane(threadIdx.x >> 6);
    const uint32_t xcd = blockIdx.x & 7u;
    const uint32_t rb_idx = xs.first[xcd] + (blockIdx.x >> 3);
    if (rb_idx >= xs.first[xcd + 1u]) return;

    const SpxPass *pass0 = a.passes + (size_t) rb_idx * a.pass_stride;
    spx_const_words_t passes = (spx_const_words_t) (uintptr_t) pass0;
    const SpxRowBlock rb = a.rbs[rb_idx];
    const uint2 xw_entry = *reinterpret_cast<const uint2 *>(a.xw_tab + (size_t) rb_idx * XW_TAB + (lane & (XW_TAB - 1)));
    PassWords c0 = load_pass(passes, wave), c1 = load_pass(passes, wave + WAVES);
    const int n_rows = rb.n_rows;
    double *tile = lds;
    for (int i = threadIdx.x; i < n_rows; i += BLOCK_THREADS) lds[i] = 0.0;
    double *win = lds + n_rows;
    {
        const int xwl = rb.xwin_len;
        const double *xsrc = a.x + rb.xwin_base;
        for (int i = threadIdx.x; i < xwl; i += BLOCK_THREADS) win[i] = xsrc[i];
    }
    double *xw = lds + ((n_rows + (int) rb.xwin_len + 1) & ~1);
    const uint32_t range = (uint32_t) __builtin_amdgcn_readlane((int) xw_entry.x, 0);
    const uint32_t xw_total = (uint32_t) __builtin_amdgcn_readlane((int) xw_entry.y, 0);
    const int lo = (int) (range & 0xffffu), hi = (int) (range >> 16);
    uint32_t *hdr = reinterpret_cast<uint32_t *>(xw + xw_total);
    uint32_t odd_base = 0, odd_at = 0xffffffffu;
#pragma unroll
    for (uint32_t k = 0; k < XW_MAX; ++k) {
        const uint32_t base = (uint32_t) __builtin_amdgcn_readlane((int) xw_entry.x, (int) (XW_RANGES + k));
        const uint32_t off_len = (uint32_t) __builtin_amdgcn_readlane((int) xw_entry.y, (int) (XW_RANGES + k));
        const uint32_t len = off_len >> 16, off = off_len & 0xffffu;
        if (len == 0) break;
        const double *src = a.x + base;
        for (uint32_t c = (uint32_t) wave * 128u; c + 1u < len; c += (uint32_t) WAVES * 128u) {
            const uint32_t i = c + 2u * (uint32_t) lane;
            if (i + 1u < len)
                __builtin_amdgcn_global_load_lds(src + i, (__attribute__((address_space(3))) void *) (xw + off + c), 16, 0, 0);
        }
        if (len & 1u) {
            odd_base = base + len - 1u;
            odd_at = off + len - 1u;
        }
    }
    if (odd_at != 0xffffffffu && threadIdx.x == 0) xw[odd_at] = a.x[odd_base];
    {
        const uint32_t n_words = 6u * (a.pass_stride + 4u * (uint32_t) WAVES);
        const uint32_t *src = reinterpret_cast<const uint32_t *>(pass0);
        for (uint32_t c = (uint32_t) wave * 256u; c < n_words; c += (uint32_t) WAVES * 256u) {
            const uint32_t i = c + 4u * (uint32_t) lane;
            if (i < n_words)
                __builtin_amdgcn_global_load_lds(src + i, (__attribute__((address_space(3))) void *) (hdr + c), 16, 0, 0);
        }
    }
    const int n_pass = rb.n_pass;
    int t = wave;
    const int n_first = xw_in_range<WAVES>(t, lo, hi);
    XwStage<2, V> A;
    if (n_first > 0) {
        if (t + WAVES >= hi) c1 = no_pass(c0);
        xw_issue<2, V>(a, rb, {c0, c1}, A, lane);
    }
    __syncthreads();

    if (n_first > 0) xw_run<WAVES, V>(a, rb, hdr, hi, n_first, t, A, tile, xw, lane);
    while (t < n_pass) {
        const int n_in = xw_in_range<WAVES>(t, lo, hi);
        c0 = lds_pass(hdr, t);
        c1 = lds_pass(hdr, t + WAVES);
        if (n_in > 0) {
            if (t + WAVES >= hi) c1 = no_pass(c0);
            xw_issue<2, V>(a, rb, {c0, c1}, A, lane);
            xw_run<WAVES, V>(a, rb, hdr, hi, n_in, t, A, tile, xw, lane);
            continue;
        }
        xw_one<V>(a, rb, c0, tile, win, xw, lane);
        if (t + WAVES < n_pass) xw_one<V>(a, rb, c1, tile, win, xw, lane);
        t += 2 * WAVES;
    }
    __syncthreads();

    if (rb.flags & SPX_RB_SHARED) {
        if (threadIdx.x == 0) a.carry[rb.carry_slot] = tile[0];
    } else {
        for (int i = threadIdx.x; i < n_rows; i += BLOCK_THREADS) {
            const size_t g = (size_t) rb.row0 + i;
            double tt = a.alpha * tile[i];
            if (a.beta != 0.0) tt += a.beta * a.y[g];
            a.y[g] = tt;
        }
    }
}

template <int WAVES>
__global__ __launch_bounds__(64 * WAVES)
void csx_spmv_xw_kernel(SPX_KERNEL_PARAMS, const XwEntry *xw_tab_)
{
    SPX_KERNEL_ARGS(a);
    a.xw_tab = xw_tab_;
    extern __shared__ double lds_dyn[];
    spmv_body_xw<WAVES>(a, xcd_split, lds_dyn);
}

template <int WAVES>
__global__ __launch_bounds__(64 * WAVES)
void csx_spmv_xw_f32_kernel(SPX_KERNEL_PARAMS, const XwEntry *xw_tab_)
{
    SPX_KERNEL_ARGS(a);
    a.xw_tab = xw_tab_;
    extern __shared__ double lds_dyn[];
    spmv_body_xw<WAVES, float>(a, xcd_split, lds_dyn);
}

void launch_spmv_xw(int waves, unsigned blocks, size_t lds_bytes, void *stream_, const KernelArgs &a, const XcdSplit &xs,
                    bool f32)
{
    hipStream_t stream = static_cast<hipStream_t>(stream_);
#define SPX_LAUNCH_XW(KERNEL, W)                                                                   \
    hipLaunchKernelGGL(KERNEL<W>, dim3(blocks), dim3(64 * W), lds_bytes, stream, a.rbs,              \
                       a.passes, a.n_rb, a.pass_stride, xs, a.values, a.descs, a.cidx, a.segrows,   \
                       a.x, a.y, a.carry, a.dvalues, a.spill, a.slot_col, a.alpha, a.beta,           \
                       a.dvalues_priv, a.beta_priv, a.xw_tab)
    if (f32) {
        if (waves == 2) SPX_LAUNCH_XW(csx_spmv_xw_f32_kernel, 2);
        else if (waves == 8) SPX_LAUNCH_XW(csx_spmv_xw_f32_kernel, 8);
        else SPX_LAUNCH_XW(csx_spmv_xw_f32_kernel, 4);
    } else {
        if (waves == 2) SPX_LAUNCH_XW(csx_spmv_xw_kernel, 2);
        else if (waves == 8) SPX_LAUNCH_XW(csx_spmv_xw_kernel, 8);
        else SPX_LAUNCH_XW(csx_spmv_xw_kernel, 4);
    }
#undef SPX_LAUNCH_XW
}

void spmv_xw_allow_lds(size_t bytes)
{
    const int b = (int) bytes;
    (void) hipFuncSetAttribute(reinterpret_cast<const void *>(&csx_spmv_xw_kernel<2>), hipFuncAttributeMaxDynamicSharedMemorySize, b);
    (void) hipFuncSetAttribute(reinterpret_cast<const void *>(&csx_spmv_xw_kernel<4>), hipFuncAttributeMaxDynamicSharedMemorySize, b);
    (void) hipFuncSetAttribute(reinterpret_cast<const void *>(&csx_spmv_xw_kernel<8>), hipFuncAttributeMaxDynamicSharedMemorySize, b);
    (void) hipFuncSetAttribute(reinterpret_cast<const void *>(&csx_spmv_xw_f32_kernel<2>), hipFuncAttributeMaxDynamicSharedMemorySize, b);
    (void) hipFuncSetAttribute(reinterpret_cast<const void *>(&csx_spmv_xw_f32_kernel<4>), hipFuncAttributeMaxDynamicSharedMemorySize, b);
    (void) hipFuncSetAttribute(reinterpret_cast<const void *>(&csx_spmv_xw_f32_kernel<8>), hipFuncAttributeMaxDynamicSharedMemorySize, b);
}

}
```

Measured before the change: 1224.

## Autotune placing matrix values in uncached HBM to bypass L2

Adds a stream_cache option (default auto) that, for large non-symmetric matrices, allocates the values array with hipDeviceMallocUncached. At tune time it times SpMV with a cached and an uncached copy and keeps whichever is faster. The goal is to stop the streamed-once values from evicting x from the L2s. It also adds an 'exact' xw kernel variant for the bypass path that avoids reading past the end of odd-width segments in uncached memory. The cost is extra tuning time and a temporary second copy of the values.

New measurement: 1210. 0.988x the previous value.

```diff
diff --git a/include/sparsex_hip.h b/include/sparsex_hip.h
--- a/include/sparsex_hip.h
+++ b/include/sparsex_hip.h
@@ -28,6 +28,7 @@
 spx_error_t spx_hip_matvec_kernel_f32(spx_value_t alpha, const spx_matrix_t *A, const spx_value_t *x_dev,
                                       spx_value_t beta, spx_value_t *y_dev, void *stream);
 int64_t spx_hip_mat_values_f32_bytes(const spx_matrix_t *A);
+int spx_hip_mat_stream_cache(const spx_matrix_t *A);
 double spx_hip_mat_values_f32_narrow_seconds(const spx_matrix_t *A);
 
 spx_error_t spx_hip_matmat_kernel(spx_value_t alpha, const spx_matrix_t *A, size_t nvec,
diff --git a/sparsex_amd/api.py b/sparsex_amd/api.py
--- a/sparsex_amd/api.py
+++ b/sparsex_amd/api.py
@@ -162,6 +162,8 @@
     L.spx_hip_matvec_kernel_f32_vec.argtypes = [d, vp, vp, d, vp, vp]
     L.spx_hip_mat_values_f32_bytes.restype = C.c_int64
     L.spx_hip_mat_values_f32_bytes.argtypes = [vp]
+    L.spx_hip_mat_stream_cache.restype = C.c_int
+    L.spx_hip_mat_stream_cache.argtypes = [vp]
     L.spx_hip_mat_values_f32_narrow_seconds.restype = C.c_double
     L.spx_hip_mat_values_f32_narrow_seconds.argtypes = [vp]
     L.spx_hip_matvec_trans_mode.restype = C.c_int
@@ -325,6 +327,9 @@
 
     def values_f32_bytes(self):
         return int(lib().spx_hip_mat_values_f32_bytes(self.handle))
+
+    def stream_cache(self):
+        return int(lib().spx_hip_mat_stream_cache(self.handle))
 
     def matvec_f32(self, alpha, x, beta, y, stream=None):
         import torch
diff --git a/sparsex_amd/csrc/api.cpp b/sparsex_amd/csrc/api.cpp
--- a/sparsex_amd/csrc/api.cpp
+++ b/sparsex_amd/csrc/api.cpp
@@ -603,6 +603,7 @@
     gs.waves = (uint32_t) A->waves;
     gs.band_order = Config::instance().get_bool("spx.gpu.band_order");
     gs.arena = Config::instance().get_bool("spx.gpu.arena");
+    gs.values_bypass = A->bypass_on && !sym;
     gs.xw_budget = (A->unit_windows != 0 && !A->deterministic && !sym) ? (A->rb_joined ? std::max(A->xw_budget, JOINED_XW_BUDGET) : A->xw_budget) : 0u;
     gs.xw_gap = A->xw_gap;
     gs.xw_on = A->xw_on;
@@ -827,6 +828,39 @@
     }
     return v == "all" ? 2 : (v == "true" ? 1 : 0);
 }
+static int read_stream_cache()
+{
+    const std::string v = Config::instance().get_str("spx.gpu.stream_cache");
+    if (v != "cached" && v != "bypass" && v != "auto") {
+        log_msg(LOG_ERR, "spx.gpu.stream_cache: cached, bypass or auto\n");
+        throw FatalError("bad spx.gpu.stream_cache");
+    }
+    return v == "auto" ? -1 : (v == "bypass" ? 1 : 0);
+}
+
+static void tune_stream_cache(spx_matrix_t *A)
+{
+    if (!A->dev || A->symmetric || A->stream_cache != -1 || A->value_bytes <= ((size_t) 256 << 20)) return;
+    if (device_values_bypass(A->dev)) return;
+    const double t_begin = now_sec();
+    A->release_wait();
+    if (!device_values_alt_make(A->dev)) return;
+    const double t_est = device_time_spmv(A->dev, 2, 3);
+    const int N = (int) std::min(100.0, std::max(8.0, 0.02 / std::max(t_est, 1e-7)));
+    double t_cached = 1e30, t_bypass = 1e30;
+    for (int rep = 0; rep < 4; ++rep) {
+        t_cached = std::min(t_cached, device_time_spmv(A->dev, rep ? 0 : std::max(2, N / 10), N));
+        device_values_alt_swap(A->dev);
+        t_bypass = std::min(t_bypass, device_time_spmv(A->dev, rep ? 0 : std::max(2, N / 10), N));
+        device_values_alt_swap(A->dev);
+    }
+    A->bypass_on = t_bypass < 0.995 * t_cached;
+    if (A->bypass_on) device_values_alt_swap(A->dev);
+    device_values_alt_drop(A->dev);
+    log_msg(LOG_INFO, "stream cache: values %s (%.2f us per SpMV from an uncached allocation, %.2f from an ordinary one; measured in %.2f s)\n",
+            A->bypass_on ? "bypass the L2s" : "stay cached", 1e6 * t_bypass, 1e6 * t_cached, now_sec() - t_begin);
+}
+
 static bool wants_values_f32(int mode, bool symmetric) { return mode == 2 || (mode == 1 && !symmetric); }
 
 static spx_matrix_t *do_tune(spx_input_t *in)
@@ -1038,6 +1072,8 @@
     A->xw_on = xw_mode == "true";
     A->trans_windows = read_trans_windows();
     A->values_f32 = read_values_f32();
+    A->stream_cache = read_stream_cache();
+    A->bypass_on = A->stream_cache == 1;
     const std::string sx_mode = cfg.get_str("spx.gpu.sym_pipeline");
     if (sx_mode != "auto" && sx_mode != "true" && sx_mode != "false") {
         log_msg(LOG_ERR, "spx.gpu.sym_pipeline: true, false or auto\n");
@@ -1068,6 +1104,7 @@
     const double t_auto = now_sec();
     if (A->dev && A->nnz_stored >= 100000 && (autotune || tune_spill || tune_wt || tune_xw))
         autotune_launch(A.get(), autotune, tune_spill, tune_wt, tune_xw);
+    tune_stream_cache(A.get());
     if (A->dev && sym && A->sym_pipeline == -1 && device_has_sx(A->dev)) {
         A->release_wait();
         const double t_est = device_time_spmv(A->dev, 2, 3);
@@ -1713,6 +1750,9 @@
     try {
         A->trans_windows = read_trans_windows();
         A->values_f32 = read_values_f32();
+        A->stream_cache = read_stream_cache();
+        A->bypass_on = A->stream_cache == 1;
+        gs->values_bypass = A->bypass_on && !A->symmetric;
     } catch (const FatalError &) {
         SETERROR_0(SPX_ERR_TUNED_MAT);
         return SPX_INVALID_MAT;
@@ -1726,6 +1766,7 @@
             A->dev = device_upload(*gs, (size_t) A->nrows, (size_t) A->ncols, A->symmetric != 0,
                                    A->own_lo, A->own_hi, A->device_ordinal);
             device_set_trans_windows(A->dev, A->trans_windows);
+            tune_stream_cache(A.get());
             if (wants_values_f32(A->values_f32, A->symmetric != 0)) device_build_values_f32(A->dev);
             keep_index(A.get(), std::move(*gs));
         } else {
@@ -2057,6 +2098,11 @@
 int64_t spx_hip_mat_values_f32_bytes(const spx_matrix_t *A)
 try {
     return A && A->dev ? device_values_f32_bytes(A->dev) : -1;
+} SPX_C_BOUNDARY(return -1;)
+
+int spx_hip_mat_stream_cache(const spx_matrix_t *A)
+try {
+    return A && A->dev ? (device_values_bypass(A->dev) ? 1 : 0) : -1;
 } SPX_C_BOUNDARY(return -1;)
 
 double spx_hip_mat_values_f32_narrow_seconds(const spx_matrix_t *A)
diff --git a/sparsex_amd/csrc/config.cpp b/sparsex_amd/csrc/config.cpp
--- a/sparsex_amd/csrc/config.cpp
+++ b/sparsex_amd/csrc/config.cpp
@@ -71,6 +71,7 @@
     props_["spx.gpu.unit_window_doubles"] = "3072";
     props_["spx.gpu.unit_window_gap"] = "16";
     props_["spx.gpu.values_f32"] = "false";
+    props_["spx.gpu.stream_cache"] = "auto";
     props_["spx.gpu.trans_windows"] = "auto";
 }
 
diff --git a/sparsex_amd/csrc/device.hpp b/sparsex_amd/csrc/device.hpp
--- a/sparsex_amd/csrc/device.hpp
+++ b/sparsex_amd/csrc/device.hpp
@@ -83,6 +83,11 @@
 void device_xw_info(const DeviceMatrix *m, uint64_t &elems_lds, uint64_t &unit_elems, uint64_t &staged_doubles,
                     uint32_t &lds_bytes);
 
+bool device_values_bypass(const DeviceMatrix *m);
+bool device_values_alt_make(DeviceMatrix *m);
+void device_values_alt_swap(DeviceMatrix *m);
+void device_values_alt_drop(DeviceMatrix *m);
+
 bool device_has_sx(const DeviceMatrix *m);
 void device_set_sx(DeviceMatrix *m, bool on);
 bool device_get_sx(const DeviceMatrix *m);
diff --git a/sparsex_amd/csrc/device_runtime.cpp b/sparsex_amd/csrc/device_runtime.cpp
--- a/sparsex_amd/csrc/device_runtime.cpp
+++ b/sparsex_amd/csrc/device_runtime.cpp
@@ -86,6 +86,8 @@
     size_t n_values = 0, n_descs = 0, n_passes = 0, n_cidx = 0, n_segrows = 0;
     void *arena = nullptr;
     size_t arena_bytes = 0;
+    bool values_bypass = false;
+    double *values_alt = nullptr;
     std::vector<uint64_t> rb_upto;
     std::vector<uint32_t> rb_row0;
     struct ChunkPlan {
@@ -162,14 +164,24 @@
 }
 
 struct Placement {
-    struct Item { void **dst; const void *src; size_t copy_bytes, alloc_bytes; };
+    struct Item { void **dst; const void *src; size_t copy_bytes, alloc_bytes; bool bypass; };
     std::vector<Item> items;
     template <typename T, typename A>
-    void put(T **dst, const std::vector<T, A> &v, size_t slack_elems = 0)
+    void put(T **dst, const std::vector<T, A> &v, size_t slack_elems = 0, bool bypass = false)
     {
         size_t bytes = (v.size() + slack_elems) * sizeof(T);
         if (bytes == 0) bytes = sizeof(T);
-        items.push_back(Item{reinterpret_cast<void **>(dst), v.data(), v.size() * sizeof(T), bytes});
+        items.push_back(Item{reinterpret_cast<void **>(dst), v.data(), v.size() * sizeof(T), bytes, bypass});
+    }
+    static void *alloc_bypass(size_t bytes)
+    {
+        void *d = nullptr;
+        if (hipExtMallocWithFlags(&d, bytes, hipDeviceMallocUncached) != hipSuccess || !d) {
+            (void) hipGetLastError();
+            log_msg(LOG_INFO, "stream cache: no uncached allocation of %zu bytes, the values go into an ordinary one\n", bytes);
+            return nullptr;
+        }
+        return d;
     }
     static size_t piece(size_t bytes)
     {
@@ -178,8 +190,21 @@
     }
     void flush(DeviceMatrix *m, bool arena)
     {
+        for (Item &it : items) {
+            if (!it.bypass) continue;
+            void *d = alloc_bypass(it.alloc_bytes);
+            if (!d) {
+                it.bypass = false;
+                continue;
+            }
+            *it.dst = d;
+            m->values_bypass = true;
+            HIP_CHECK(hipMemset(d, 0, it.alloc_bytes));
+            if (it.copy_bytes) HIP_CHECK(hipMemcpy(d, it.src, it.copy_bytes, hipMemcpyHostToDevice));
+        }
         if (!arena) {
             for (const Item &it : items) {
+                if (it.bypass) continue;
                 void *d = nullptr;
                 HIP_CHECK(hipMalloc(&d, it.alloc_bytes));
                 *it.dst = d;
@@ -189,7 +214,7 @@
             return;
         }
         size_t total = 0;
-        for (const Item &it : items) total += piece(it.alloc_bytes);
+        for (const Item &it : items) total += it.bypass ? 0 : piece(it.alloc_bytes);
         total = (total + ((size_t) 2 << 20) - 1) & ~(((size_t) 2 << 20) - 1);
         void *base = nullptr;
         HIP_CHECK(hipMalloc(&base, total));
@@ -202,6 +227,7 @@
         size_t at = 0;
         for (size_t i : order) {
             const Item &it = items[i];
+            if (it.bypass) continue;
             char *d = static_cast<char *>(base) + at;
             *it.dst = d;
             if (it.copy_bytes) HIP_CHECK(hipMemcpy(d, it.src, it.copy_bytes, hipMemcpyHostToDevice));
@@ -384,7 +410,7 @@
             if (!any) order.clear();
         }
         if (order.empty()) {
-            place.put(&m->values, s.values, VALUES_SLACK);
+            place.put(&m->values, s.values, VALUES_SLACK, s.values_bypass && !symmetric);
             place.put(&m->descs, s.descs, 8);
             place.put(&m->rbs, s.rbs);
             place.put(&m->passes, s.passes, (size_t) s.pass_stride + 6 * MAX_WAVES_PER_BLOCK);
@@ -400,7 +426,7 @@
                 std::copy(s.passes.begin() + (size_t) order[i] * stride, s.passes.begin() + ((size_t) order[i] + 1) * stride,
                           passes.begin() + i * stride);
             }
-            place.put(&m->values, s.values, VALUES_SLACK);
+            place.put(&m->values, s.values, VALUES_SLACK, s.values_bypass && !symmetric);
             place.put(&m->descs, s.descs, 8);
             place.put(&m->rbs, rbs);
             place.put(&m->passes, passes, stride + 6 * MAX_WAVES_PER_BLOCK);
@@ -535,8 +561,10 @@
 void device_free(DeviceMatrix *m)
 {
     if (!m) return;
+    if (m->values_alt) (void) hipFree(m->values_alt);
     if (m->arena) {
         (void) hipFree(m->arena);
+        if (m->values_bypass) (void) hipFree(m->values);
     } else {
         (void) hipFree(m->rbs); (void) hipFree(m->values); (void) hipFree(m->descs);
         (void) hipFree(m->passes);
@@ -752,7 +780,8 @@
         ax.passes = m->passes_xw;
         ax.descs = m->xdescs;
         ax.xw_tab = m->xw_tab;
-        launch_spmv_xw(m->waves, blocks, (size_t) m->lds_doubles_xw * sizeof(double), stream, ax, xcd_now, f32);
+        launch_spmv_xw(m->waves, blocks, (size_t) m->lds_doubles_xw * sizeof(double), stream, ax, xcd_now, f32,
+                       m->values_bypass && !f32);
     } else {
         launch_spmv(SpmvFamily::plain, m->waves, blocks, lds, stream, a, xcd_now, f32);
     }
@@ -1179,6 +1208,50 @@
     unit_elems = m->xw_unit_elems;
     staged = m->xw_staged;
     lds_bytes = (uint32_t) (m->lds_doubles_xw * sizeof(double));
+}
+
+bool device_values_bypass(const DeviceMatrix *m) { return m->values_bypass; }
+bool device_values_alt_make(DeviceMatrix *m)
+{
+    if (m->values_alt) return true;
+    if (m->symmetric || m->arena) return false;
+    HIP_CHECK(hipSetDevice(m->device));
+    const size_t bytes = (m->n_values + VALUES_SLACK) * sizeof(double);
+    size_t free_b = 0, total_b = 0;
+    if (hipMemGetInfo(&free_b, &total_b) != hipSuccess || free_b < bytes + ((size_t) 256 << 20)) {
+        (void) hipGetLastError();
+        log_msg(LOG_INFO, "stream cache: no room in HBM for a second copy of the values (%zu bytes), not measured\n", bytes);
+        return false;
+    }
+    void *d = nullptr;
+    if (m->values_bypass) {
+        if (hipMalloc(&d, bytes) != hipSuccess) {
+            (void) hipGetLastError();
+            return false;
+        }
+    } else if (!(d = Placement::alloc_bypass(bytes))) {
+        return false;
+    }
+    if (hipMemcpy(d, m->values, bytes, hipMemcpyDeviceToDevice) != hipSuccess) {
+        (void) hipGetLastError();
+        (void) hipFree(d);
+        return false;
+    }
+    m->values_alt = static_cast<double *>(d);
+    return true;
+}
+void device_values_alt_swap(DeviceMatrix *m)
+{
+    if (!m->values_alt) return;
+    std::swap(m->values, m->values_alt);
+    m->values_bypass = !m->values_bypass;
+}
+void device_values_alt_drop(DeviceMatrix *m)
+{
+    if (!m->values_alt) return;
+    HIP_CHECK(hipDeviceSynchronize());
+    (void) hipFree(m->values_alt);
+    m->values_alt = nullptr;
 }
 
 static void ensure_staging(DeviceMatrix *m)
diff --git a/sparsex_amd/csrc/gpu_emit.hpp b/sparsex_amd/csrc/gpu_emit.hpp
--- a/sparsex_amd/csrc/gpu_emit.hpp
+++ b/sparsex_amd/csrc/gpu_emit.hpp
@@ -48,6 +48,7 @@
     uint32_t waves = 4;
     bool band_order = false;
     bool arena = false;
+    bool values_bypass = false;
     uint32_t xw_budget = 0, xw_gap = 16;
     bool xw_on = false;
     bool sx_plan = false, sx_on = false;
diff --git a/sparsex_amd/csrc/handles.hpp b/sparsex_amd/csrc/handles.hpp
--- a/sparsex_amd/csrc/handles.hpp
+++ b/sparsex_amd/csrc/handles.hpp
@@ -95,6 +95,8 @@
     bool xw_on = false;
     int values_f32 = 0;
     int trans_windows = -1;
+    int stream_cache = -1;
+    bool bypass_on = false;
     bool rb_joined = false;
     int sym_pipeline = -1;
     bool sx_on = false;
diff --git a/sparsex_amd/csrc/spmv_launch.hpp b/sparsex_amd/csrc/spmv_launch.hpp
--- a/sparsex_amd/csrc/spmv_launch.hpp
+++ b/sparsex_amd/csrc/spmv_launch.hpp
@@ -70,8 +70,10 @@
 void spmv_sx_allow_lds(size_t bytes);
 
 void launch_spmv_xw(int waves, unsigned blocks, size_t lds_bytes, void *stream, const KernelArgs &a, const XcdSplit &xs,
-                    bool f32 = false);
+                    bool f32 = false, bool exact = false);
 void spmv_xw_allow_lds(size_t bytes);
+void launch_spmv_xw_exact(int waves, unsigned blocks, size_t lds_bytes, void *stream, const KernelArgs &a, const XcdSplit &xs);
+void spmv_xw_exact_allow_lds(size_t bytes);
 
 struct TransArgs : StreamArgs {
     const double *x;
diff --git a/sparsex_amd/csrc/spmv_xw_device.hpp b/sparsex_amd/csrc/spmv_xw_device.hpp
--- /dev/null
+++ b/sparsex_amd/csrc/spmv_xw_device.hpp
@@ -0,0 +1,261 @@
+#pragma once
+
+#include "spmv_device.hpp"
+
+namespace spx {
+
+
+template <int B, class V = double>
+struct XwStage {
+    uint2 q[B];
+    uint32_t segl[B];
+    uint32_t width[B];
+    uint32_t row0[B];
+    typename ValueVec<V>::pair_u va[B], vb[B];
+};
+
+template <int B, class V = double, bool EXACT = false>
+__device__ __forceinline__ void xw_issue(const KernelArgs &a, const SpxRowBlock &rb, const PassWords (&ps)[B],
+                                         XwStage<B, V> &S, int lane)
+{
+#pragma unroll
+    for (int b = 0; b < B; ++b) {
+        const uint32_t nseg = ps[b].nseg(), W = ps[b].width();
+        const bool active = (uint32_t) lane < nseg;
+        const uint32_t l = active ? (uint32_t) lane : 0u;
+        S.segl[b] = ps[b].seg0() + l + (active ? 0x10000u : 0u);
+        S.width[b] = W;
+        S.row0[b] = ps[b].w[5];
+        const uint64_t mk = (ps[b].flags() & SPX_PASSF_INLINE) ? 0ull : ps[b].mask();
+        const uint32_t rank = ps[b].rank0() + (active ? starts_upto(mk, lane) : 0u);
+        S.q[b] = ld_stream(reinterpret_cast<const uint2 *>(a.descs + rb.desc_off + rank));
+        const V *vals = reinterpret_cast<const V *>(a.values) + rb.val_off + ps[b].val_off();
+        const bool back = EXACT && (W & 1u) && l + 1u == nseg && nseg > 1u;
+        S.segl[b] += back ? 0x20000u : 0u;
+        const uint32_t lo = l - (back ? 1u : 0u);
+        const uint32_t off_a = W == 1u ? lo : 2u * l;
+        const uint32_t off_b = W == 3u ? 2u * nseg + lo : (W == 4u ? 2u * nseg + 2u * l : off_a);
+        S.va[b] = *reinterpret_cast<const typename ValueVec<V>::pair_u *>(vals + off_a);
+        S.vb[b] = *reinterpret_cast<const typename ValueVec<V>::pair_u *>(vals + off_b);
+    }
+}
+
+template <int W, bool EXACT = false, class V2 = spx_d2u_t>
+__device__ __forceinline__ void xw_finish_pass(uint2 q, uint32_t segl, uint32_t row0, V2 va, V2 vb,
+                                               double *tile, const double *xw)
+{
+    const UnitOrigin o = unit_origin(q.y, segl, row0);
+    const int row = o.row;
+    const double *xp = xw + (int) (q.x + (uint32_t) o.dcol);
+    const bool back = EXACT && (segl & 0x20000u) != 0u;
+    double t = (double) (W == 1 && back ? va.y : va.x) * xp[0];
+    if (W >= 2) t = fma((double) va.y, xp[1], t);
+    if (W >= 3) t = fma((double) (W == 3 && back ? vb.y : vb.x), xp[2], t);
+    if (W >= 4) t = fma((double) vb.y, xp[3], t);
+    if (EXACT ? (segl & 0x10000u) != 0u : (segl >> 16) != 0u) atomicAdd(&tile[row], t);
+}
+
+template <int B, class V = double, bool EXACT = false>
+__device__ __forceinline__ void xw_finish(const XwStage<B, V> &S, double *tile, const double *xw)
+{
+#pragma unroll
+    for (int b = 0; b < B; ++b) {
+        switch (S.width[b]) {
+        case 1: xw_finish_pass<1, EXACT>(S.q[b], S.segl[b], S.row0[b], S.va[b], S.vb[b], tile, xw); break;
+        case 2: xw_finish_pass<2, EXACT>(S.q[b], S.segl[b], S.row0[b], S.va[b], S.vb[b], tile, xw); break;
+        case 3: xw_finish_pass<3, EXACT>(S.q[b], S.segl[b], S.row0[b], S.va[b], S.vb[b], tile, xw); break;
+        default: xw_finish_pass<4, EXACT>(S.q[b], S.segl[b], S.row0[b], S.va[b], S.vb[b], tile, xw); break;
+        }
+    }
+}
+
+template <int W, class V = double>
+__device__ __forceinline__ void xw_wide(const KernelArgs &a, const SpxRowBlock &rb, const PassWords &ps,
+                                        double *tile, const double *xw, int lane)
+{
+    const uint32_t nseg = ps.nseg();
+    const bool active = (uint32_t) lane < nseg;
+    const uint32_t l = active ? (uint32_t) lane : 0u;
+    const uint64_t mk = (ps.flags() & SPX_PASSF_INLINE) ? 0ull : ps.mask();
+    const uint32_t rank = ps.rank0() + (active ? starts_upto(mk, lane) : 0u);
+    const uint2 q = ld_stream(reinterpret_cast<const uint2 *>(a.descs + rb.desc_off + rank));
+    const V *vals = reinterpret_cast<const V *>(a.values) + rb.val_off + ps.val_off();
+    typename ValueVec<V>::pair v2[W / 2];
+    V v1 = 0;
+#pragma unroll
+    for (int p = 0; p < W / 2; ++p)
+        v2[p] = ld_stream(reinterpret_cast<const typename ValueVec<V>::pair *>(vals + (uint32_t) p * 2u * nseg + l * 2u));
+    if (W & 1) v1 = ld_stream(vals + (uint32_t) (W / 2) * 2u * nseg + l);
+    const UnitOrigin o = unit_origin(q.y, ps.seg0() + l, ps.w[5]);
+    const int row = o.row;
+    const double *xp = xw + (int) (q.x + (uint32_t) o.dcol);
+    double t = 0.0;
+#pragma unroll
+    for (int p = 0; p < W / 2; ++p) {
+        t = fma((double) v2[p].x, xp[2 * p], t);
+        t = fma((double) v2[p].y, xp[2 * p + 1], t);
+    }
+    if (W & 1) t = fma((double) v1, xp[W - 1], t);
+    if (active) atomicAdd(&tile[row], t);
+}
+
+template <class V = double, bool EXACT = false>
+__device__ __forceinline__ void xw_one(const KernelArgs &a, const SpxRowBlock &rb, const PassWords &ps,
+                                       double *tile, const double *win, const double *xw, int lane)
+{
+    if (ps.kind() == SPX_PASS_UNIT && (ps.flags() & SPX_PASSF_XLDS)) {
+        if (ps.width() <= 4u) {
+            XwStage<1, V> S;
+            xw_issue<1, V, EXACT>(a, rb, {ps}, S, lane);
+            xw_finish<1, V, EXACT>(S, tile, xw);
+            return;
+        }
+        switch (ps.width()) {
+        case 5: xw_wide<5, V>(a, rb, ps, tile, xw, lane); break;
+        case 6: xw_wide<6, V>(a, rb, ps, tile, xw, lane); break;
+        case 7: xw_wide<7, V>(a, rb, ps, tile, xw, lane); break;
+        default: xw_wide<8, V>(a, rb, ps, tile, xw, lane); break;
+        }
+    } else {
+        run_pass<1, V>(a, rb, ps.pass(), tile, win, lane);
+    }
+}
+
+template <int WAVES>
+__device__ __forceinline__ int xw_in_range(int t, int lo, int hi)
+{
+    return (t >= lo && t < hi) ? (hi - 1 - t) / WAVES + 1 : 0;
+}
+
+template <int WAVES, class V = double, bool EXACT = false>
+__device__ __forceinline__ void xw_run(const KernelArgs &a, const SpxRowBlock &rb, const uint32_t *hdr, int hi,
+                                       int n_in, int &t, XwStage<2, V> &A, double *tile, const double *xw, int lane)
+{
+    XwStage<2, V> B;
+    PassWords c0, c1;
+    const int n_rounds = (n_in + 1) / 2, t_end = t + n_in * WAVES;
+#define SPX_XW_HEADERS()                                                                          \
+    do {                                                                                          \
+        t += 2 * WAVES;                                                                           \
+        c0 = lds_pass(hdr, t);                                                                    \
+        c1 = lds_pass(hdr, t + WAVES);                                                            \
+        if (t + WAVES >= hi) c1 = no_pass(c0);                                                    \
+    } while (0)
+    int r = 1;
+    for (; r + 1 < n_rounds; r += 2) {
+        SPX_XW_HEADERS();
+        xw_issue<2, V, EXACT>(a, rb, {c0, c1}, B, lane);
+        xw_finish<2, V, EXACT>(A, tile, xw);
+        SPX_XW_HEADERS();
+        xw_issue<2, V, EXACT>(a, rb, {c0, c1}, A, lane);
+        xw_finish<2, V, EXACT>(B, tile, xw);
+    }
+    if (r < n_rounds) {
+        SPX_XW_HEADERS();
+        xw_issue<2, V, EXACT>(a, rb, {c0, c1}, B, lane);
+        xw_finish<2, V, EXACT>(A, tile, xw);
+        xw_finish<2, V, EXACT>(B, tile, xw);
+    } else {
+        xw_finish<2, V, EXACT>(A, tile, xw);
+    }
+    t = t_end;
+#undef SPX_XW_HEADERS
+}
+
+template <int WAVES, class V = double, bool EXACT = false>
+__device__ __forceinline__ void spmv_body_xw(const KernelArgs &a, const XcdSplit &xs, double *lds)
+{
+    constexpr int BLOCK_THREADS = 64 * WAVES;
+    const int lane = threadIdx.x & 63;
+    const int wave = __builtin_amdgcn_readfirstlane(threadIdx.x >> 6);
+    const uint32_t xcd = blockIdx.x & 7u;
+    const uint32_t rb_idx = xs.first[xcd] + (blockIdx.x >> 3);
+    if (rb_idx >= xs.first[xcd + 1u]) return;
+
+    const SpxPass *pass0 = a.passes + (size_t) rb_idx * a.pass_stride;
+    spx_const_words_t passes = (spx_const_words_t) (uintptr_t) pass0;
+    const SpxRowBlock rb = a.rbs[rb_idx];
+    const uint2 xw_entry = *reinterpret_cast<const uint2 *>(a.xw_tab + (size_t) rb_idx * XW_TAB + (lane & (XW_TAB - 1)));
+    PassWords c0 = load_pass(passes, wave), c1 = load_pass(passes, wave + WAVES);
+    const int n_rows = rb.n_rows;
+    double *tile = lds;
+    for (int i = threadIdx.x; i < n_rows; i += BLOCK_THREADS) lds[i] = 0.0;
+    double *win = lds + n_rows;
+    {
+        const int xwl = rb.xwin_len;
+        const double *xsrc = a.x + rb.xwin_base;
+        for (int i = threadIdx.x; i < xwl; i += BLOCK_THREADS) win[i] = xsrc[i];
+    }
+    double *xw = lds + ((n_rows + (int) rb.xwin_len + 1) & ~1);
+    const uint32_t range = (uint32_t) __builtin_amdgcn_readlane((int) xw_entry.x, 0);
+    const uint32_t xw_total = (uint32_t) __builtin_amdgcn_readlane((int) xw_entry.y, 0);
+    const int lo = (int) (range & 0xffffu), hi = (int) (range >> 16);
+    uint32_t *hdr = reinterpret_cast<uint32_t *>(xw + xw_total);
+    uint32_t odd_base = 0, odd_at = 0xffffffffu;
+#pragma unroll
+    for (uint32_t k = 0; k < XW_MAX; ++k) {
+        const uint32_t base = (uint32_t) __builtin_amdgcn_readlane((int) xw_entry.x, (int) (XW_RANGES + k));
+        const uint32_t off_len = (uint32_t) __builtin_amdgcn_readlane((int) xw_entry.y, (int) (XW_RANGES + k));
+        const uint32_t len = off_len >> 16, off = off_len & 0xffffu;
+        if (len == 0) break;
+        const double *src = a.x + base;
+        for (uint32_t c = (uint32_t) wave * 128u; c + 1u < len; c += (uint32_t) WAVES * 128u) {
+            const uint32_t i = c + 2u * (uint32_t) lane;
+            if (i + 1u < len)
+                __builtin_amdgcn_global_load_lds(src + i, (__attribute__((address_space(3))) void *) (xw + off + c), 16, 0, 0);
+        }
+        if (len & 1u) {
+            odd_base = base + len - 1u;
+            odd_at = off + len - 1u;
+        }
+    }
+    if (odd_at != 0xffffffffu && threadIdx.x == 0) xw[odd_at] = a.x[odd_base];
+    {
+        const uint32_t n_words = 6u * (a.pass_stride + 4u * (uint32_t) WAVES);
+        const uint32_t *src = reinterpret_cast<const uint32_t *>(pass0);
+        for (uint32_t c = (uint32_t) wave * 256u; c < n_words; c += (uint32_t) WAVES * 256u) {
+            const uint32_t i = c + 4u * (uint32_t) lane;
+            if (i < n_words)
+                __builtin_amdgcn_global_load_lds(src + i, (__attribute__((address_space(3))) void *) (hdr + c), 16, 0, 0);
+        }
+    }
+    const int n_pass = rb.n_pass;
+    int t = wave;
+    const int n_first = xw_in_range<WAVES>(t, lo, hi);
+    XwStage<2, V> A;
+    if (n_first > 0) {
+        if (t + WAVES >= hi) c1 = no_pass(c0);
+        xw_issue<2, V, EXACT>(a, rb, {c0, c1}, A, lane);
+    }
+    __syncthreads();
+
+    if (n_first > 0) xw_run<WAVES, V, EXACT>(a, rb, hdr, hi, n_first, t, A, tile, xw, lane);
+    while (t < n_pass) {
+        const int n_in = xw_in_range<WAVES>(t, lo, hi);
+        c0 = lds_pass(hdr, t);
+        c1 = lds_pass(hdr, t + WAVES);
+        if (n_in > 0) {
+            if (t + WAVES >= hi) c1 = no_pass(c0);
+            xw_issue<2, V, EXACT>(a, rb, {c0, c1}, A, lane);
+            xw_run<WAVES, V, EXACT>(a, rb, hdr, hi, n_in, t, A, tile, xw, lane);
+            continue;
+        }
+        xw_one<V, EXACT>(a, rb, c0, tile, win, xw, lane);
+        if (t + WAVES < n_pass) xw_one<V, EXACT>(a, rb, c1, tile, win, xw, lane);
+        t += 2 * WAVES;
+    }
+    __syncthreads();
+
+    if (rb.flags & SPX_RB_SHARED) {
+        if (threadIdx.x == 0) a.carry[rb.carry_slot] = tile[0];
+    } else {
+        for (int i = threadIdx.x; i < n_rows; i += BLOCK_THREADS) {
+            const size_t g = (size_t) rb.row0 + i;
+            double tt = a.alpha * tile[i];
+            if (a.beta != 0.0) tt += a.beta * a.y[g];
+            a.y[g] = tt;
+        }
+    }
+}
+
+}
diff --git a/sparsex_amd/csrc/spmv_xw_exact_kernels.hip b/sparsex_amd/csrc/spmv_xw_exact_kernels.hip
--- /dev/null
+++ b/sparsex_amd/csrc/spmv_xw_exact_kernels.hip
@@ -0,0 +1,37 @@
+#include "spmv_xw_device.hpp"
+
+namespace spx {
+
+template <int WAVES>
+__global__ __launch_bounds__(64 * WAVES)
+void csx_spmv_xw_exact_kernel(SPX_KERNEL_PARAMS, const XwEntry *xw_tab_)
+{
+    SPX_KERNEL_ARGS(a);
+    a.xw_tab = xw_tab_;
+    extern __shared__ double lds_dyn[];
+    spmv_body_xw<WAVES, double, true>(a, xcd_split, lds_dyn);
+}
+
+void launch_spmv_xw_exact(int waves, unsigned blocks, size_t lds_bytes, void *stream_, const KernelArgs &a, const XcdSplit &xs)
+{
+    hipStream_t stream = static_cast<hipStream_t>(stream_);
+#define SPX_LAUNCH_XW(KERNEL, W)                                                                   \
+    hipLaunchKernelGGL(KERNEL<W>, dim3(blocks), dim3(64 * W), lds_bytes, stream, a.rbs,              \
+                       a.passes, a.n_rb, a.pass_stride, xs, a.values, a.descs, a.cidx, a.segrows,   \
+                       a.x, a.y, a.carry, a.dvalues, a.spill, a.slot_col, a.alpha, a.beta,           \
+                       a.dvalues_priv, a.beta_priv, a.xw_tab)
+    if (waves == 2) SPX_LAUNCH_XW(csx_spmv_xw_exact_kernel, 2);
+    else if (waves == 8) SPX_LAUNCH_XW(csx_spmv_xw_exact_kernel, 8);
+    else SPX_LAUNCH_XW(csx_spmv_xw_exact_kernel, 4);
+#undef SPX_LAUNCH_XW
+}
+
+void spmv_xw_exact_allow_lds(size_t bytes)
+{
+    const int b = (int) bytes;
+    (void) hipFuncSetAttribute(reinterpret_cast<const void *>(&csx_spmv_xw_exact_kernel<2>), hipFuncAttributeMaxDynamicSharedMemorySize, b);
+    (void) hipFuncSetAttribute(reinterpret_cast<const void *>(&csx_spmv_xw_exact_kernel<4>), hipFuncAttributeMaxDynamicSharedMemorySize, b);
+    (void) hipFuncSetAttribute(reinterpret_cast<const void *>(&csx_spmv_xw_exact_kernel<8>), hipFuncAttributeMaxDynamicSharedMemorySize, b);
+}
+
+}
diff --git a/sparsex_amd/csrc/spmv_xw_kernels.hip b/sparsex_amd/csrc/spmv_xw_kernels.hip
--- a/sparsex_amd/csrc/spmv_xw_kernels.hip
+++ b/sparsex_amd/csrc/spmv_xw_kernels.hip
@@ -1,4 +1,4 @@
-#include "spmv_device.hpp"
+#include "spmv_xw_device.hpp"
 
 #include <cstddef>
 #include <cstdio>
@@ -6,256 +6,6 @@
 #include <vector>
 
 namespace spx {
-
-
-template <int B, class V = double>
-struct XwStage {
-    uint2 q[B];
-    uint32_t segl[B];
-    uint32_t width[B];
-    uint32_t row0[B];
-    typename ValueVec<V>::pair_u va[B], vb[B];
-};
-
-template <int B, class V = double>
-__device__ __forceinline__ void xw_issue(const KernelArgs &a, const SpxRowBlock &rb, const PassWords (&ps)[B],
-                                         XwStage<B, V> &S, int lane)
-{
-#pragma unroll
-    for (int b = 0; b < B; ++b) {
-        const uint32_t nseg = ps[b].nseg(), W = ps[b].width();
-        const bool active = (uint32_t) lane < nseg;
-        const uint32_t l = active ? (uint32_t) lane : 0u;
-        S.segl[b] = ps[b].seg0() + l + (active ? 0x10000u : 0u);
-        S.width[b] = W;
-        S.row0[b] = ps[b].w[5];
-        const uint64_t mk = (ps[b].flags() & SPX_PASSF_INLINE) ? 0ull : ps[b].mask();
-        const uint32_t rank = ps[b].rank0() + (active ? starts_upto(mk, lane) : 0u);
-        S.q[b] = ld_stream(reinterpret_cast<const uint2 *>(a.descs + rb.desc_off + rank));
-        const V *vals = reinterpret_cast<const V *>(a.values) + rb.val_off + ps[b].val_off();
-        const uint32_t off_a = W == 1u ? l : 2u * l;
-        const uint32_t off_b = W == 3u ? 2u * nseg + l : (W == 4u ? 2u * nseg + 2u * l : off_a);
-        S.va[b] = *reinterpret_cast<const typename ValueVec<V>::pair_u *>(vals + off_a);
-        S.vb[b] = *reinterpret_cast<const typename ValueVec<V>::pair_u *>(vals + off_b);
-    }
-}
-
-template <int W, class V2 = spx_d2u_t>
-__device__ __forceinline__ void xw_finish_pass(uint2 q, uint32_t segl, uint32_t row0, V2 va, V2 vb,
-                                               double *tile, const double *xw)
-{
-    const UnitOrigin o = unit_origin(q.y, segl, row0);
-    const int row = o.row;
-    const double *xp = xw + (int) (q.x + (uint32_t) o.dcol);
-    double t = (double) va.x * xp[0];
-    if (W >= 2) t = fma((double) va.y, xp[1], t);
-    if (W >= 3) t = fma((double) vb.x, xp[2], t);
-    if (W >= 4) t = fma((double) vb.y, xp[3], t);
-    if (segl >> 16) atomicAdd(&tile[row], t);
-}
-
-template <int B, class V = double>
-__device__ __forceinline__ void xw_finish(const XwStage<B, V> &S, double *tile, const double *xw)
-{
-#pragma unroll
-    for (int b = 0; b < B; ++b) {
-        switch (S.width[b]) {
-        case 1: xw_finish_pass<1>(S.q[b], S.segl[b], S.row0[b], S.va[b], S.vb[b], tile, xw); break;
-        case 2: xw_finish_pass<2>(S.q[b], S.segl[b], S.row0[b], S.va[b], S.vb[b], tile, xw); break;
-        case 3: xw_finish_pass<3>(S.q[b], S.segl[b], S.row0[b], S.va[b], S.vb[b], tile, xw); break;
-        default: xw_finish_pass<4>(S.q[b], S.segl[b], S.row0[b], S.va[b], S.vb[b], tile, xw); break;
-        }
-    }
-}
-
-template <int W, class V = double>
-__device__ __forceinline__ void xw_wide(const KernelArgs &a, const SpxRowBlock &rb, const PassWords &ps,
-                                        double *tile, const double *xw, int lane)
-{
-    const uint32_t nseg = ps.nseg();
-    const bool active = (uint32_t) lane < nseg;
-    const uint32_t l = active ? (uint32_t) lane : 0u;
-    const uint64_t mk = (ps.flags() & SPX_PASSF_INLINE) ? 0ull : ps.mask();
-    const uint32_t rank = ps.rank0() + (active ? starts_upto(mk, lane) : 0u);
-    const uint2 q = ld_stream(reinterpret_cast<const uint2 *>(a.descs + rb.desc_off + rank));
-    const V *vals = reinterpret_cast<const V *>(a.values) + rb.val_off + ps.val_off();
-    typename ValueVec<V>::pair v2[W / 2];
-    V v1 = 0;
-#pragma unroll
-    for (int p = 0; p < W / 2; ++p)
-        v2[p] = ld_stream(reinterpret_cast<const typename ValueVec<V>::pair *>(vals + (uint32_t) p * 2u * nseg + l * 2u));
-    if (W & 1) v1 = ld_stream(vals + (uint32_t) (W / 2) * 2u * nseg + l);
-    const UnitOrigin o = unit_origin(q.y, ps.seg0() + l, ps.w[5]);
-    const int row = o.row;
-    const double *xp = xw + (int) (q.x + (uint32_t) o.dcol);
-    double t = 0.0;
-#pragma unroll
-    for (int p = 0; p < W / 2; ++p) {
-        t = fma((double) v2[p].x, xp[2 * p], t);
-        t = fma((double) v2[p].y, xp[2 * p + 1], t);
-    }
-    if (W & 1) t = fma((double) v1, xp[W - 1], t);
-    if (active) atomicAdd(&tile[row], t);
-}
-
-template <class V = double>
-__device__ __forceinline__ void xw_one(const KernelArgs &a, const SpxRowBlock &rb, const PassWords &ps,
-                                       double *tile, const double *win, const double *xw, int lane)
-{
-    if (ps.kind() == SPX_PASS_UNIT && (ps.flags() & SPX_PASSF_XLDS)) {
-        if (ps.width() <= 4u) {
-            XwStage<1, V> S;
-            xw_issue<1, V>(a, rb, {ps}, S, lane);
-            xw_finish<1, V>(S, tile, xw);
-            return;
-        }
-        switch (ps.width()) {
-        case 5: xw_wide<5, V>(a, rb, ps, tile, xw, lane); break;
-        case 6: xw_wide<6, V>(a, rb, ps, tile, xw, lane); break;
-        case 7: xw_wide<7, V>(a, rb, ps, tile, xw, lane); break;
-        default: xw_wide<8, V>(a, rb, ps, tile, xw, lane); break;
-        }
-    } else {
-        run_pass<1, V>(a, rb, ps.pass(), tile, win, lane);
-    }
-}
-
-template <int WAVES>
-__device__ __forceinline__ int xw_in_range(int t, int lo, int hi)
-{
-    return (t >= lo && t < hi) ? (hi - 1 - t) / WAVES + 1 : 0;
-}
-
-template <int WAVES, class V = double>
-__device__ __forceinline__ void xw_run(const KernelArgs &a, const SpxRowBlock &rb, const uint32_t *hdr, int hi,
-                                       int n_in, int &t, XwStage<2, V> &A, double *tile, const double *xw, int lane)
-{
-    XwStage<2, V> B;
-    PassWords c0, c1;
-    const int n_rounds = (n_in + 1) / 2, t_end = t + n_in * WAVES;
-#define SPX_XW_HEADERS()                                                                          \
-    do {                                                                                          \
-        t += 2 * WAVES;                                                                           \
-        c0 = lds_pass(hdr, t);                                                                    \
-        c1 = lds_pass(hdr, t + WAVES);                                                            \
-        if (t + WAVES >= hi) c1 = no_pass(c0);                                                    \
-    } while (0)
-    int r = 1;
-    for (; r + 1 < n_rounds; r += 2) {
-        SPX_XW_HEADERS();
-        xw_issue<2, V>(a, rb, {c0, c1}, B, lane);
-        xw_finish<2, V>(A, tile, xw);
-        SPX_XW_HEADERS();
-        xw_issue<2, V>(a, rb, {c0, c1}, A, lane);
-        xw_finish<2, V>(B, tile, xw);
-    }
-    if (r < n_rounds) {
-        SPX_XW_HEADERS();
-        xw_issue<2, V>(a, rb, {c0, c1}, B, lane);
-        xw_finish<2, V>(A, tile, xw);
-        xw_finish<2, V>(B, tile, xw);
-    } else {
-        xw_finish<2, V>(A, tile, xw);
-    }
-    t = t_end;
-#undef SPX_XW_HEADERS
-}
-
-template <int WAVES, class V = double>
-__device__ __forceinline__ void spmv_body_xw(const KernelArgs &a, const XcdSplit &xs, double *lds)
-{
-    constexpr int BLOCK_THREADS = 64 * WAVES;
-    const int lane = threadIdx.x & 63;
-    const int wave = __builtin_amdgcn_readfirstlane(threadIdx.x >> 6);
-    const uint32_t xcd = blockIdx.x & 7u;
-    const uint32_t rb_idx = xs.first[xcd] + (blockIdx.x >> 3);
-    if (rb_idx >= xs.first[xcd + 1u]) return;
-
-    const SpxPass *pass0 = a.passes + (size_t) rb_idx * a.pass_stride;
-    spx_const_words_t passes = (spx_const_words_t) (uintptr_t) pass0;
-    const SpxRowBlock rb = a.rbs[rb_idx];
-    const uint2 xw_entry = *reinterpret_cast<const uint2 *>(a.xw_tab + (size_t) rb_idx * XW_TAB + (lane & (XW_TAB - 1)));
-    PassWords c0 = load_pass(passes, wave), c1 = load_pass(passes, wave + WAVES);
-    const int n_rows = rb.n_rows;
-    double *tile = lds;
-    for (int i = threadIdx.x; i < n_rows; i += BLOCK_THREADS) lds[i] = 0.0;
-    double *win = lds + n_rows;
-    {
-        const int xwl = rb.xwin_len;
-        const double *xsrc = a.x + rb.xwin_base;
-        for (int i = threadIdx.x; i < xwl; i += BLOCK_THREADS) win[i] = xsrc[i];
-    }
-    double *xw = lds + ((n_rows + (int) rb.xwin_len + 1) & ~1);
-    const uint32_t range = (uint32_t) __builtin_amdgcn_readlane((int) xw_entry.x, 0);
-    const uint32_t xw_total = (uint32_t) __builtin_amdgcn_readlane((int) xw_entry.y, 0);
-    const int lo = (int) (range & 0xffffu), hi = (int) (range >> 16);
-    uint32_t *hdr = reinterpret_cast<uint32_t *>(xw + xw_total);
-    uint32_t odd_base = 0, odd_at = 0xffffffffu;
-#pragma unroll
-    for (uint32_t k = 0; k < XW_MAX; ++k) {
-        const uint32_t base = (uint32_t) __builtin_amdgcn_readlane((int) xw_entry.x, (int) (XW_RANGES + k));
-        const uint32_t off_len = (uint32_t) __builtin_amdgcn_readlane((int) xw_entry.y, (int) (XW_RANGES + k));
-        const uint32_t len = off_len >> 16, off = off_len & 0xffffu;
-        if (len == 0) break;
-        const double *src = a.x + base;
-        for (uint32_t c = (uint32_t) wave * 128u; c + 1u < len; c += (uint32_t) WAVES * 128u) {
-            const uint32_t i = c + 2u * (uint32_t) lane;
-            if (i + 1u < len)
-                __builtin_amdgcn_global_load_lds(src + i, (__attribute__((address_space(3))) void *) (xw + off + c), 16, 0, 0);
-        }
-        if (len & 1u) {
-            odd_base = base + len - 1u;
-            odd_at = off + len - 1u;
-        }
-    }
-    if (odd_at != 0xffffffffu && threadIdx.x == 0) xw[odd_at] = a.x[odd_base];
-    {
-        const uint32_t n_words = 6u * (a.pass_stride + 4u * (uint32_t) WAVES);
-        const uint32_t *src = reinterpret_cast<const uint32_t *>(pass0);
-        for (uint32_t c = (uint32_t) wave * 256u; c < n_words; c += (uint32_t) WAVES * 256u) {
-            const uint32_t i = c + 4u * (uint32_t) lane;
-            if (i < n_words)
-                __builtin_amdgcn_global_load_lds(src + i, (__attribute__((address_space(3))) void *) (hdr + c), 16, 0, 0);
-        }
-    }
-    const int n_pass = rb.n_pass;
-    int t = wave;
-    const int n_first = xw_in_range<WAVES>(t, lo, hi);
-    XwStage<2, V> A;
-    if (n_first > 0) {
-        if (t + WAVES >= hi) c1 = no_pass(c0);
-        xw_issue<2, V>(a, rb, {c0, c1}, A, lane);
-    }
-    __syncthreads();
-
-    if (n_first > 0) xw_run<WAVES, V>(a, rb, hdr, hi, n_first, t, A, tile, xw, lane);
-    while (t < n_pass) {
-        const int n_in = xw_in_range<WAVES>(t, lo, hi);
-        c0 = lds_pass(hdr, t);
-        c1 = lds_pass(hdr, t + WAVES);
-        if (n_in > 0) {
-            if (t + WAVES >= hi) c1 = no_pass(c0);
-            xw_issue<2, V>(a, rb, {c0, c1}, A, lane);
-            xw_run<WAVES, V>(a, rb, hdr, hi, n_in, t, A, tile, xw, lane);
-            continue;
-        }
-        xw_one<V>(a, rb, c0, tile, win, xw, lane);
-        if (t + WAVES < n_pass) xw_one<V>(a, rb, c1, tile, win, xw, lane);
-        t += 2 * WAVES;
-    }
-    __syncthreads();
-
-    if (rb.flags & SPX_RB_SHARED) {
-        if (threadIdx.x == 0) a.carry[rb.carry_slot] = tile[0];
-    } else {
-        for (int i = threadIdx.x; i < n_rows; i += BLOCK_THREADS) {
-            const size_t g = (size_t) rb.row0 + i;
-            double tt = a.alpha * tile[i];
-            if (a.beta != 0.0) tt += a.beta * a.y[g];
-            a.y[g] = tt;
-        }
-    }
-}
 
 template <int WAVES>
 __global__ __launch_bounds__(64 * WAVES)
@@ -278,8 +28,12 @@
 }
 
 void launch_spmv_xw(int waves, unsigned blocks, size_t lds_bytes, void *stream_, const KernelArgs &a, const XcdSplit &xs,
-                    bool f32)
+                    bool f32, bool exact)
 {
+    if (exact && !f32) {
+        launch_spmv_xw_exact(waves, blocks, lds_bytes, stream_, a, xs);
+        return;
+    }
     hipStream_t stream = static_cast<hipStream_t>(stream_);
 #define SPX_LAUNCH_XW(KERNEL, W)                                                                   \
     hipLaunchKernelGGL(KERNEL<W>, dim3(blocks), dim3(64 * W), lds_bytes, stream, a.rbs,              \
@@ -301,6 +55,7 @@
 void spmv_xw_allow_lds(size_t bytes)
 {
     const int b = (int) bytes;
+    spmv_xw_exact_allow_lds(bytes);
     (void) hipFuncSetAttribute(reinterpret_cast<const void *>(&csx_spmv_xw_kernel<2>), hipFuncAttributeMaxDynamicSharedMemorySize, b);
     (void) hipFuncSetAttribute(reinterpret_cast<const void *>(&csx_spmv_xw_kernel<4>), hipFuncAttributeMaxDynamicSharedMemorySize, b);
     (void) hipFuncSetAttribute(reinterpret_cast<const void *>(&csx_spmv_xw_kernel<8>), hipFuncAttributeMaxDynamicSharedMemorySize, b);
```
